# ANKITSANJYAL/nerf-few-shot-limitations

Measured on AMD Instinct MI355X. Metric: M ray-samples/sec (sample+MLP+composite) at 800^2x64, higher is better.
Workload: dtype f16; 1 GPU; 800x800 camera frame x 64 samples/ray, NeRFMLP v1 8x256, scene solid, 1 view(s)/step, 16-row pixel tiles dealt round-robin over 1 GPU(s), one launch + one all_gather per step; samples_per_ray=64, parallelism=pixel-tile x1, gather=none (one GPU)

## Files before the change

include/nerfhip.h:

```cpp
#ifndef NERFHIP_H
#define NERFHIP_H

#include <stdint.h>

#ifdef __cplusplus
extern "C" {
#endif

#define NRF_ABI_VERSION 5

#define NRF_OK            0
#define NRF_EINVAL       -1
#define NRF_EUNSUPPORTED -2
#define NRF_EHIP         -3
#define NRF_ENOMEM       -4

#define NRF_NET_V1 1
#define NRF_NET_V2 2
#define NRF_NET_V3 3

#define NRF_MMA_BF16 0
#define NRF_MMA_F16  1
#define NRF_MMA_F32  2
#define NRF_MMA_F16X3 3
// ... 79 lines not shown
                                  int64_t tile_rays, int64_t first_tile, int64_t tile_step, int64_t n_tiles,
                                  const nrf_render_opts* opts, const nrf_tail* tail,
                                  float* rgb, float* depth, float* weights, float* z_vals, void* stream);

typedef struct nrf_occupancy {
    int32_t  struct_bytes;
    int32_t  outside;
    const uint32_t* bits;
    int32_t  res[3];
    float    lo[3];
    float    scale[3];
    unsigned long long* stats;
} nrf_occupancy;

int nrf_render_rays_occ(const nrf_model* m, const float* rays_o, const float* rays_d, int64_t n_rays,
                        const nrf_render_opts* opts, const nrf_occupancy* occ,
                        float* rgb, float* depth, float* weights, float* z_vals, void* stream);
int nrf_render_camera_occ(const nrf_model* m, int H, int W, float focal, const float c2w[12],
                          int64_t ray_begin, int64_t ray_end, const nrf_render_opts* opts, const nrf_occupancy* occ,
                          float* rgb, float* depth, float* weights, float* z_vals, void* stream);
int nrf_render_cameras_tiles_occ(const nrf_model* m, int H, int W, float focal, const float* c2w, int n_cams,
                                 int64_t tile_rays, int64_t first_tile, int64_t tile_step, int64_t n_tiles,
                                 const nrf_render_opts* opts, const nrf_occupancy* occ,
                                 float* rgb, float* depth, float* weights, float* z_vals, void* stream);

int nrf_occupancy_pack(const float* density, int64_t n_cells, int k, float threshold, uint32_t* bits, void* stream);
int nrf_occupancy_dilate(const uint32_t* bits_in, const int32_t res[3], uint32_t* bits_out, void* stream);

int nrf_occupancy_mark_rays(const float* rays_o, const float* rays_d, int64_t n_rays, int n_samples,
                            const float* z_vals, const float* weights,
                            const int32_t res[3], const float lo[3], const float scale[3],
                            float weight_threshold, float seen_eps,
                            uint32_t* hit_bits, uint32_t* seen_bits, void* stream);
int nrf_occupancy_mark_camera(int H, int W, float focal, const float c2w[12], int64_t ray_begin, int64_t ray_end,
                              int n_samples, const float* z_vals, const float* weights,
                              const int32_t res[3], const float lo[3], const float scale[3],
                              float weight_threshold, float seen_eps,
                              uint32_t* hit_bits, uint32_t* seen_bits, void* stream);


int nrf_get_rays(int H, int W, float focal, const float c2w[12], int64_t ray_begin, int64_t ray_end,
                 float* rays_o, float* rays_d, void* stream);
int nrf_sample_along_rays(const float* rays_o, const float* rays_d, int64_t n_rays,
                          float near, float far, int n_samples, int lindisp, int perturb,
                          const float* t_rand, const float* z_ladder, uint64_t rng_seed,
                          float* pts, float* z_vals, void* stream);
int nrf_encode(const float* x, int64_t n, int dim, int num_freqs, int include_input, const float* freq_bands, float* out, void* stream);
int nrf_mlp_forward_v1(const nrf_model* m, int mma_mode, const float* x_enc, int64_t n, float* out4, void* stream);
int nrf_mlp_forward(const nrf_model* m, int mma_mode, const float* positions, const float* directions,
                    const float* dino, int64_t n, float* rgb, float* density, void* stream);
int nrf_composite(const float* rgb, int rgb_stride, const float* sigma, int sigma_stride,
                  const float* z_vals, const float* rays_d, int64_t n_rays, int n_samples, int white_bkgd,
                  float* out_rgb, float* out_depth, float* out_weights, void* stream);
int nrf_sample_pdf(const float* z_vals, const float* weights, int64_t n_rays, int n_samples, int n_importance,
                   const float* u, int64_t u_ray_stride, float* samples, float* z_union, void* stream);
int nrf_project_fetch(const nrf_dino* dino, const float* points, int64_t n, float* feats, float* xy, void* stream);

int nrf_sample_features(const float* features, int Hp, int Wp, int C, const float* points_2d, int64_t n, float* feats, void* stream);

int64_t nrf_fetch_backward_workspace_bytes(int Hp, int Wp, int C, int64_t n);
int nrf_project_fetch_backward(const nrf_dino* dino, const float* points, int64_t n, const float* d_feats,
                               float* d_map, int accumulate, void* ws, int64_t ws_bytes, void* stream);
int nrf_sample_features_backward(int Hp, int Wp, int C, const float* points_2d, int64_t n, const float* d_feats,
                                 float* d_map, int accumulate, void* ws, int64_t ws_bytes, void* stream);

int nrf_project_fetch_backward_points(const nrf_dino* dino, const float* points, int64_t n, const float* d_feats,
                                      float* d_points, int accumulate, void* stream);
int nrf_sample_features_backward_points(const float* features, int Hp, int Wp, int C, const float* points_2d, int64_t n,
                                        const float* d_feats, float* d_xy, void* stream);

int nrf_debug_pack(const nrf_arch* arch, const nrf_linear* linears, int n_linear, int mma_mode,
                   uint8_t* stream_out, int64_t stream_cap, int64_t* stream_bytes,
                   float* bias_out, int64_t bias_cap, int64_t* n_bias);

int nrf_debug_pack_backward(const nrf_arch* arch, const nrf_linear* linears, int n_linear, int mma_mode,
                            uint8_t* stream_out, int64_t stream_cap, int64_t* stream_bytes);
int nrf_debug_train_plan(const nrf_arch* arch, const nrf_linear* linears, int n_linear,
                         int32_t* out, int64_t cap, int64_t* n_ints);
int nrf_debug_pack_dino_grad(const nrf_arch* arch, const nrf_linear* linears, int n_linear, int mma_mode,
                             uint8_t* stream_out, int64_t stream_cap, int64_t* stream_bytes);
int nrf_debug_pack_input_grad(const nrf_arch* arch, const nrf_linear* linears, int n_linear, int mma_mode,
                              uint8_t* stream_out, int64_t stream_cap, int64_t* stream_bytes);

int nrf_debug_pack_input_grad_v3(const nrf_arch* arch, const nrf_linear* linears, int n_linear, int mma_mode,
                                 uint8_t* stream_out, int64_t stream_cap, int64_t* stream_bytes);

int nrf_debug_ray_deal(int64_t n_rays, int n_samples, int cols_per_wave, int n_cu, int64_t* head,
                       int64_t* items, int64_t cap, int64_t* n_items);

const char* nrf_last_error(void);
int nrf_abi_version(void);
int nrf_abi_sizeof(int which);

int64_t nrf_param_count(const nrf_model* m);

int nrf_model_update_device(nrf_model* m, const float* flat_params, int mode_mask, void* stream);

int64_t nrf_train_context_bytes(nrf_model* m, int mma_mode, int64_t n);

int nrf_mlp_forward_train_v1(nrf_model* m, int mma_mode, const float* x_enc, int64_t n, float* out4,
                             void* ctx, int64_t ctx_bytes, void* stream);

int nrf_mlp_backward_v1(nrf_model* m, int mma_mode, const float* out4, const float* g_out4, int64_t n,
                        void* ctx, int64_t ctx_bytes, float* flat_grad, void* stream);

int nrf_mlp_forward_train(nrf_model* m, int mma_mode, const float* positions, const float* directions,
                          const float* dino , int64_t n,
                          float* rgb, float* density, void* ctx, int64_t ctx_bytes, void* stream);
int nrf_mlp_backward(nrf_model* m, int mma_mode, const float* rgb, const float* density,
                     const float* g_rgb, const float* g_density, int64_t n,
                     void* ctx, int64_t ctx_bytes, float* flat_grad, void* stream);

int nrf_mlp_backward_dino(nrf_model* m, int mma_mode, int64_t n, void* ctx, int64_t ctx_bytes, float* d_dino, void* stream);

int nrf_mlp_backward_inputs(nrf_model* m, int mma_mode, int64_t n, void* ctx, int64_t ctx_bytes,
                            const float* positions, const float* directions,
                            float* d_x_enc, float* d_positions, float* d_directions, void* stream);

int nrf_mlp_backward_inputs_v3(nrf_model* m, int mma_mode, int64_t n, void* ctx, int64_t ctx_bytes,
                               const float* positions, const float* directions,
                               float* d_positions, float* d_directions, void* stream);

int nrf_composite_backward(const float* rgb, int rgb_stride, const float* sigma, int sigma_stride,
                           const float* z_vals, const float* rays_d, int64_t n_rays, int n_samples, int white_bkgd,
                           const float* g_rgb, const float* g_depth, const float* g_weights,
                           float* d_rgb, int d_rgb_stride, float* d_sigma, int d_sigma_stride, void* stream);
int nrf_composite_backward_geom(const float* rgb, int rgb_stride, const float* sigma, int sigma_stride,
                                const float* z_vals, const float* rays_d, int64_t n_rays, int n_samples, int white_bkgd,
                                const float* g_rgb, const float* g_depth, const float* g_weights,
                                float* d_rgb, int d_rgb_stride, float* d_sigma, int d_sigma_stride,
                                float* d_z, float* d_rays_d, void* stream);
int nrf_ray_grad(const float* d_points, const float* d_dirs, const float* z_vals, const float* rays_d,
                 const float* d_z_in, const float* d_rays_d_in, int64_t n_rays, int n_samples,
                 float* d_rays_o, float* d_rays_d, float* d_z_out, void* stream);

int nrf_mse_grad(const float* pred, const float* target, int64_t n, float weight, float* g_pred, float* loss, void* stream);

int nrf_composite_mse_backward(const float* rgb, int rgb_stride, const float* sigma, int sigma_stride,
                               const float* z_vals, const float* rays_d, int64_t n_rays, int n_samples, int white_bkgd,
                               const float* target, float weight, float* pred,
                               float* d_rgb, int d_rgb_stride, float* d_sigma, int d_sigma_stride,
                               float* ray_loss, float* zero_buf, int64_t zero_n, void* stream);

int nrf_adam_step(float* params, const float* grads, float* exp_avg, float* exp_avg_sq, int64_t n,
                  float lr, float beta1, float beta2, float eps, float weight_decay, int step, void* stream);
int nrf_adam_step_loss(float* params, const float* grads, float* exp_avg, float* exp_avg_sq, int64_t n,
                       float lr, float beta1, float beta2, float eps, float weight_decay, int step,
                       const float* ray_loss, int64_t n_rays, float loss_weight, float* loss, void* stream);

typedef struct nrf_loss_opts {
    int32_t      struct_bytes;
    float        rgb_weight;
    float        reg_weight;
    float        depth_weight;
    const float* target_depth;
    float        noise_std;
    const float* noise;
    uint64_t     rng_seed;
} nrf_loss_opts;

int nrf_composite_loss_backward(const float* rgb, int rgb_stride, const float* sigma, int sigma_stride,
                                const float* z_vals, const float* rays_d, int64_t n_rays, int n_samples, int white_bkgd,
                                const float* target, const nrf_loss_opts* loss, float* pred,
                                float* d_rgb, int d_rgb_stride, float* d_sigma, int d_sigma_stride,
                                float* ray_terms, float* zero_buf, int64_t zero_n, void* stream);

// ... 56 lines not shown
```

nerf_few_shot_limitations_amd/_lib.py:

```python
from __future__ import annotations

import ctypes as C
import os
import threading

import torch

_PKG = os.path.dirname(os.path.abspath(__file__))
LIB_PATH = os.path.join(_PKG, "libnerfhip.so")

NRF_NET_V1, NRF_NET_V2, NRF_NET_V3 = 1, 2, 3
MMA_MODES = {"bf16": 0, "f16": 1, "f32": 2, "f16x3": 3}
TRAIN_MODE = {"bf16": "bf16", "f16": "f16", "f32": "f32", "f16x3": "f32"}
TAIL_MODES = {"f16x3": 3}
TAIL_BASE_MODES = ("bf16", "f16")
ERRORS = {-1: "NRF_EINVAL", -2: "NRF_EUNSUPPORTED", -3: "NRF_EHIP", -4: "NRF_ENOMEM"}

c_float_p = C.POINTER(C.c_float)


class NrfError(RuntimeError):
    def __init__(self, code: int, msg: str):
        super().__init__(f"libnerfhip: {ERRORS.get(code, code)}: {msg}")
        self.code = code
# ... 56 lines not shown
class nrf_compact(C.Structure):
    _fields_ = [("struct_bytes", C.c_int32), ("reserved", C.c_int32), ("capacity", C.c_int64), ("index", C.c_void_p), ("slot", C.c_void_p),
                ("positions", C.c_void_p), ("directions", C.c_void_p), ("count", C.c_void_p), ("workspace", C.c_void_p),
                ("workspace_bytes", C.c_int64)]


def compact(capacity=0, index=None, slot=None, positions=None, directions=None, count=None, workspace=None, workspace_bytes=0):
    return nrf_compact(C.sizeof(nrf_compact), 0, int(capacity), index, slot, positions, directions, count, workspace, int(workspace_bytes))


SIGNATURES = {
    "nrf_abi_version": (C.c_int, []),
    "nrf_last_error": (C.c_char_p, []),
    "nrf_abi_sizeof": (C.c_int, [C.c_int]),
    "nrf_model_create": (C.c_int, [C.POINTER(C.c_void_p), C.c_int, C.POINTER(nrf_arch), C.POINTER(nrf_linear), C.c_int]),
    "nrf_model_update": (C.c_int, [C.c_void_p, C.POINTER(nrf_linear), C.c_int, C.c_void_p]),
    "nrf_model_destroy": (None, [C.c_void_p]),
    "nrf_model_flops_per_sample": (C.c_int64, [C.c_void_p]),
    "nrf_render_rays": (C.c_int, [C.c_void_p, C.c_void_p, C.c_void_p, C.c_int64, C.POINTER(nrf_render_opts),
                                  C.c_void_p, C.c_void_p, C.c_void_p, C.c_void_p, C.c_void_p]),
    "nrf_render_camera": (C.c_int, [C.c_void_p, C.c_int, C.c_int, C.c_float, C.c_float * 12, C.c_int64, C.c_int64,
                                    C.POINTER(nrf_render_opts), C.c_void_p, C.c_void_p, C.c_void_p, C.c_void_p, C.c_void_p]),
    "nrf_render_cameras_tiles": (C.c_int, [C.c_void_p, C.c_int, C.c_int, C.c_float, C.c_void_p, C.c_int, C.c_int64, C.c_int64, C.c_int64,
                                           C.c_int64, C.POINTER(nrf_render_opts), C.c_void_p, C.c_void_p, C.c_void_p, C.c_void_p, C.c_void_p]),
    "nrf_render_tail_bytes": (C.c_int64, [C.c_int64]),
    "nrf_render_rays_tail": (C.c_int, [C.c_void_p, C.c_void_p, C.c_void_p, C.c_int64, C.POINTER(nrf_render_opts), C.POINTER(nrf_tail),
                                       C.c_void_p, C.c_void_p, C.c_void_p, C.c_void_p, C.c_void_p]),
    "nrf_render_camera_tail": (C.c_int, [C.c_void_p, C.c_int, C.c_int, C.c_float, C.c_float * 12, C.c_int64, C.c_int64,
                                         C.POINTER(nrf_render_opts), C.POINTER(nrf_tail), C.c_void_p, C.c_void_p, C.c_void_p, C.c_void_p, C.c_void_p]),
    "nrf_render_cameras_tiles_tail": (C.c_int, [C.c_void_p, C.c_int, C.c_int, C.c_float, C.c_void_p, C.c_int, C.c_int64, C.c_int64, C.c_int64,
                                                C.c_int64, C.POINTER(nrf_render_opts), C.POINTER(nrf_tail), C.c_void_p, C.c_void_p, C.c_void_p,
                                                C.c_void_p, C.c_void_p]),
    "nrf_render_rays_occ": (C.c_int, [C.c_void_p, C.c_void_p, C.c_void_p, C.c_int64, C.POINTER(nrf_render_opts), C.POINTER(nrf_occupancy),
                                      C.c_void_p, C.c_void_p, C.c_void_p, C.c_void_p, C.c_void_p]),
    "nrf_render_camera_occ": (C.c_int, [C.c_void_p, C.c_int, C.c_int, C.c_float, C.c_float * 12, C.c_int64, C.c_int64,
                                        C.POINTER(nrf_render_opts), C.POINTER(nrf_occupancy), C.c_void_p, C.c_void_p, C.c_void_p, C.c_void_p, C.c_void_p]),
    "nrf_render_cameras_tiles_occ": (C.c_int, [C.c_void_p, C.c_int, C.c_int, C.c_float, C.c_void_p, C.c_int, C.c_int64, C.c_int64, C.c_int64,
                                               C.c_int64, C.POINTER(nrf_render_opts), C.POINTER(nrf_occupancy), C.c_void_p, C.c_void_p, C.c_void_p,
                                               C.c_void_p, C.c_void_p]),
    "nrf_occupancy_pack": (C.c_int, [C.c_void_p, C.c_int64, C.c_int, C.c_float, C.c_void_p, C.c_void_p]),
    "nrf_occupancy_dilate": (C.c_int, [C.c_void_p, C.c_int32 * 3, C.c_void_p, C.c_void_p]),
    "nrf_occupancy_mark_rays": (C.c_int, [C.c_void_p, C.c_void_p, C.c_int64, C.c_int, C.c_void_p, C.c_void_p, C.c_int32 * 3, C.c_float * 3,
                                          C.c_float * 3, C.c_float, C.c_float, C.c_void_p, C.c_void_p, C.c_void_p]),
    "nrf_occupancy_mark_camera": (C.c_int, [C.c_int, C.c_int, C.c_float, C.c_float * 12, C.c_int64, C.c_int64, C.c_int, C.c_void_p, C.c_void_p,
                                            C.c_int32 * 3, C.c_float * 3, C.c_float * 3, C.c_float, C.c_float, C.c_void_p, C.c_void_p, C.c_void_p]),
    "nrf_get_rays": (C.c_int, [C.c_int, C.c_int, C.c_float, C.c_float * 12, C.c_int64, C.c_int64, C.c_void_p, C.c_void_p, C.c_void_p]),
    "nrf_sample_along_rays": (C.c_int, [C.c_void_p, C.c_void_p, C.c_int64, C.c_float, C.c_float, C.c_int, C.c_int, C.c_int,
                                        C.c_void_p, C.c_void_p, C.c_uint64, C.c_void_p, C.c_void_p, C.c_void_p]),
    "nrf_encode": (C.c_int, [C.c_void_p, C.c_int64, C.c_int, C.c_int, C.c_int, C.c_void_p, C.c_void_p, C.c_void_p]),
    "nrf_mlp_forward_v1": (C.c_int, [C.c_void_p, C.c_int, C.c_void_p, C.c_int64, C.c_void_p, C.c_void_p]),
    "nrf_mlp_forward": (C.c_int, [C.c_void_p, C.c_int, C.c_void_p, C.c_void_p, C.c_void_p, C.c_int64, C.c_void_p, C.c_void_p, C.c_void_p]),
    "nrf_composite": (C.c_int, [C.c_void_p, C.c_int, C.c_void_p, C.c_int, C.c_void_p, C.c_void_p, C.c_int64, C.c_int, C.c_int,
                                C.c_void_p, C.c_void_p, C.c_void_p, C.c_void_p]),
    "nrf_sample_pdf": (C.c_int, [C.c_void_p, C.c_void_p, C.c_int64, C.c_int, C.c_int, C.c_void_p, C.c_int64, C.c_void_p, C.c_void_p, C.c_void_p]),
    "nrf_debug_pack": (C.c_int, [C.POINTER(nrf_arch), C.POINTER(nrf_linear), C.c_int, C.c_int, C.c_void_p, C.c_int64,
                                 C.POINTER(C.c_int64), C.c_void_p, C.c_int64, C.POINTER(C.c_int64)]),
    "nrf_debug_ray_deal": (C.c_int, [C.c_int64, C.c_int, C.c_int, C.c_int, C.POINTER(C.c_int64), C.POINTER(C.c_int64), C.c_int64, C.POINTER(C.c_int64)]),
    "nrf_project_fetch": (C.c_int, [C.POINTER(nrf_dino), C.c_void_p, C.c_int64, C.c_void_p, C.c_void_p, C.c_void_p]),
    "nrf_sample_features": (C.c_int, [C.c_void_p, C.c_int, C.c_int, C.c_int, C.c_void_p, C.c_int64, C.c_void_p, C.c_void_p]),
    "nrf_debug_pack_backward": (C.c_int, [C.POINTER(nrf_arch), C.POINTER(nrf_linear), C.c_int, C.c_int, C.c_void_p, C.c_int64, C.POINTER(C.c_int64)]),
    "nrf_debug_train_plan": (C.c_int, [C.POINTER(nrf_arch), C.POINTER(nrf_linear), C.c_int, C.c_void_p, C.c_int64, C.POINTER(C.c_int64)]),
    "nrf_debug_pack_dino_grad": (C.c_int, [C.POINTER(nrf_arch), C.POINTER(nrf_linear), C.c_int, C.c_int, C.c_void_p, C.c_int64, C.POINTER(C.c_int64)]),
    "nrf_fetch_backward_workspace_bytes": (C.c_int64, [C.c_int, C.c_int, C.c_int, C.c_int64]),
    "nrf_project_fetch_backward": (C.c_int, [C.POINTER(nrf_dino), C.c_void_p, C.c_int64, C.c_void_p, C.c_void_p, C.c_int, C.c_void_p, C.c_int64,
                                             C.c_void_p]),
    "nrf_sample_features_backward": (C.c_int, [C.c_int, C.c_int, C.c_int, C.c_void_p, C.c_int64, C.c_void_p, C.c_void_p, C.c_int, C.c_void_p,
                                               C.c_int64, C.c_void_p]),
    "nrf_mlp_backward_dino": (C.c_int, [C.c_void_p, C.c_int, C.c_int64, C.c_void_p, C.c_int64, C.c_void_p, C.c_void_p]),
    "nrf_mlp_backward_inputs": (C.c_int, [C.c_void_p, C.c_int, C.c_int64, C.c_void_p, C.c_int64, C.c_void_p, C.c_void_p, C.c_void_p, C.c_void_p,
                                          C.c_void_p, C.c_void_p]),
    "nrf_composite_backward_geom": (C.c_int, [C.c_void_p, C.c_int, C.c_void_p, C.c_int, C.c_void_p, C.c_void_p, C.c_int64, C.c_int, C.c_int,
                                              C.c_void_p, C.c_void_p, C.c_void_p, C.c_void_p, C.c_int, C.c_void_p, C.c_int, C.c_void_p, C.c_void_p,
                                              C.c_void_p]),
    "nrf_ray_grad": (C.c_int, [C.c_void_p, C.c_void_p, C.c_void_p, C.c_void_p, C.c_void_p, C.c_void_p, C.c_int64, C.c_int, C.c_void_p, C.c_void_p,
                               C.c_void_p, C.c_void_p]),
    "nrf_debug_pack_input_grad": (C.c_int, [C.POINTER(nrf_arch), C.POINTER(nrf_linear), C.c_int, C.c_int, C.c_void_p, C.c_int64, C.POINTER(C.c_int64)]),
    "nrf_mlp_backward_inputs_v3": (C.c_int, [C.c_void_p, C.c_int, C.c_int64, C.c_void_p, C.c_int64, C.c_void_p, C.c_void_p, C.c_void_p, C.c_void_p,
                                             C.c_void_p]),
    "nrf_project_fetch_backward_points": (C.c_int, [C.POINTER(nrf_dino), C.c_void_p, C.c_int64, C.c_void_p, C.c_void_p, C.c_int, C.c_void_p]),
    "nrf_sample_features_backward_points": (C.c_int, [C.c_void_p, C.c_int, C.c_int, C.c_int, C.c_void_p, C.c_int64, C.c_void_p, C.c_void_p,
                                                      C.c_void_p]),
    "nrf_debug_pack_input_grad_v3": (C.c_int, [C.POINTER(nrf_arch), C.POINTER(nrf_linear), C.c_int, C.c_int, C.c_void_p, C.c_int64,
                                               C.POINTER(C.c_int64)]),
    "nrf_param_count": (C.c_int64, [C.c_void_p]),
    "nrf_model_update_device": (C.c_int, [C.c_void_p, C.c_void_p, C.c_int, C.c_void_p]),
    "nrf_train_context_bytes": (C.c_int64, [C.c_void_p, C.c_int, C.c_int64]),
    "nrf_mlp_forward_train_v1": (C.c_int, [C.c_void_p, C.c_int, C.c_void_p, C.c_int64, C.c_void_p, C.c_void_p, C.c_int64, C.c_void_p]),
    "nrf_mlp_backward_v1": (C.c_int, [C.c_void_p, C.c_int, C.c_void_p, C.c_void_p, C.c_int64, C.c_void_p, C.c_int64, C.c_void_p, C.c_void_p]),
    "nrf_mlp_forward_train": (C.c_int, [C.c_void_p, C.c_int, C.c_void_p, C.c_void_p, C.c_void_p, C.c_int64, C.c_void_p, C.c_void_p, C.c_void_p, C.c_int64,
                                        C.c_void_p]),
    "nrf_mlp_backward": (C.c_int, [C.c_void_p, C.c_int, C.c_void_p, C.c_void_p, C.c_void_p, C.c_void_p, C.c_int64, C.c_void_p, C.c_int64,
                                   C.c_void_p, C.c_void_p]),
    "nrf_composite_backward": (C.c_int, [C.c_void_p, C.c_int, C.c_void_p, C.c_int, C.c_void_p, C.c_void_p, C.c_int64, C.c_int, C.c_int,
                                         C.c_void_p, C.c_void_p, C.c_void_p, C.c_void_p, C.c_int, C.c_void_p, C.c_int, C.c_void_p]),
    "nrf_mse_grad": (C.c_int, [C.c_void_p, C.c_void_p, C.c_int64, C.c_float, C.c_void_p, C.c_void_p, C.c_void_p]),
    "nrf_composite_mse_backward": (C.c_int, [C.c_void_p, C.c_int, C.c_void_p, C.c_int, C.c_void_p, C.c_void_p, C.c_int64, C.c_int, C.c_int,
                                             C.c_void_p, C.c_float, C.c_void_p, C.c_void_p, C.c_int, C.c_void_p, C.c_int, C.c_void_p, C.c_void_p,
                                             C.c_int64, C.c_void_p]),
    "nrf_adam_step": (C.c_int, [C.c_void_p, C.c_void_p, C.c_void_p, C.c_void_p, C.c_int64, C.c_float, C.c_float, C.c_float, C.c_float,
                                C.c_float, C.c_int, C.c_void_p]),
    "nrf_adam_step_loss": (C.c_int, [C.c_void_p, C.c_void_p, C.c_void_p, C.c_void_p, C.c_int64, C.c_float, C.c_float, C.c_float, C.c_float,
                                     C.c_float, C.c_int, C.c_void_p, C.c_int64, C.c_float, C.c_void_p, C.c_void_p]),
    "nrf_composite_loss_backward": (C.c_int, [C.c_void_p, C.c_int, C.c_void_p, C.c_int, C.c_void_p, C.c_void_p, C.c_int64, C.c_int, C.c_int,
                                              C.c_void_p, C.POINTER(nrf_loss_opts), C.c_void_p, C.c_void_p, C.c_int, C.c_void_p, C.c_int,
                                              C.c_void_p, C.c_void_p, C.c_int64, C.c_void_p]),
    "nrf_grad_sqnorm_workspace_bytes": (C.c_int64, [C.c_int64]),
    "nrf_grad_sqnorm_partials": (C.c_int, [C.c_void_p, C.c_int64, C.c_void_p, C.c_int64, C.c_void_p]),
    "nrf_adamw_step_loss": (C.c_int, [C.c_void_p, C.c_void_p, C.c_void_p, C.c_void_p, C.c_int64, C.c_float, C.c_float, C.c_float, C.c_float,
                                      C.c_float, C.c_int, C.c_int, C.c_float, C.c_void_p, C.c_void_p, C.c_void_p, C.c_int64, C.c_int,
                                      C.c_float, C.c_float, C.c_float, C.c_void_p, C.c_void_p]),
    "nrf_mlp_forward_train_rays": (C.c_int, [C.c_void_p, C.POINTER(nrf_train_rays), C.c_int64, C.POINTER(nrf_render_opts), C.c_void_p, C.c_void_p,
                                             C.c_void_p, C.c_int64, C.c_void_p]),
    "nrf_occupancy_compact_workspace_bytes": (C.c_int64, [C.c_int64]),
    "nrf_occupancy_compact_rays": (C.c_int, [C.POINTER(nrf_train_rays), C.c_int64, C.POINTER(nrf_render_opts), C.POINTER(nrf_occupancy),
                                             C.POINTER(nrf_compact), C.c_void_p]),
    "nrf_composite_loss_backward_indexed": (C.c_int, [C.c_void_p, C.c_int, C.c_void_p, C.c_int, C.c_void_p, C.c_void_p, C.c_int64, C.c_int, C.c_int,
                                                      C.c_void_p, C.POINTER(nrf_loss_opts), C.c_void_p, C.c_void_p, C.c_void_p, C.c_int, C.c_void_p,
                                                      C.c_int, C.c_void_p, C.c_void_p, C.c_int64, C.c_void_p]),
}

_lib = None
_lock = threading.Lock()


def lib() -> C.CDLL:
    global _lib
    if _lib is not None:
        return _lib
    with _lock:
        if _lib is None:
            if not os.path.exists(LIB_PATH):
                raise RuntimeError(f"{LIB_PATH} is missing: build it with `python -m nerf_few_shot_limitations_amd.build` "
                                   "(there is no fallback path)")
            handle = C.CDLL(LIB_PATH, mode=C.RTLD_GLOBAL)
            for name, (res, args) in SIGNATURES.items():
                fn = getattr(handle, name)
                fn.restype, fn.argtypes = res, args
            if handle.nrf_abi_version() != 5:
                raise RuntimeError("libnerfhip.so ABI version mismatch")
            for which, st in enumerate((nrf_arch, nrf_linear, nrf_dino, nrf_render_opts, nrf_tail)):
                if handle.nrf_abi_sizeof(which) != C.sizeof(st):
                    raise RuntimeError(f"libnerfhip.so: sizeof({st.__name__}) differs from the ctypes declaration")
            _lib = handle
    return _lib


def check(code: int) -> None:
    if code != 0:
        raise NrfError(code, lib().nrf_last_error().decode("utf-8", "replace"))


def ptr(t):
    if t is None:
        return None
    if not (t.is_cuda and t.dtype == torch.float32 and t.is_contiguous()):
        raise ValueError("expected a contiguous float32 tensor on the GPU")
    return t.data_ptr()


def dev_f32(t, device=None):
    if (type(t) is torch.Tensor and t.is_cuda and t.dtype == torch.float32 and not t.requires_grad and t.is_contiguous()
            and (device is None or t.device == device)):
        return t
    t = torch.as_tensor(t)
    if device is None:
        device = t.device if t.is_cuda else torch.device("cuda", torch.cuda.current_device())
# ... 77 lines not shown
```

nerf_few_shot_limitations_amd/build.py:

```python
from __future__ import annotations

import concurrent.futures as cf
import os
import shutil
import subprocess
import sys

PKG = os.path.dirname(os.path.abspath(__file__))
CSRC = os.path.join(PKG, "csrc")
OBJ = os.path.join(PKG, "build")
LIB = os.path.join(PKG, "libnerfhip.so")
INCLUDE = os.path.join(os.path.dirname(PKG), "include")

HALF16 = ["-DNRF_TU_HALF=16", "-DNRF_ACT_AGPR=1", "-mllvm", "-amdgpu-mfma-vgpr-form=1"]
HALF32 = ["-DNRF_TU_HALF=32"]
FUSED = [(f"fused_{fam}.hip", f"fused_{fam}_{half}", flags) for fam in ("v1", "v2", "v3", "v3w") for half, flags in (("16", HALF16), ("32", HALF32))]
TAIL = [("fused_tail.hip", "fused_tail", HALF32)]
OCC = [(f"fused_occ_{fam}.hip", f"fused_occ_{fam}_{half}", flags) for fam in ("v1", "v2", "v3", "v3w") for half, flags in (("16", HALF16), ("32", HALF32))]
SOURCES = FUSED + OCC + TAIL + [(f, os.path.splitext(f)[0], []) for f in
                   ("fused_kernels.hip", "train_shared.hip", "train_v1.hip", "train_v2.hip", "train_v3.hip", "train_dino_grad.hip", "train_input_grad.hip", "train_input_grad_v3.hip", "staged_kernels.hip", "api.cpp",
                    "packing.cpp")]
FLAGS = ["--offload-arch=gfx950", "-O3", "-std=c++17", "-fPIC", "-x", "hip", "-Wall", "-Wno-unused-function", "-Wno-unused-variable",
         "-fno-gpu-rdc", "-ffp-contract=off", "-Rpass-analysis=kernel-resource-usage", f"-I{INCLUDE}"]


def hipcc() -> str:
    exe = shutil.which("hipcc") or "/opt/rocm/bin/hipcc"
    if not os.path.exists(exe):
        raise RuntimeError("hipcc not found: libnerfhip.so cannot be built (ROCm toolchain required)")
    return exe


def _newest(paths):
    return max(os.path.getmtime(p) for p in paths)


def _deps():
    return [os.path.join(CSRC, f) for f in os.listdir(CSRC) if os.path.isfile(os.path.join(CSRC, f))] + [os.path.join(INCLUDE, "nerfhip.h"), os.path.abspath(__file__)]


def _obj_fresh(obj: str, cmd_key: str) -> bool:
    dep, key = obj + ".d", obj + ".cmd"
    if not (os.path.exists(obj) and os.path.exists(dep) and os.path.exists(key)):
        return False
    with open(key) as f:
        if f.read() != cmd_key:
            return False
    with open(dep) as f:
        words = f.read().replace("\\\n", " ").split()
    files = [w for w in words[1:] if not w.endswith(":")]
    t = os.path.getmtime(obj)
    return all(os.path.exists(p) and os.path.getmtime(p) <= t for p in files)


def build(force: bool = False, verbose: bool = False) -> str:
    deps = _deps()
    if not force and os.path.exists(LIB) and os.path.getmtime(LIB) >= _newest(deps):
        return LIB
    os.makedirs(OBJ, exist_ok=True)

    def one(item):
        src, name, flags = item
        obj = os.path.join(OBJ, name + ".o")
        cmd = [hipcc(), *FLAGS, *flags, "-MD", "-MF", obj + ".d", "-c", os.path.join(CSRC, src), "-o", obj]
        cmd_key = " ".join(cmd)
        if not force and _obj_fresh(obj, cmd_key):
            return obj, False
        if verbose:
            print(cmd_key, flush=True)
        r = subprocess.run(cmd, capture_output=True, text=True)
        if r.returncode != 0:
            raise RuntimeError(f"hipcc failed on {src}:\n{r.stdout}\n{r.stderr}")
        with open(obj + ".remarks", "w") as f:
            f.write(r.stderr)
        with open(obj + ".cmd", "w") as f:
            f.write(cmd_key)
        return obj, True

    with cf.ThreadPoolExecutor(max_workers=os.cpu_count() or 8) as ex:
        res = list(ex.map(one, SOURCES))
    objs = [o for o, _ in res]
    if not any(built for _, built in res) and os.path.exists(LIB) and os.path.getmtime(LIB) >= _newest(objs):
        os.utime(LIB)
        return LIB
    cmd = [hipcc(), "--offload-arch=gfx950", "-shared", "-fPIC", "-o", LIB + ".tmp", *objs]
    if verbose:
        print(" ".join(cmd), flush=True)
    r = subprocess.run(cmd, capture_output=True, text=True)
    if r.returncode != 0:
        raise RuntimeError(f"link failed:\n{r.stdout}\n{r.stderr}")
    os.replace(LIB + ".tmp", LIB)
    return LIB


def kernel_resources(obj_dir: str = OBJ):
    import re
    keys = {"VGPRs": "vgprs", "AGPRs": "agprs", "TotalSGPRs": "sgprs", "ScratchSize [bytes/lane]": "scratch", "VGPRs Spill": "vgpr_spill",
            "SGPRs Spill": "sgpr_spill", "Occupancy [waves/SIMD]": "occupancy", "LDS Size [bytes/block]": "lds"}
    out, mangled = {}, []
    for fn in sorted(os.listdir(obj_dir)):
        if not fn.endswith(".o.remarks"):
            continue
        cur = None
        with open(os.path.join(obj_dir, fn)) as f:
            for line in f:
                m = re.search(r"remark:\s+Function Name: (\S+)", line)
                if m:
                    cur = {"tu": fn[: -len(".o.remarks")]}
                    out[(fn, m.group(1))] = cur
                    mangled.append((fn, m.group(1)))
                    continue
                m = re.search(r"remark:\s+([A-Za-z ]+(?:\[[^\]]+\])?): (\d+)", line)
                if m and cur is not None and m.group(1).strip() in keys:
                    cur[keys[m.group(1).strip()]] = int(m.group(2))
    filt = shutil.which("c++filt") or shutil.which("llvm-cxxfilt") or "/usr/bin/c++filt"
    names = [n for _, n in mangled]
    if names and os.path.exists(filt):
        names = subprocess.run([filt], input="\n".join(names), capture_output=True, text=True).stdout.splitlines()
    return {f"{out[k]['tu']}: {n}": out[k] for k, n in zip(mangled, names)}


if __name__ == "__main__":
    print(build(force="--force" in sys.argv[1:], verbose=True))
```

nerf_few_shot_limitations_amd/csrc/api.cpp:

```cpp
#include <hip/hip_runtime.h>

#include <algorithm>
#include <cmath>
#include <cstdint>
#include <cstring>
#include <new>
#include <string>
#include <vector>

#include "../../include/nerfhip.h"
#include "kernels.hpp"
#include "packing.hpp"
#include "ray_deal.hpp"

namespace {

thread_local std::string g_err;

int fail(int code, const std::string& msg) {
    g_err = msg;
    return code;
}

int hip_fail(hipError_t e, const char* what) {
// ... 1 lines not shown
}

#define NRF_HIP(call)                                    \
    do {                                                 \
        const hipError_t e_ = (call);                    \
        if (e_ != hipSuccess) return hip_fail(e_, #call); \
    } while (0)

struct DeviceGuard {
    int prev = -1;
    bool ok = false;
    explicit DeviceGuard(int dev) {
        if (hipGetDevice(&prev) != hipSuccess) return;
        ok = (prev == dev) || (hipSetDevice(dev) == hipSuccess);
    }
    ~DeviceGuard() {
        int cur = -1;
        if (prev >= 0 && hipGetDevice(&cur) == hipSuccess && cur != prev) (void)hipSetDevice(prev);
    }
};

bool copy_linears(const nrf_linear* in, int n, std::vector<nrf::HostLinear>& out, std::string& err) {
    out.resize(n);
    for (int i = 0; i < n; ++i) {
        if (!in[i].weight || !in[i].bias || in[i].out_f <= 0 || in[i].in_f <= 0) {
            err = "linear " + std::to_string(i) + ": null pointer or non-positive shape";
            return false;
        }
        out[i].out_f = in[i].out_f;
        out[i].in_f = in[i].in_f;
        out[i].w.assign(in[i].weight, in[i].weight + (size_t)in[i].out_f * in[i].in_f);
        out[i].b.assign(in[i].bias, in[i].bias + in[i].out_f);
    }
    return true;
}

nrf::Camera make_camera(int H, int W, float focal, const float c2w[12]) {
    nrf::Camera c;
    c.H = H; c.W = W; c.focal = focal;
    for (int i = 0; i < 3; ++i) {
        for (int j = 0; j < 3; ++j) c.r[i][j] = c2w[4 * i + j];
        c.t[i] = c2w[4 * i + 3];
    }
    return c;
}

bool make_dino(const nrf_dino* in, int want_c, nrf::DinoDev& d, std::string& err) {
    if (!in || !in->features) { err = "dino side channel missing (features == NULL)"; return false; }
    if (in->Hp < 1 || in->Wp < 1 || in->C < 1 || in->H < 1 || in->W < 1) { err = "dino: bad map / image size"; return false; }
    if (want_c > 0 && in->C != want_c) { err = "dino: channel count differs from the model's dino_dim"; return false; }
    d.features = in->features; d.Hp = in->Hp; d.Wp = in->Wp; d.C = in->C;
    std::memcpy(d.inv_pose, in->inv_pose, sizeof(float) * 12);
    d.focal = in->focal; d.H = in->H; d.W = in->W;
    return true;
}

}

struct nrf_model {
    nrf_arch arch{};
    int device = 0;
    nrf::NetPlan plan;
    std::vector<nrf::HostLinear> lin;
    nrf::PackedStream h_stream[nrf::kModes];
    std::vector<float> h_bias;
    void* d_stream[nrf::kModes] = {nullptr, nullptr, nullptr, nullptr};
    float* d_bias = nullptr;
    unsigned long long* d_queues = nullptr;
    nrf::DeviceNet net{};
    bool train_ready = false;
    bool lin_stale = false;
    bool bfresh[3] = {false, false, false};
    nrf::ParamLayout layout;
    nrf::NetPlan bplan;
    int g_frags16 = 0;
    int i_frags16[2] = {0, 0};
    nrf::TrainPlan tplan;
    nrf::TrainDev train{};
    void* d_bstream[3] = {nullptr, nullptr, nullptr};
    int32_t* d_maps = nullptr;
    int32_t* d_src[2][3] = {{nullptr, nullptr, nullptr}, {nullptr, nullptr, nullptr}};
    int64_t n_src[2][3] = {{0, 0, 0}, {0, 0, 0}};
    int32_t* d_bias_src = nullptr;
};

namespace {

int upload(nrf_model* m, hipStream_t s, bool allocate) {
    for (int mode = 0; mode < nrf::kModes; ++mode) {
        m->h_stream[mode] = nrf::pack_stream(m->plan, m->lin, mode);
        const size_t bytes = m->h_stream[mode].bytes.size();
        if (allocate) NRF_HIP(hipMalloc(&m->d_stream[mode], bytes));
        NRF_HIP(hipMemcpyAsync(m->d_stream[mode], m->h_stream[mode].bytes.data(), bytes, hipMemcpyHostToDevice, s));
        m->net.stream[mode] = m->d_stream[mode];
        m->net.n_chunks[mode] = m->h_stream[mode].n_chunks;
    }
    m->lin_stale = false;
    if (m->train_ready) {
        for (int mode = 0; mode < 3; ++mode) {
            const nrf::PackedStream ps = nrf::pack_stream(m->bplan, m->lin, mode);
            NRF_HIP(hipMemcpyAsync(m->d_bstream[mode], ps.bytes.data(), ps.bytes.size(), hipMemcpyHostToDevice, s));
            NRF_HIP(hipStreamSynchronize(s));
            m->bfresh[mode] = true;
        }
    }
    m->h_bias = nrf::pack_bias(m->plan, m->lin);
    if (allocate) NRF_HIP(hipMalloc((void**)&m->d_bias, m->h_bias.size() * sizeof(float)));
    if (allocate) {
        NRF_HIP(hipMalloc((void**)&m->d_queues, nrf::kQueueSlots * sizeof(unsigned long long)));
        m->net.queues = m->d_queues;
    }
    NRF_HIP(hipMemcpyAsync(m->d_bias, m->h_bias.data(), m->h_bias.size() * sizeof(float), hipMemcpyHostToDevice, s));
    NRF_HIP(hipStreamSynchronize(s));
    m->net.bias = m->d_bias;
    m->net.n_bias = m->plan.n_bias;
    m->net.flops_per_sample = m->plan.flops_per_sample;
    return NRF_OK;
}

int ensure_sources(nrf_model* m) {
    if (m->d_src[0][0]) return NRF_OK;
    m->layout = nrf::param_layout(m->lin);
    for (int kind = 0; kind < 3; ++kind) {
        const std::vector<int32_t> src = nrf::stream_sources(m->plan, m->layout, kind);
        NRF_HIP(hipMalloc((void**)&m->d_src[0][kind], src.size() * sizeof(int32_t)));
        NRF_HIP(hipMemcpy(m->d_src[0][kind], src.data(), src.size() * sizeof(int32_t), hipMemcpyHostToDevice));
        m->n_src[0][kind] = (int64_t)src.size();
    }
    const std::vector<int32_t> bsrc = nrf::bias_sources(m->plan, m->layout);
    NRF_HIP(hipMalloc((void**)&m->d_bias_src, bsrc.size() * sizeof(int32_t)));
    NRF_HIP(hipMemcpy(m->d_bias_src, bsrc.data(), bsrc.size() * sizeof(int32_t), hipMemcpyHostToDevice));
    return NRF_OK;
}

int ensure_train(nrf_model* m) {
    if (m->train_ready) return NRF_OK;
    int rc = ensure_sources(m);
    if (rc != NRF_OK) return rc;
    std::string err;
    if (!nrf::make_backward_plan(m->arch, m->lin, m->bplan, err) || !nrf::make_train_plan(m->arch, m->plan, m->layout, m->tplan, err))
        return fail(NRF_EUNSUPPORTED, err);
    if ((int)m->tplan.slot_tiles.size() > nrf::kMaxSlots || (int)m->tplan.jobs.size() > nrf::kMaxJobs || m->tplan.n_mask_slots > nrf::kMaxMaskSlots)
        return fail(NRF_EUNSUPPORTED, "network too deep for the training path");
    if (m->arch.net == NRF_NET_V3) {
        nrf::NetPlan gplan;
        if (!nrf::make_dino_grad_plan(m->arch, m->lin, gplan, err)) return fail(NRF_EUNSUPPORTED, err);
        m->g_frags16 = gplan.layers[0].MT * gplan.layers[0].KT * 2;
        m->bplan.layers.push_back(gplan.layers[0]);
        nrf::NetPlan iplan;
        if (!nrf::make_input_grad_v3_plan(m->arch, m->lin, iplan, err)) return fail(NRF_EUNSUPPORTED, err);
        for (size_t i = 0; i < iplan.layers.size() && i < 2; ++i) {
            m->i_frags16[i] = iplan.layers[i].MT * iplan.layers[i].KT * 2;
            m->bplan.layers.push_back(iplan.layers[i]);
        }
    } else {
        nrf::NetPlan iplan;
        if (!nrf::make_input_grad_plan(m->arch, m->lin, iplan, err)) return fail(NRF_EUNSUPPORTED, err);
        for (size_t i = 0; i < iplan.layers.size() && i < 2; ++i) {
            m->i_frags16[i] = iplan.layers[i].MT * iplan.layers[i].KT * 2;
            m->bplan.layers.push_back(iplan.layers[i]);
        }
    }
    for (int mode = 0; mode < 3; ++mode) {
        const nrf::PackedStream ps = nrf::pack_stream(m->bplan, m->lin, mode);
        NRF_HIP(hipMalloc(&m->d_bstream[mode], ps.bytes.size()));
        NRF_HIP(hipMemcpy(m->d_bstream[mode], ps.bytes.data(), ps.bytes.size(), hipMemcpyHostToDevice));
        const uint32_t g_chunks = (uint32_t)(m->g_frags16 * (mode == NRF_MMA_F32 ? 2 : 1) / 16);
        uint32_t i_chunks = 0;
        for (int i = 0; i < 2; ++i) i_chunks += (uint32_t)((m->i_frags16[i] * (mode == NRF_MMA_F32 ? 2 : 1) + 15) / 16);
        m->train.bstream[mode] = m->d_bstream[mode];
        m->train.n_bchunks[mode] = ps.n_chunks - g_chunks - i_chunks;
        m->train.gstream[mode] = g_chunks ? static_cast<const char*>(m->d_bstream[mode]) + (size_t)m->train.n_bchunks[mode] * 16 * 1024 : nullptr;
        m->train.istream[mode] = i_chunks ? static_cast<const char*>(m->d_bstream[mode]) + ((size_t)m->train.n_bchunks[mode] + g_chunks) * 16 * 1024 : nullptr;
        m->bfresh[mode] = !m->lin_stale;
    }
    for (int f32 = 0; f32 < 2; ++f32) {
        const std::vector<int32_t> src = nrf::stream_sources(m->bplan, m->layout, f32);
        NRF_HIP(hipMalloc((void**)&m->d_src[1][f32], src.size() * sizeof(int32_t)));
        NRF_HIP(hipMemcpy(m->d_src[1][f32], src.data(), src.size() * sizeof(int32_t), hipMemcpyHostToDevice));
        m->n_src[1][f32] = (int64_t)src.size();
    }
    const int nj = (int)m->tplan.jobs.size();
    std::vector<int32_t> maps((size_t)nj * nrf::kMapStride, -1);
    for (int j = 0; j < nj; ++j) {
        const nrf::GradJobPlan& J = m->tplan.jobs[j];
        if (J.row_w.size() > 320 || J.col.size() > 320) return fail(NRF_EUNSUPPORTED, "layer too wide for the weight-gradient maps");
        std::copy(J.row_w.begin(), J.row_w.end(), maps.begin() + (size_t)j * nrf::kMapStride);
        std::copy(J.row_b.begin(), J.row_b.end(), maps.begin() + (size_t)j * nrf::kMapStride + 320);
        std::copy(J.col.begin(), J.col.end(), maps.begin() + (size_t)j * nrf::kMapStride + 640);
        m->train.job_x_slot[j] = J.x_slot; m->train.job_dz_slot[j] = J.dz_slot; m->train.job_KT[j] = J.KT; m->train.job_MT[j] = J.MT; m->train.job_x_first[j] = J.x_first;
    }
    NRF_HIP(hipMalloc((void**)&m->d_maps, maps.size() * sizeof(int32_t)));
    NRF_HIP(hipMemcpy(m->d_maps, maps.data(), maps.size() * sizeof(int32_t), hipMemcpyHostToDevice));
    m->train.maps = m->d_maps;
    m->train.n_jobs = nj;
    m->train.n_slots = (int)m->tplan.slot_tiles.size();
    for (int i = 0; i < m->train.n_slots; ++i) m->train.slot_tiles[i] = m->tplan.slot_tiles[i];
    m->train.n_mask_slots = m->tplan.n_mask_slots;
    m->train.aux_floats = m->tplan.aux_floats;
    m->train.cu_count = m->net.cu_count;
    m->train.n_params = m->layout.total;
    m->train_ready = true;
    return NRF_OK;
}

int check_opts(const nrf_render_opts* o) {
    if (!o) return fail(NRF_EINVAL, "opts is NULL");
    if (o->n_samples < 1 || o->n_samples > 4096) return fail(NRF_EINVAL, "n_samples must be in 1..4096");
    if (!(o->near > 0.0f) || !(o->far > o->near) || !std::isfinite(o->far)) return fail(NRF_EINVAL, "need 0 < near < far");
    if (o->mma_mode < 0 || o->mma_mode >= nrf::kModes) return fail(NRF_EINVAL, "unknown mma_mode");
// ... 55 lines not shown

int launch_any(const nrf_model* m, const nrf_render_opts* opts, const nrf_tail* tail, const nrf_occupancy* occ, const nrf::RenderArgs& a, void* stream,
               std::string& err) {
    if (occ) return nrf::launch_render_occ(m->net, opts->mma_mode, a, make_occ(occ), (hipStream_t)stream, err);
    if (tail) return nrf::launch_render_tail(m->net, opts->mma_mode, a, static_cast<float*>(tail->workspace), (hipStream_t)stream, err);
    return nrf::launch_render(m->net, opts->mma_mode, a, (hipStream_t)stream, err);
}

int render_rays_any(const nrf_model* m, const float* rays_o, const float* rays_d, int64_t n_rays, const nrf_render_opts* opts,
                    const nrf_tail* tail, bool tailed, const nrf_occupancy* occ, float* rgb, float* depth, float* weights, float* z_vals, void* stream);
int render_camera_any(const nrf_model* m, int H, int W, float focal, const float c2w[12], int64_t ray_begin, int64_t ray_end,
                      const nrf_render_opts* opts, const nrf_tail* tail, bool tailed, const nrf_occupancy* occ, float* rgb, float* depth, float* weights, float* z_vals,
                      void* stream);
int render_cameras_tiles_any(const nrf_model* m, int H, int W, float focal, const float* c2w, int n_cams, int64_t tile_rays,
                             int64_t first_tile, int64_t tile_step, int64_t n_tiles, const nrf_render_opts* opts, const nrf_tail* tail,
                             bool tailed, const nrf_occupancy* occ, float* rgb, float* depth, float* weights, float* z_vals, void* stream);

}

extern "C" {

int nrf_abi_version(void) { return NRF_ABI_VERSION; }

int nrf_abi_sizeof(int which) {
    switch (which) {
        case 0: return (int)sizeof(nrf_arch);
        case 1: return (int)sizeof(nrf_linear);
        case 2: return (int)sizeof(nrf_dino);
        case 3: return (int)sizeof(nrf_render_opts);
        case 4: return (int)sizeof(nrf_tail);
        default: return -1;
    }
}

const char* nrf_last_error(void) { return g_err.c_str(); }

int nrf_model_create(nrf_model** out, int device, const nrf_arch* arch, const nrf_linear* linears, int n_linear) {
    if (!out || !arch || !linears || n_linear <= 0) return fail(NRF_EINVAL, "nrf_model_create: null argument");
    *out = nullptr;
    nrf_model* m = new (std::nothrow) nrf_model();
    if (!m) return fail(NRF_ENOMEM, "out of host memory");
    m->arch = *arch;
    m->device = device;
    std::string err;
    if (!copy_linears(linears, n_linear, m->lin, err) || !nrf::make_plan(*arch, m->lin, m->plan, err)) {
        delete m;
        return fail(NRF_EINVAL, err);
    }
    DeviceGuard guard(device);
    if (!guard.ok) { delete m; return fail(NRF_EHIP, "cannot select device " + std::to_string(device)); }
    hipDeviceProp_t prop;
    if (hipGetDeviceProperties(&prop, device) != hipSuccess) { delete m; return fail(NRF_EHIP, "hipGetDeviceProperties failed"); }
    if (std::string(prop.gcnArchName).rfind("gfx950", 0) != 0) {
        delete m;
        return fail(NRF_EUNSUPPORTED, std::string("libnerfhip is built for gfx950 only, device is ") + prop.gcnArchName);
    }
    m->net.arch = *arch;
    m->net.device = device;
    m->net.cu_count = prop.multiProcessorCount;
    const int rc = upload(m, nullptr, true);
    if (rc != NRF_OK) { nrf_model_destroy(m); return rc; }
    *out = m;
    return NRF_OK;
}

int nrf_model_update(nrf_model* m, const nrf_linear* linears, int n_linear, void* stream) {
    if (!m || !linears) return fail(NRF_EINVAL, "nrf_model_update: null argument");
    std::string err;
    std::vector<nrf::HostLinear> lin;
    nrf::NetPlan plan;
    if (!copy_linears(linears, n_linear, lin, err) || !nrf::make_plan(m->arch, lin, plan, err)) return fail(NRF_EINVAL, err);
    m->lin.swap(lin);
    m->plan = plan;
    DeviceGuard guard(m->device);
    if (!guard.ok) return fail(NRF_EHIP, "cannot select the model's device");
    return upload(m, (hipStream_t)stream, false);
}

void nrf_model_destroy(nrf_model* m) {
    if (!m) return;
    DeviceGuard guard(m->device);
    for (int i = 0; i < nrf::kModes; ++i)
        if (m->d_stream[i]) (void)hipFree(m->d_stream[i]);
    if (m->d_bias) (void)hipFree(m->d_bias);
    if (m->d_queues) (void)hipFree(m->d_queues);
    for (int i = 0; i < 3; ++i)
        if (m->d_bstream[i]) (void)hipFree(m->d_bstream[i]);
    for (int i = 0; i < 2; ++i)
        for (int j = 0; j < 3; ++j)
            if (m->d_src[i][j]) (void)hipFree(m->d_src[i][j]);
    if (m->d_maps) (void)hipFree(m->d_maps);
    if (m->d_bias_src) (void)hipFree(m->d_bias_src);
    delete m;
}

int64_t nrf_model_flops_per_sample(const nrf_model* m) { return m ? m->plan.flops_per_sample : 0; }

int64_t nrf_render_tail_bytes(int64_t n_rays) {
    if (n_rays < 0) { (void)fail(NRF_EINVAL, "nrf_render_tail_bytes: n_rays < 0"); return -1; }
    return (nrf::render_tail_floats(n_rays) * (int64_t)sizeof(float) + 15) & ~(int64_t)15;
}

int nrf_render_rays(const nrf_model* m, const float* rays_o, const float* rays_d, int64_t n_rays, const nrf_render_opts* opts,
                    float* rgb, float* depth, float* weights, float* z_vals, void* stream) {
    return render_rays_any(m, rays_o, rays_d, n_rays, opts, nullptr, false, nullptr, rgb, depth, weights, z_vals, stream);
}
int nrf_render_rays_tail(const nrf_model* m, const float* rays_o, const float* rays_d, int64_t n_rays, const nrf_render_opts* opts,
                         const nrf_tail* tail, float* rgb, float* depth, float* weights, float* z_vals, void* stream) {
    return render_rays_any(m, rays_o, rays_d, n_rays, opts, tail, true, nullptr, rgb, depth, weights, z_vals, stream);
}
int nrf_render_camera(const nrf_model* m, int H, int W, float focal, const float c2w[12], int64_t ray_begin, int64_t ray_end,
                      const nrf_render_opts* opts, float* rgb, float* depth, float* weights, float* z_vals, void* stream) {
    return render_camera_any(m, H, W, focal, c2w, ray_begin, ray_end, opts, nullptr, false, nullptr, rgb, depth, weights, z_vals, stream);
}
int nrf_render_camera_tail(const nrf_model* m, int H, int W, float focal, const float c2w[12], int64_t ray_begin, int64_t ray_end,
                           const nrf_render_opts* opts, const nrf_tail* tail, float* rgb, float* depth, float* weights, float* z_vals,
                           void* stream) {
    return render_camera_any(m, H, W, focal, c2w, ray_begin, ray_end, opts, tail, true, nullptr, rgb, depth, weights, z_vals, stream);
}
int nrf_render_cameras_tiles(const nrf_model* m, int H, int W, float focal, const float* c2w, int n_cams, int64_t tile_rays,
                             int64_t first_tile, int64_t tile_step, int64_t n_tiles, const nrf_render_opts* opts, float* rgb, float* depth,
                             float* weights, float* z_vals, void* stream) {
    return render_cameras_tiles_any(m, H, W, focal, c2w, n_cams, tile_rays, first_tile, tile_step, n_tiles, opts, nullptr, false, nullptr, rgb, depth,
                                    weights, z_vals, stream);
}
int nrf_render_cameras_tiles_tail(const nrf_model* m, int H, int W, float focal, const float* c2w, int n_cams, int64_t tile_rays,
                                  int64_t first_tile, int64_t tile_step, int64_t n_tiles, const nrf_render_opts* opts, const nrf_tail* tail,
                                  float* rgb, float* depth, float* weights, float* z_vals, void* stream) {
    return render_cameras_tiles_any(m, H, W, focal, c2w, n_cams, tile_rays, first_tile, tile_step, n_tiles, opts, tail, true, nullptr, rgb, depth,
                                    weights, z_vals, stream);
}

int nrf_render_rays_occ(const nrf_model* m, const float* rays_o, const float* rays_d, int64_t n_rays, const nrf_render_opts* opts,
                        const nrf_occupancy* occ, float* rgb, float* depth, float* weights, float* z_vals, void* stream) {
    if (check_occ(occ, n_rays) != NRF_OK) return NRF_EINVAL;
    return render_rays_any(m, rays_o, rays_d, n_rays, opts, nullptr, false, occ, rgb, depth, weights, z_vals, stream);
}
int nrf_render_camera_occ(const nrf_model* m, int H, int W, float focal, const float c2w[12], int64_t ray_begin, int64_t ray_end,
                          const nrf_render_opts* opts, const nrf_occupancy* occ, float* rgb, float* depth, float* weights, float* z_vals,
                          void* stream) {
    if (check_occ(occ, ray_end - ray_begin) != NRF_OK) return NRF_EINVAL;
    return render_camera_any(m, H, W, focal, c2w, ray_begin, ray_end, opts, nullptr, false, occ, rgb, depth, weights, z_vals, stream);
}
int nrf_render_cameras_tiles_occ(const nrf_model* m, int H, int W, float focal, const float* c2w, int n_cams, int64_t tile_rays,
                                 int64_t first_tile, int64_t tile_step, int64_t n_tiles, const nrf_render_opts* opts, const nrf_occupancy* occ,
                                 float* rgb, float* depth, float* weights, float* z_vals, void* stream) {
    const double rays = (double)(n_tiles > 0 ? n_tiles : 0) * (double)(tile_rays > 0 ? tile_rays : 0) * (double)(n_cams > 0 ? n_cams : 0);
    if (check_occ(occ, rays >= 2147483648.0 ? (int64_t)1 << 31 : (int64_t)rays) != NRF_OK) return NRF_EINVAL;
    return render_cameras_tiles_any(m, H, W, focal, c2w, n_cams, tile_rays, first_tile, tile_step, n_tiles, opts, nullptr, false, occ, rgb, depth,
                                    weights, z_vals, stream);
}

int nrf_occupancy_pack(const float* density, int64_t n_cells, int k, float threshold, uint32_t* bits, void* stream) {
    if (n_cells < 0 || n_cells % 32 != 0 || k < 1) return fail(NRF_EINVAL, "nrf_occupancy_pack: n_cells must be a non-negative multiple of 32 and k >= 1");
    if (n_cells == 0) return NRF_OK;
    if (!density || !bits) return fail(NRF_EINVAL, "nrf_occupancy_pack: null pointer");
    const int r = nrf::launch_occupancy_pack(density, n_cells, k, threshold, bits, (hipStream_t)stream);
    return r == NRF_OK ? NRF_OK : fail(r, "occupancy_pack launch failed");
}

int nrf_occupancy_dilate(const uint32_t* bits_in, const int32_t res[3], uint32_t* bits_out, void* stream) {
    if (!bits_in || !bits_out || !res || bits_in == bits_out) return fail(NRF_EINVAL, "nrf_occupancy_dilate: null pointer, or bits_out is bits_in");
    for (int k = 0; k < 3; ++k)
        if (res[k] < 1 || res[k] > 512) return fail(NRF_EINVAL, "nrf_occupancy_dilate: res must be in 1..512 on every axis");
    if (res[0] % 32 != 0) return fail(NRF_EINVAL, "nrf_occupancy_dilate: res[0] must be a multiple of 32");
    const int r3[3] = {res[0], res[1], res[2]};
// ... 138 lines not shown

int nrf_sample_along_rays(const float* rays_o, const float* rays_d, int64_t n_rays, float near, float far, int n_samples, int lindisp,
                          int perturb, const float* t_rand, const float* z_ladder, uint64_t rng_seed, float* pts, float* z_vals,
                          void* stream) {
    if (n_rays < 0 || n_samples < 1) return fail(NRF_EINVAL, "bad sizes");
    if (n_rays == 0) return NRF_OK;
    if (!rays_o || !rays_d || (!pts && !z_vals)) return fail(NRF_EINVAL, "null pointer");
    const int r = nrf::launch_sample(rays_o, rays_d, n_rays, near, far, n_samples, lindisp, perturb, perturb ? t_rand : nullptr, z_ladder, rng_seed,
                                     pts, z_vals, (hipStream_t)stream);
    return r == NRF_OK ? NRF_OK : fail(r, "sample launch failed");
}

int nrf_encode(const float* x, int64_t n, int dim, int num_freqs, int include_input, const float* freq_bands, float* out, void* stream) {
    if (n < 0 || dim < 1 || num_freqs < 0 || (num_freqs > 31 && !freq_bands)) return fail(NRF_EINVAL, "bad sizes");
    if (n == 0) return NRF_OK;
    if (!x || !out) return fail(NRF_EINVAL, "null pointer");
    const int r = nrf::launch_encode(x, n, dim, num_freqs, include_input, freq_bands, out, (hipStream_t)stream);
    return r == NRF_OK ? NRF_OK : fail(r, "encode launch failed");
}

int nrf_mlp_forward_v1(const nrf_model* m, int mma_mode, const float* x_enc, int64_t n, float* out4, void* stream) {
    if (!m) return fail(NRF_EINVAL, "model is NULL");
    if (n < 0) return fail(NRF_EINVAL, "n < 0");
    if (n == 0) return NRF_OK;
    if (!x_enc || !out4) return fail(NRF_EINVAL, "null pointer");
    DeviceGuard guard(m->device);
    if (!guard.ok) return fail(NRF_EHIP, "cannot select the model's device");
    std::string err;
    const int r = nrf::launch_forward_v1(m->net, mma_mode, x_enc, n, out4, (hipStream_t)stream, err);
    return r == NRF_OK ? NRF_OK : fail(r, err);
}

int nrf_mlp_forward(const nrf_model* m, int mma_mode, const float* positions, const float* directions, const float* dino, int64_t n,
                    float* rgb, float* density, void* stream) {
    if (!m) return fail(NRF_EINVAL, "model is NULL");
    if (n < 0) return fail(NRF_EINVAL, "n < 0");
    if (n == 0) return NRF_OK;
    if (!positions || !directions || !rgb || !density) return fail(NRF_EINVAL, "null pointer");
    if (m->arch.net == NRF_NET_V3 && !dino) return fail(NRF_EINVAL, "V3 needs dino features");
    DeviceGuard guard(m->device);
    if (!guard.ok) return fail(NRF_EHIP, "cannot select the model's device");
    std::string err;
    const int r = nrf::launch_forward(m->net, mma_mode, positions, directions, dino, n, rgb, density, (hipStream_t)stream, err);
    return r == NRF_OK ? NRF_OK : fail(r, err);
}

int nrf_composite(const float* rgb, int rgb_stride, const float* sigma, int sigma_stride, const float* z_vals, const float* rays_d,
                  int64_t n_rays, int n_samples, int white_bkgd, float* out_rgb, float* out_depth, float* out_weights, void* stream) {
    if (n_rays < 0 || n_samples < 1) return fail(NRF_EINVAL, "bad sizes");
    if (rgb_stride < 3 || sigma_stride < 1) return fail(NRF_EINVAL, "bad strides");
    if (n_rays == 0) return NRF_OK;
    if (!rgb || !sigma || !z_vals || !rays_d || !out_rgb) return fail(NRF_EINVAL, "null pointer");
    const int r = nrf::launch_composite(rgb, rgb_stride, sigma, sigma_stride, z_vals, rays_d, n_rays, n_samples, white_bkgd, out_rgb,
                                        out_depth, out_weights, (hipStream_t)stream);
    return r == NRF_OK ? NRF_OK : fail(r, "composite launch failed");
}

int64_t nrf_param_count(const nrf_model* m) {
    if (!m) return 0;
    int64_t n = 0;
    for (const auto& l : m->lin) n += (int64_t)l.out_f * l.in_f + l.out_f;
    return n;
}

int nrf_model_update_device(nrf_model* m, const float* flat_params, int mode_mask, void* stream) {
    if (!m || !flat_params) return fail(NRF_EINVAL, "nrf_model_update_device: null argument");
    if (mode_mask <= 0 || mode_mask >= (1 << nrf::kModes)) return fail(NRF_EINVAL, "mode_mask must select at least one of the NRF_MMA_* modes");
    DeviceGuard guard(m->device);
    if (!guard.ok) return fail(NRF_EHIP, "cannot select the model's device");
    int rc = ensure_sources(m);
    if (rc != NRF_OK) return rc;
    hipStream_t s = (hipStream_t)stream;
    bool bias = true;
    for (int mode = 0; mode < nrf::kModes; ++mode) {
        if (!(mode_mask & (1 << mode))) continue;
        const int kind = nrf::stream_kind(mode);
        const bool bwd = m->train_ready && mode < 3;
        const int32_t* src[3] = {m->d_src[0][kind], bwd ? m->d_src[1][kind] : nullptr, bias ? m->d_bias_src : nullptr};
        const int64_t n[3] = {m->n_src[0][kind], bwd ? m->n_src[1][kind] : 0, bias ? m->plan.n_bias : 0};
        const int modes[3] = {mode, mode, NRF_MMA_F32};
        void* out[3] = {m->d_stream[mode], bwd ? m->d_bstream[mode] : nullptr, bias ? m->d_bias : nullptr};
        rc = nrf::launch_repack3(flat_params, src, n, modes, out, s);
        if (rc != NRF_OK) return fail(rc, "repack launch failed");
        bias = false;
    }
    m->lin_stale = true;
    for (int k = 0; k < 3; ++k) m->bfresh[k] = (mode_mask & (1 << k)) && m->train_ready;
    return NRF_OK;
}

int64_t nrf_train_context_bytes(nrf_model* m, int mma_mode, int64_t n) {
    if (!m || n < 0 || mma_mode < 0 || mma_mode > 2) { (void)fail(NRF_EINVAL, "nrf_train_context_bytes: bad argument"); return -1; }
    DeviceGuard guard(m->device);
    if (!guard.ok) { (void)fail(NRF_EHIP, "cannot select the model's device"); return -1; }
    if (ensure_train(m) != NRF_OK) return -1;
    return nrf::train_ctx_bytes(m->train, mma_mode, n);
}

extern "C++" {
namespace {

template <class Wrong, class Launch>
int train_entry(nrf_model* m, int mma_mode, int64_t n, bool null_ptr, int64_t ctx_bytes, bool backward, Wrong&& wrong, Launch&& launch) {
    if (!m) return fail(NRF_EINVAL, "model is NULL");
    if (n < 0 || mma_mode < 0 || mma_mode > 2) return fail(NRF_EINVAL, "bad n / mma_mode (the training path is built for bf16, f16 and f32)");
    if (n == 0) return NRF_OK;
    if (null_ptr) return fail(NRF_EINVAL, "null pointer");
    if (const char* w = wrong()) return fail(NRF_EINVAL, w);
    DeviceGuard guard(m->device);
    if (!guard.ok) return fail(NRF_EHIP, "cannot select the model's device");
    const int rc = ensure_train(m);
    if (rc != NRF_OK) return rc;
    if (ctx_bytes < nrf::train_ctx_bytes(m->train, mma_mode, n)) return fail(NRF_EINVAL, "context buffer smaller than nrf_train_context_bytes");
    if (backward && !m->bfresh[mma_mode])
        return fail(NRF_EINVAL, "backward weights of this mode are older than the parameters: call nrf_model_update_device (with this mode) first");
    std::string err;
    const int r = launch(err);
    return r == NRF_OK ? NRF_OK : fail(r, err);
}

const char* any_family() { return nullptr; }

}
}

int nrf_mlp_forward_train_v1(nrf_model* m, int mma_mode, const float* x_enc, int64_t n, float* out4, void* ctx, int64_t ctx_bytes,
                             void* stream) {
    return train_entry(m, mma_mode, n, !x_enc || !out4 || !ctx, ctx_bytes, false, any_family, [&](std::string& err) {
        return nrf::launch_train_forward(m->net, m->train, mma_mode, x_enc, n, out4, ctx, (hipStream_t)stream, err);
    });
}

int nrf_mlp_backward_v1(nrf_model* m, int mma_mode, const float* out4, const float* g_out4, int64_t n, void* ctx, int64_t ctx_bytes,
                        float* flat_grad, void* stream) {
    return train_entry(m, mma_mode, n, !out4 || !g_out4 || !ctx || !flat_grad, ctx_bytes, true, any_family, [&](std::string& err) {
        return nrf::launch_train_backward(m->net, m->train, mma_mode, out4, g_out4, n, ctx, flat_grad, (hipStream_t)stream, err);
    });
}

int nrf_mlp_forward_train(nrf_model* m, int mma_mode, const float* positions, const float* directions, const float* dino, int64_t n, float* rgb,
                          float* density, void* ctx, int64_t ctx_bytes, void* stream) {
    auto wrong = [&]() -> const char* {
        if (m->arch.net == NRF_NET_V1) return "V1 models take encoded inputs: nrf_mlp_forward_train_v1";
        if (m->arch.net == NRF_NET_V3 && !dino) return "V3 needs per-sample dino features";
        return nullptr;
    };
    return train_entry(m, mma_mode, n, !positions || !directions || !rgb || !density || !ctx, ctx_bytes, false, wrong, [&](std::string& err) {
        return m->arch.net == NRF_NET_V3
            ? nrf::launch_train_forward_v3(m->net, m->train, mma_mode, positions, directions, dino, n, rgb, density, ctx, (hipStream_t)stream, err)
            : nrf::launch_train_forward_v2(m->net, m->train, mma_mode, positions, directions, n, rgb, density, ctx, (hipStream_t)stream, err);
    });
}

int nrf_mlp_backward(nrf_model* m, int mma_mode, const float* rgb, const float* density, const float* g_rgb, const float* g_density, int64_t n,
                     void* ctx, int64_t ctx_bytes, float* flat_grad, void* stream) {
    auto wrong = [&]() -> const char* { return m->arch.net == NRF_NET_V1 ? "V1 models: nrf_mlp_backward_v1" : nullptr; };
    return train_entry(m, mma_mode, n, !rgb || !density || !g_rgb || !g_density || !ctx || !flat_grad, ctx_bytes, true, wrong,
                       [&](std::string& err) {
        return m->arch.net == NRF_NET_V3
            ? nrf::launch_train_backward_v3(m->net, m->train, mma_mode, rgb, density, g_rgb, g_density, n, ctx, flat_grad, (hipStream_t)stream, err)
            : nrf::launch_train_backward_v2(m->net, m->train, mma_mode, rgb, density, g_rgb, g_density, n, ctx, flat_grad, (hipStream_t)stream, err);
    });
}

int nrf_mlp_backward_dino(nrf_model* m, int mma_mode, int64_t n, void* ctx, int64_t ctx_bytes, float* d_dino, void* stream) {
    auto wrong = [&]() -> const char* {
// ... 363 lines not shown
int nrf_project_fetch_backward(const nrf_dino* dino, const float* points, int64_t n, const float* d_feats, float* d_map, int accumulate, void* ws,
                               int64_t ws_bytes, void* stream) {
    if (!dino) return fail(NRF_EINVAL, "dino is NULL");
    if (dino->Hp < 1 || dino->Wp < 1 || dino->C < 1 || dino->H < 1 || dino->W < 1) return fail(NRF_EINVAL, "dino: bad map / image size");
    const int c = fetch_backward_check(dino->Hp, dino->Wp, dino->C, points, n, d_feats, d_map, accumulate, ws, ws_bytes);
    if (c != NRF_OK) return c == 1 ? NRF_OK : c;
    nrf::DinoDev d{};
    d.Hp = dino->Hp; d.Wp = dino->Wp; d.C = dino->C;
    std::memcpy(d.inv_pose, dino->inv_pose, sizeof(float) * 12);
    d.focal = dino->focal; d.H = dino->H; d.W = dino->W;
    const int r = nrf::launch_project_fetch_backward(d, points, n, d_feats, d_map, accumulate, (float*)ws, (hipStream_t)stream);
    return r == NRF_OK ? NRF_OK : fail(r, "project_fetch backward launch failed");
}

int nrf_sample_features_backward(int Hp, int Wp, int C, const float* points_2d, int64_t n, const float* d_feats, float* d_map, int accumulate,
                                 void* ws, int64_t ws_bytes, void* stream) {
    const int c = fetch_backward_check(Hp, Wp, C, points_2d, n, d_feats, d_map, accumulate, ws, ws_bytes);
    if (c != NRF_OK) return c == 1 ? NRF_OK : c;
    const int r = nrf::launch_sample_features_backward(Hp, Wp, C, points_2d, n, d_feats, d_map, accumulate, (float*)ws, (hipStream_t)stream);
    return r == NRF_OK ? NRF_OK : fail(r, "sample_features backward launch failed");
}

int nrf_project_fetch_backward_points(const nrf_dino* dino, const float* points, int64_t n, const float* d_feats, float* d_points, int accumulate,
                                      void* stream) {
    if (n < 0) return fail(NRF_EINVAL, "n < 0");
    if (n == 0) return NRF_OK;
    if (!points || !d_feats || !d_points) return fail(NRF_EINVAL, "null pointer");
    if (((reinterpret_cast<uintptr_t>(points) | reinterpret_cast<uintptr_t>(d_feats) | reinterpret_cast<uintptr_t>(d_points)) & 3u) != 0)
        return fail(NRF_EINVAL, "nrf_project_fetch_backward_points: float tensors must be 4-byte aligned");
    nrf::DinoDev d{};
    std::string err;
    if (!make_dino(dino, 0, d, err)) return fail(NRF_EINVAL, err);
    if ((reinterpret_cast<uintptr_t>(d.features) & 3u) != 0) return fail(NRF_EINVAL, "nrf_project_fetch_backward_points: float tensors must be 4-byte aligned");
    const int r = nrf::launch_project_fetch_backward_points(d, points, n, d_feats, d_points, accumulate, (hipStream_t)stream);
    return r == NRF_OK ? NRF_OK : fail(r, "project_fetch backward (points) launch failed");
}

int nrf_sample_features_backward_points(const float* features, int Hp, int Wp, int C, const float* points_2d, int64_t n, const float* d_feats,
                                        float* d_xy, void* stream) {
    if (n < 0 || Hp < 1 || Wp < 1 || C < 1) return fail(NRF_EINVAL, "bad sizes");
    if (n == 0) return NRF_OK;
    if (!features || !points_2d || !d_feats || !d_xy) return fail(NRF_EINVAL, "null pointer");
    if (((reinterpret_cast<uintptr_t>(features) | reinterpret_cast<uintptr_t>(points_2d) | reinterpret_cast<uintptr_t>(d_feats) |
          reinterpret_cast<uintptr_t>(d_xy)) & 3u) != 0)
        return fail(NRF_EINVAL, "nrf_sample_features_backward_points: float tensors must be 4-byte aligned");
    const int r = nrf::launch_sample_features_backward_points(features, Hp, Wp, C, points_2d, n, d_feats, d_xy, (hipStream_t)stream);
    return r == NRF_OK ? NRF_OK : fail(r, "sample_features backward (points) launch failed");
}

int nrf_debug_pack_dino_grad(const nrf_arch* arch, const nrf_linear* linears, int n_linear, int mma_mode, uint8_t* stream_out, int64_t stream_cap,
                             int64_t* stream_bytes) {
    if (!arch || !linears || n_linear <= 0) return fail(NRF_EINVAL, "nrf_debug_pack_dino_grad: null argument");
    if (mma_mode < 0 || mma_mode > 2) return fail(NRF_EINVAL, "unknown mma_mode");
    std::string err;
    std::vector<nrf::HostLinear> lin;
    nrf::NetPlan plan;
    if (!copy_linears(linears, n_linear, lin, err) || !nrf::make_dino_grad_plan(*arch, lin, plan, err)) return fail(NRF_EINVAL, err);
    const nrf::PackedStream ps = nrf::pack_stream(plan, lin, mma_mode);
    if (stream_bytes) *stream_bytes = (int64_t)ps.bytes.size();
    if (stream_out) {
        if (stream_cap < (int64_t)ps.bytes.size()) return fail(NRF_EINVAL, "stream_out too small");
        std::memcpy(stream_out, ps.bytes.data(), ps.bytes.size());
    }
    return NRF_OK;
}

int nrf_debug_pack_input_grad(const nrf_arch* arch, const nrf_linear* linears, int n_linear, int mma_mode, uint8_t* stream_out, int64_t stream_cap,
                              int64_t* stream_bytes) {
    if (!arch || !linears || n_linear <= 0) return fail(NRF_EINVAL, "nrf_debug_pack_input_grad: null argument");
    if (mma_mode < 0 || mma_mode > 2) return fail(NRF_EINVAL, "unknown mma_mode");
    std::string err;
    std::vector<nrf::HostLinear> lin;
    nrf::NetPlan plan;
    if (!copy_linears(linears, n_linear, lin, err) || !nrf::make_input_grad_plan(*arch, lin, plan, err)) return fail(NRF_EINVAL, err);
    const nrf::PackedStream ps = nrf::pack_stream(plan, lin, mma_mode);
    if (stream_bytes) *stream_bytes = (int64_t)ps.bytes.size();
    if (stream_out) {
        if (stream_cap < (int64_t)ps.bytes.size()) return fail(NRF_EINVAL, "stream_out too small");
        std::memcpy(stream_out, ps.bytes.data(), ps.bytes.size());
    }
    return NRF_OK;
}

int nrf_debug_pack_input_grad_v3(const nrf_arch* arch, const nrf_linear* linears, int n_linear, int mma_mode, uint8_t* stream_out, int64_t stream_cap,
                                 int64_t* stream_bytes) {
    if (!arch || !linears || n_linear <= 0) return fail(NRF_EINVAL, "nrf_debug_pack_input_grad_v3: null argument");
    if (mma_mode < 0 || mma_mode > 2) return fail(NRF_EINVAL, "unknown mma_mode");
    std::string err;
    std::vector<nrf::HostLinear> lin;
    nrf::NetPlan plan;
    if (!copy_linears(linears, n_linear, lin, err) || !nrf::make_input_grad_v3_plan(*arch, lin, plan, err)) return fail(NRF_EINVAL, err);
    const nrf::PackedStream ps = nrf::pack_stream(plan, lin, mma_mode);
    if (stream_bytes) *stream_bytes = (int64_t)ps.bytes.size();
    if (stream_out) {
        if (stream_cap < (int64_t)ps.bytes.size()) return fail(NRF_EINVAL, "stream_out too small");
        std::memcpy(stream_out, ps.bytes.data(), ps.bytes.size());
    }
    return NRF_OK;
}

int nrf_debug_pack_backward(const nrf_arch* arch, const nrf_linear* linears, int n_linear, int mma_mode, uint8_t* stream_out, int64_t stream_cap,
                            int64_t* stream_bytes) {
    if (!arch || !linears || n_linear <= 0) return fail(NRF_EINVAL, "nrf_debug_pack_backward: null argument");
    if (mma_mode < 0 || mma_mode > 2) return fail(NRF_EINVAL, "unknown mma_mode");
    std::string err;
    std::vector<nrf::HostLinear> lin;
    nrf::NetPlan plan, bplan;
    if (!copy_linears(linears, n_linear, lin, err) || !nrf::make_plan(*arch, lin, plan, err)) return fail(NRF_EINVAL, err);
    if (!nrf::make_backward_plan(*arch, lin, bplan, err)) return fail(NRF_EUNSUPPORTED, err);
    const nrf::PackedStream ps = nrf::pack_stream(bplan, lin, mma_mode);
    if (stream_bytes) *stream_bytes = (int64_t)ps.bytes.size();
    if (stream_out) {
        if (stream_cap < (int64_t)ps.bytes.size()) return fail(NRF_EINVAL, "stream_out too small");
        std::memcpy(stream_out, ps.bytes.data(), ps.bytes.size());
    }
    return NRF_OK;
}

int nrf_debug_train_plan(const nrf_arch* arch, const nrf_linear* linears, int n_linear, int32_t* out, int64_t cap, int64_t* n_ints) {
    if (!arch || !linears || n_linear <= 0) return fail(NRF_EINVAL, "nrf_debug_train_plan: null argument");
    std::string err;
    std::vector<nrf::HostLinear> lin;
    nrf::NetPlan plan;
    nrf::TrainPlan tp;
    if (!copy_linears(linears, n_linear, lin, err) || !nrf::make_plan(*arch, lin, plan, err)) return fail(NRF_EINVAL, err);
    if (!nrf::make_train_plan(*arch, plan, nrf::param_layout(lin), tp, err)) return fail(NRF_EUNSUPPORTED, err);
    std::vector<int32_t> v;
    v.push_back((int32_t)tp.slot_tiles.size());
    v.insert(v.end(), tp.slot_tiles.begin(), tp.slot_tiles.end());
    v.push_back((int32_t)tp.jobs.size());
    for (const auto& J : tp.jobs) {
        v.push_back(J.x_slot); v.push_back(J.dz_slot); v.push_back(J.KT); v.push_back(J.MT); v.push_back(J.x_first);
        v.insert(v.end(), J.row_w.begin(), J.row_w.end());
        v.insert(v.end(), J.row_b.begin(), J.row_b.end());
        v.insert(v.end(), J.col.begin(), J.col.end());
    }
    v.push_back(tp.n_mask_slots);
    if (n_ints) *n_ints = (int64_t)v.size();
    if (out) {
        if (cap < (int64_t)v.size()) return fail(NRF_EINVAL, "out too small");
        std::memcpy(out, v.data(), v.size() * sizeof(int32_t));
    }
    return NRF_OK;
}

int nrf_debug_ray_deal(int64_t n_rays, int n_samples, int cols_per_wave, int n_cu, int64_t* head, int64_t* items, int64_t cap, int64_t* n_items) {
    if (n_rays <= 0 || n_samples <= 0 || n_cu <= 0 || (cols_per_wave != 32 && cols_per_wave != 64) || !head)
        return fail(NRF_EINVAL, "nrf_debug_ray_deal: bad argument");
    constexpr int waves = 4;
    const int whole = waves * cols_per_wave;
    const nrf::Deal d = nrf::pick_deal(n_rays, n_samples, waves, cols_per_wave, n_cu);
    const int64_t grid = d.items < n_cu ? d.items : n_cu;
    head[0] = d.even; head[1] = d.spw_log2; head[2] = grid; head[3] = d.passes;
    int64_t n = 0;
    auto put = [&](int64_t b, int64_t first, int64_t rays, int l) {
        if (items && n < cap) { items[4 * n] = b; items[4 * n + 1] = first; items[4 * n + 2] = rays; items[4 * n + 3] = l; }
        ++n;
    };
    for (int64_t b = 0; b < grid; ++b) {
        if (d.even) {
            nrf::DealRange r = nrf::deal_range(d.items, grid, b, waves);
            while (r.rays > 0) {
                const int l = nrf::deal_split(r.rays, whole);
                put(b, r.first, whole >> l, l);
                r.first += whole >> l;
                r.rays -= whole >> l;
// ... 24 lines not shown
```

nerf_few_shot_limitations_amd/csrc/feature_map.hpp:

```cpp
#pragma once

namespace nrf {

constexpr __host__ __device__ int pe_tiles(int L) { return (3 * L + 2 + 15) / 16; }
constexpr __host__ __device__ int pe_dim(int L) { return 3 * (2 * L + 1); }

constexpr __host__ __device__ int pe_ref_index(int L, int u, int h) {
    if (u < 3 * L) return 3 + 6 * (u / 3) + 3 * h + (u % 3);
    if (u == 3 * L) return h ? 2 : 0;
    if (u == 3 * L + 1) return h ? -1 : 1;
    return -1;
}

constexpr __host__ __device__ int k_tile(int k) { return k >> 5; }
constexpr __host__ __device__ int k_half(int k) { return (k >> 2) & 1; }
constexpr __host__ __device__ int k_reg(int k) { return (k & 3) | (((k & 31) >> 3) << 2); }
constexpr __host__ __device__ int k_slot(int k) { return 16 * k_tile(k) + k_reg(k); }
constexpr __host__ __device__ int slot_k(int u, int h) {
    const int t = u >> 4, r = u & 15;
    return 32 * t + (r & 3) + 8 * (r >> 2) + 4 * h;
}

}
```

nerf_few_shot_limitations_amd/csrc/fused_impl.hpp:

```cpp
#pragma once
#include <atomic>
#include <cstdlib>

#include "kernels.hpp"
#include "nets.hpp"
#include "ray_deal.hpp"

namespace nrf {

constexpr int kBiasMaxFloats = 4096;
constexpr int kLdsRing = kSlots * kChunkBytes;
constexpr int kLdsBytes = kLdsRing + kBiasMaxFloats * 4 + 64 + 4096;
constexpr int kLadderLds = 4096;
constexpr int kRenderThreads = 256;
constexpr int kLdsBytesQueue = kLdsRing + kBiasMaxFloats * 4 + 64 + kLadderLds * 4 + 14 * kRenderThreads * 4;
static_assert(kLdsBytesQueue <= 160 * 1024, "renderers: LDS over budget (use a 6-slot ring)");

struct NetArgs {
    const void* stream;
    const float* bias;
    uint32_t n_chunks;
    int n_bias;
    int n_layers;
};

struct RenderKArgs {
    NetArgs net;
    RenderArgs a;
    int64_t n_tiles;
    int even = 0;
    float* carry = nullptr;
};

struct ForwardKArgs {
    NetArgs net;
    const float* x_enc;
    const float* pos;
    const float* dir;
    const float* dino;
    int64_t n;
    float* out4;
    float* rgb;
    float* density;
    int64_t n_tiles;
};

struct OccKArgs {
    RenderKArgs r;
    OccDev g;
};

template <bool FAST>
__device__ __forceinline__ float sigmoid_sel(float x) { return FAST ? sigmoid_fast(x) : sigmoid_precise(x); }

__device__ __forceinline__ float pick_reg(float lo, float hi, bool take_hi) {
    asm volatile("" : "+v"(lo), "+v"(hi));
    return take_hi ? hi : lo;
}

__device__ __forceinline__ void load_bias_table(NRF_LDS float* bias, const float* src, int n) {
    for (int i = threadIdx.x; i < n; i += blockDim.x) bias[i] = src[i];
    __syncthreads();
}

__device__ __forceinline__ int64_t global_ray(const RenderArgs& a, int64_t i, int& cam) {
    cam = 0;
    if (!a.camera_mode) return i;
    if (a.n_cams > 1) {
        cam = (int)(i / a.rays_per_cam);
        i -= (int64_t)cam * a.rays_per_cam;
    }
    int64_t g = a.ray_begin + i;
    if (a.tile_rays < a.rays_per_cam) {
        const int64_t k = i / a.tile_rays;
        g = a.ray_begin + k * a.tile_stride + (i - k * a.tile_rays);
    }
    const int64_t last = (int64_t)a.cams[0].H * a.cams[0].W - 1;
    return g < last ? g : last;
}

enum { F_OX, F_OY, F_OZ, F_DX, F_DY, F_DZ, F_NORM, F_Z, F_T, F_R, F_G, F_B, F_DEPTH, F_ACC, kFields };
constexpr int kLdsState = kLdsRing + kBiasMaxFloats * 4 + 64 + kLadderLds * 4;

enum { kWhole = 0, kPrefix = 1, kTail = 2 };

template <class Net, class Mode, int NT, int WAVES, int LP, int LD, int PART>
__device__ __forceinline__ void render_march(const RenderKArgs& P) {
    static_assert(NT == 1 || NT == 2, "a wave marches 32 or 64 sample columns");
    constexpr int COLS = 32 * NT;
    extern __shared__ __attribute__((aligned(16))) char smem[];
    NRF_LDS char* lds = (NRF_LDS char*)smem;
    NRF_LDS float* bias = (NRF_LDS float*)(lds + kLdsRing);
    NRF_LDS float* st = (NRF_LDS float*)(lds + kLdsState);
    constexpr int nthreads = WAVES * 64;
    int tid_now = threadIdx.x;
    NRF_LDS float* st_me = st + tid_now;
    auto ST = [&](int f) -> NRF_LDS float& { return st_me[f * nthreads]; };
    typedef typename Mode::Act Act;
    constexpr int KT0 = pe_tiles(LP);

    int lane = threadIdx.x & 63, c = lane & 31, h = lane >> 5;
    const int wave = __builtin_amdgcn_readfirstlane(threadIdx.x >> 6);
    const RenderArgs& a = P.a;
    const int S = a.n_samples;
    static_assert(WAVES * 64 <= kRenderThreads, "state rows are sized for 4 waves");
    NRF_LDS float* zl = (NRF_LDS float*)(bias + kBiasMaxFloats) + 16;
    {
        const DepthLadder lad = make_ladder(a.near, a.far, S, a.lindisp, nullptr);
        for (int i = threadIdx.x; i < S; i += blockDim.x) zl[i] = a.z_ladder ? a.z_ladder[i] : ladder_z(lad, i);
    }
    load_bias_table(bias, P.net.bias, P.net.n_bias);

    Pipe<WAVES, pinned_walk<Mode, NT>()> pipe;
    pipe.init(P.net.stream, P.net.n_chunks, lds);
    pipe.start();

    auto z_base = [&](int s) -> float { return zl[s]; };
    const int SM = PART == kPrefix ? S - 1 : S;
    const int s_begin = PART == kTail ? S - 1 : 0;

    auto z_ray = [&](int64_t ray, int s) -> float {
        if (a.z_in) return a.z_in[ray * S + s];
        if (!a.perturb) return z_base(s);
        float u;
        if (a.t_rand) {
            u = a.t_rand[ray * S + s];
        } else {
            int ci;
            const int64_t g = global_ray(a, ray, ci);
            u = counter_uniform(a.seed + (uint64_t)ci * 0x51ED27ull, (uint64_t)g, (uint32_t)s);
        }
        const float zc = z_base(s);
        const float lower = s > 0 ? __fmul_rn(0.5f, __fadd_rn(zc, z_base(s - 1))) : zc;
        const float upper = s < S - 1 ? __fmul_rn(0.5f, __fadd_rn(z_base(s + 1), zc)) : zc;
        return __fadd_rn(lower, __fmul_rn(__fsub_rn(upper, lower), u));
    };

    const bool even = PART != kTail && P.even;
    int64_t next = blockIdx.x, left = 0;
    if (even) {
        const DealRange r = deal_range(P.n_tiles, gridDim.x, blockIdx.x, WAVES);
        next = r.first;
        left = r.rays;
    }
    for (;;) {
        int spw_log2 = 0;
        int64_t base;
        if (even) {
            if (left <= 0) break;
            spw_log2 = deal_split(left, WAVES * COLS);
            base = next;
            next += (WAVES * COLS) >> spw_log2;
            left -= (WAVES * COLS) >> spw_log2;
        } else {
            if (next >= P.n_tiles) break;
            if (PART != kTail) spw_log2 = a.spw_log2;
            base = next * (int64_t)(WAVES * (COLS >> spw_log2));
            next += gridDim.x;
        }
        const int rpw_log2 = (NT == 2 ? 6 : 5) - spw_log2;
        const int SPW = 1 << spw_log2, RPW = COLS >> spw_log2;
        const int n_pass = PART == kTail ? 1 : (SM + SPW - 1) >> spw_log2;
        auto column_ray = [&](int q) -> int64_t {
            const int64_t r = base + wave * RPW + (q & (RPW - 1));
            return r < a.n_rays ? r : a.n_rays - 1;
        };
        {
            const int64_t rid = column_ray(lane);
            float o[3], d[3];
            if (a.camera_mode) {
                int ci;
                const int64_t g = global_ray(a, rid, ci);
                camera_ray(a.cams[ci], g, o, d);
            } else {
#pragma unroll
                for (int k = 0; k < 3; ++k) { o[k] = a.rays_o[rid * 3 + k]; d[k] = a.rays_d[rid * 3 + k]; }
            }
            ST(F_OX) = o[0]; ST(F_OY) = o[1]; ST(F_OZ) = o[2];
            ST(F_DX) = d[0]; ST(F_DY) = d[1]; ST(F_DZ) = d[2];
            ST(F_NORM) = ray_norm(d);
            int s_first = s_begin;
            asm volatile("" : "+s"(s_first));
            ST(F_Z) = z_ray(rid, s_first);
            if (PART == kTail && S > 1) {
                const float* cy = P.carry + rid;
                ST(F_T) = cy[0]; ST(F_R) = cy[a.n_rays]; ST(F_G) = cy[2 * a.n_rays]; ST(F_B) = cy[3 * a.n_rays];
                ST(F_DEPTH) = cy[4 * a.n_rays]; ST(F_ACC) = cy[5 * a.n_rays];
            } else {
                ST(F_T) = 1.0f; ST(F_R) = 0.0f; ST(F_G) = 0.0f; ST(F_B) = 0.0f; ST(F_DEPTH) = 0.0f; ST(F_ACC) = 0.0f;
            }
        }

        for (int p = 0; p < n_pass; ++p) {
            tid_now = threadIdx.x;
            asm volatile("" : "+v"(tid_now));
            lane = tid_now & 63; c = lane & 31; h = lane >> 5;
            st_me = st + tid_now;

            auto SQ = [&](int n, int f) -> NRF_LDS float& { return (NT == 1 ? st_me : st_me - lane + c + 32 * n)[f * nthreads]; };
            auto dirT = [&](Act (&dt)[1][NT]) {
#pragma unroll
                for (int n = 0; n < NT; ++n) {
                    const float d[3] = {SQ(n, F_DX), SQ(n, F_DY), SQ(n, F_DZ)};
                    Act t1[pe_tiles(LD)];
                    encode3<Mode, LD>(d, h, t1);
                    dt[0][n] = t1[0];
                }
            };
            DinoHeld<Mode, Net::kDino ? Net::KT0 - KT0 : 1> held[NT];
            auto inputs = [&](const float (&w0)[NT], const float (&w1)[NT], Act (&x)[Net::KT0][NT], auto pass_) {
                constexpr int PASS = decltype(pass_)::value;
#pragma unroll
                for (int n = 0; n < NT; ++n) {
                    float zc;
                    if (SPW == 1) {
                        zc = SQ(n, F_Z);
                    } else {
                        const int q = c + 32 * n;
                        const int sc = p * SPW + (q >> rpw_log2);
                        zc = z_ray(column_ray(q), sc < S ? sc : S - 1);
                    }
                    float pt[3];
                    pt[0] = point_on_ray(SQ(n, F_OX), SQ(n, F_DX), zc);
                    pt[1] = point_on_ray(SQ(n, F_OY), SQ(n, F_DY), zc);
                    pt[2] = point_on_ray(SQ(n, F_OZ), SQ(n, F_DZ), zc);
                    DinoTaps tp;
                    DinoRaw<Net::kDino ? Net::KT0 - KT0 : 1> raw;
                    if constexpr (Net::kDino && PASS == 0) {
                        tp = dino_taps(a.dino, pt);
                        raw.issue(a.dino.features, tp, h);
                    }
                    Act e1[KT0];
                    encode3<Mode, LP>(pt, h, e1, w0[n]);
#pragma unroll
                    for (int t = 0; t < KT0; ++t) x[t][n] = e1[t];
                    if constexpr (Net::kDino) {
                        constexpr int DT = Net::KT0 - KT0;
                        if constexpr (PASS == 0) held[n].finish(raw, tp);
                        Act dt[DT];
                        held[n].template tiles<PASS>(w1[n], dt);
#pragma unroll
                        for (int t = 0; t < DT; ++t) x[KT0 + t][n] = dt[t];
                    }
                }
            };

            float out4[NT][4];
            Net::eval(pipe, bias, h, P.net.n_layers, inputs, dirT, out4);

            tid_now = threadIdx.x;
            asm volatile("" : "+v"(tid_now));
            lane = tid_now & 63; c = lane & 31; h = lane >> 5;
            st_me = st + tid_now;
            const int64_t rid = column_ray(lane);
            const int64_t raw = base + wave * RPW + (lane & (RPW - 1));
            const bool own_valid = lane < RPW && raw < a.n_rays;
            Composite comp;
            comp.T = ST(F_T); comp.r = ST(F_R); comp.g = ST(F_G); comp.b = ST(F_B); comp.depth = ST(F_DEPTH); comp.acc = ST(F_ACC);
            float zo = ST(F_Z);
            const float norm = ST(F_NORM);
            if (SPW == 1) {
                const int s = PART == kTail ? S - 1 : p;
                const bool last = PART == kTail || (PART == kWhole && s + 1 == S);
                float v[4];
#pragma unroll
                for (int k = 0; k < 4; ++k) v[k] = NT == 2 ? pick_reg(out4[0][k], out4[NT - 1][k], h != 0) : out4[0][k];
                const float zn = last ? 0.0f : z_ray(rid, s + 1);
                const float dist = last ? __fmul_rn(1e10f, norm) : __fmul_rn(__fsub_rn(zn, zo), norm);
                const float w = comp.template add<Mode::FAST_EXP>(v[3], sigmoid_sel<Mode::FAST_EXP>(v[0]), sigmoid_sel<Mode::FAST_EXP>(v[1]),
                                                                  sigmoid_sel<Mode::FAST_EXP>(v[2]), zo, dist);
                if (own_valid) {
                    if (a.weights) a.weights[rid * S + s] = w;
                    if (a.z_vals) a.z_vals[rid * S + s] = zo;
                }
                zo = zn;
            } else {
                const int q = NT == 2 ? lane : c;
                const int sq = p * SPW + (q >> rpw_log2);
                float ca = 0.0f, cr = 0.0f, cg = 0.0f, cb = 0.0f, cz = 0.0f;
                if (sq < SM) {
                    const bool last = PART == kWhole && (sq + 1 == S);
                    float v[4];
#pragma unroll
                    for (int k = 0; k < 4; ++k) v[k] = NT == 2 ? pick_reg(out4[0][k], out4[NT - 1][k], h != 0) : out4[0][k];
                    cz = z_ray(rid, sq);
                    const float zn = last ? 0.0f : z_ray(rid, sq + 1);
                    const float dist = last ? __fmul_rn(1e10f, norm) : __fmul_rn(__fsub_rn(zn, cz), norm);
                    ca = Composite::alpha_of<Mode::FAST_EXP>(v[3], dist);
                    cr = sigmoid_sel<Mode::FAST_EXP>(v[0]); cg = sigmoid_sel<Mode::FAST_EXP>(v[1]); cb = sigmoid_sel<Mode::FAST_EXP>(v[2]);
                }
                for (int j = 0; j < SPW; ++j) {
                    const int s = p * SPW + j;
                    if (s >= SM) break;
                    const int qj = lane + (j << rpw_log2);
                    const int src = (NT == 2 ? (qj & 63) : ((lane & 32) | (qj & 31))) << 2;
                    auto from = [&](float x) { return __builtin_bit_cast(float, __builtin_amdgcn_ds_bpermute(src, __builtin_bit_cast(int, x))); };
                    const float aj = from(ca), rj = from(cr), gj = from(cg), bj = from(cb), zj = from(cz);
                    const float w = comp.add_alpha(aj, rj, gj, bj, zj);
                    if (own_valid) {
                        if (a.weights) a.weights[rid * S + s] = w;
                        if (a.z_vals) a.z_vals[rid * S + s] = zj;
                    }
                }
            }
            ST(F_T) = comp.T; ST(F_R) = comp.r; ST(F_G) = comp.g; ST(F_B) = comp.b; ST(F_DEPTH) = comp.depth; ST(F_ACC) = comp.acc;
            ST(F_Z) = zo;
        }

        {
            const int64_t raw = base + wave * RPW + (lane & (RPW - 1));
            if (PART == kPrefix) {
                if (lane < RPW && raw < a.n_rays) {
                    float* cy = P.carry + raw;
                    cy[0] = ST(F_T); cy[a.n_rays] = ST(F_R); cy[2 * a.n_rays] = ST(F_G); cy[3 * a.n_rays] = ST(F_B);
                    cy[4 * a.n_rays] = ST(F_DEPTH); cy[5 * a.n_rays] = ST(F_ACC);
                }
            } else if (lane < RPW && raw < a.n_rays) {
                float r = ST(F_R), g = ST(F_G), b = ST(F_B);
                if (a.white_bkgd) {
                    const float bg = __fsub_rn(1.0f, ST(F_ACC));
                    r = __fadd_rn(r, bg); g = __fadd_rn(g, bg); b = __fadd_rn(b, bg);
                }
                if (a.interleaved) {
                    *(float4*)(a.rgb + raw * 4) = make_float4(r, g, b, ST(F_DEPTH));
                } else {
                    a.rgb[raw * 3 + 0] = r;
                    a.rgb[raw * 3 + 1] = g;
                    a.rgb[raw * 3 + 2] = b;
                    a.depth[raw] = ST(F_DEPTH);
                }
            }
        }
    }
    pipe.drain();
}

template <class Net, class Mode, int NT, int WAVES, int LP, int LD>
__global__ void __launch_bounds__(WAVES * 64) render_kernel(const RenderKArgs P) {
    render_march<Net, Mode, NT, WAVES, LP, LD, kWhole>(P);
}
template <class Net, class Mode, int NT, int WAVES, int LP, int LD>
__global__ void __launch_bounds__(WAVES * 64) render_hold_kernel(const RenderKArgs P) {
    render_march<Net, Mode, NT, WAVES, LP, LD, kPrefix>(P);
}
template <class Net, class Mode, int NT, int WAVES, int LP, int LD>
__global__ void __launch_bounds__(WAVES * 64) render_tail_kernel(const RenderKArgs P) {
    render_march<Net, Mode, NT, WAVES, LP, LD, kTail>(P);
}

constexpr int kStrip = 32;

__device__ __forceinline__ bool occ_skips(const OccDev& g, const float (&p)[3]) {
    float t[3];
    bool inside = true;
#pragma unroll
    for (int k = 0; k < 3; ++k) {
        t[k] = __fmul_rn(__fsub_rn(p[k], g.lo[k]), g.scale[k]);
        inside = inside && t[k] >= 0.0f && t[k] < (float)g.res[k];
    }
    if (!inside) {
        const float big = __builtin_huge_valf();
        return g.outside && fabsf(p[0]) < big && fabsf(p[1]) < big && fabsf(p[2]) < big;
    }
    const int idx = ((int)floorf(t[2]) * g.res[1] + (int)floorf(t[1])) * g.res[0] + (int)floorf(t[0]);
    return ((g.bits[idx >> 5] >> (idx & 31)) & 1u) == 0u;
}

template <class Net, class Mode, int NT, int WAVES, int LP, int LD>
__global__ void __launch_bounds__(WAVES * 64) render_queue_kernel(const RenderKArgs P) {
    constexpr bool OCC = false;
    const OccDev G{};
#include "render_queue_body.inc"
}
template <class Net, class Mode, int NT, int WAVES, int LP, int LD>
__global__ void __launch_bounds__(WAVES * 64) render_queue_occ_kernel(const OccKArgs Q) {
    constexpr bool OCC = true;
    const RenderKArgs& P = Q.r;
    const OccDev& G = Q.g;
// ... 32 lines not shown
                for (int n = 0; n < NT; ++n) {
                    float dd[3];
#pragma unroll
                    for (int k = 0; k < 3; ++k) dd[k] = P.dir[sid[n] * 3 + k];
                    Act t1[pe_tiles(LD)];
                    encode3<Mode, LD>(dd, h, t1);
                    dt[0][n] = t1[0];
                }
            }
        };
        auto inputs = [&](const float (&w0)[NT], const float (&w1)[NT], Act (&x)[Net::KT0][NT], auto) {
#pragma unroll
            for (int n = 0; n < NT; ++n) {
                if constexpr (Net::kNeedsDir) {
                    float p[3];
#pragma unroll
                    for (int k = 0; k < 3; ++k) p[k] = P.pos[sid[n] * 3 + k];
                    Act e1[KT0];
                    encode3<Mode, LP>(p, h, e1, w0[n]);
#pragma unroll
                    for (int t = 0; t < KT0; ++t) x[t][n] = e1[t];
                    if constexpr (Net::kDino) {
                        constexpr int DT = Net::KT0 - KT0;
                        const float* f = P.dino + sid[n] * (32 * DT);
#pragma unroll
                        for (int t = 0; t < DT; ++t) {
                            f32x16 e;
#pragma unroll
                            for (int g = 0; g < 4; ++g) {
                                const f32x4 v = *(const f32x4*)(f + 32 * t + 8 * g + 4 * h);
#pragma unroll
                                for (int q = 0; q < 4; ++q) e[4 * g + q] = v[q] * w1[n];
                            }
                            x[KT0 + t][n] = Mode::template to_act<false>(e);
                        }
                    }
                } else {
                    const float* xin = P.x_enc + sid[n] * PE;
                    f32x16 e[KT0];
                    static_for<16 * KT0>([&](auto u_) {
                        constexpr int u = decltype(u_)::value;
                        constexpr int i0 = pe_ref_index(LP, u, 0), i1 = pe_ref_index(LP, u, 1);
                        float val = 0.0f;
                        if constexpr (i0 >= 0 && i1 >= 0) val = xin[h ? i1 : i0];
                        else if constexpr (i0 >= 0) val = h ? 0.0f : xin[i0];
                        else if constexpr (i1 >= 0) val = h ? xin[i1] : 0.0f;
                        e[u / 16][u % 16] = val;
                    });
#pragma unroll
                    for (int t = 0; t < KT0; ++t) x[t][n] = Mode::template to_act<false>(e[t]);
                }
            }
        };
        float out4[NT][4];
        Net::eval(pipe, bias, h, P.net.n_layers, inputs, dirT, out4);
        const int64_t own_raw = tile * TILE + wave * (32 * NT) + 32 * own + c;
        if (owner && own_raw < P.n) {
            float v[4];
#pragma unroll
            for (int k = 0; k < 4; ++k) v[k] = NT == 2 ? pick_reg(out4[0][k], out4[NT - 1][k], own != 0) : out4[0][k];
            const float r = sigmoid_sel<Mode::FAST_EXP>(v[0]), g = sigmoid_sel<Mode::FAST_EXP>(v[1]), b = sigmoid_sel<Mode::FAST_EXP>(v[2]);
            if constexpr (Net::kNeedsDir) {
                P.rgb[own_raw * 3 + 0] = r; P.rgb[own_raw * 3 + 1] = g; P.rgb[own_raw * 3 + 2] = b;
                P.density[own_raw] = fmaxf(v[3], 0.0f);
            } else {
                *(float4*)(P.out4 + own_raw * 4) = make_float4(r, g, b, v[3]);
            }
        }
    }
    pipe.drain();
}

namespace {

template <class K>
int prepare(K kernel, int device, unsigned char (&done)[64], std::string& err, int lds_bytes = kLdsBytes) {
    if (device >= 0 && device < 64 && done[device]) return NRF_OK;
    const hipError_t e = hipFuncSetAttribute((const void*)kernel, hipFuncAttributeMaxDynamicSharedMemorySize, lds_bytes);
    if (e != hipSuccess) { err = std::string("hipFuncSetAttribute: ") + hipGetErrorString(e); return NRF_EHIP; }
    if (device >= 0 && device < 64) done[device] = 1;
    return NRF_OK;
}

NetArgs net_args(const DeviceNet& net, int mode) {
    NetArgs n;
    n.stream = net.stream[mode]; n.bias = net.bias; n.n_chunks = net.n_chunks[mode]; n.n_bias = net.n_bias; n.n_layers = net.arch.n_layers;
    return n;
}

template <auto kernel, int WAVES, int LDS = kLdsBytes, class KArgs>
int launch_persistent(const DeviceNet& net, const NetArgs& na, KArgs k, int64_t n_tiles, hipStream_t s, const char* what, std::string& err) {
    static unsigned char done[64] = {};
    const int prepared = prepare(kernel, net.device, done, err, LDS);
    if (prepared != NRF_OK) return prepared;
    k.net = na;
    k.n_tiles = n_tiles;
    const int64_t grid = n_tiles < net.cu_count ? n_tiles : net.cu_count;
    hipLaunchKernelGGL(kernel, dim3((unsigned)grid), dim3(WAVES * 64), LDS, s, k);
    const hipError_t e = hipGetLastError();
    if (e != hipSuccess) { err = std::string(what) + " launch: " + hipGetErrorString(e); return NRF_EHIP; }
    return NRF_OK;
}

template <class Net, class Mode, int NT, int WAVES, int LP, int LD>
int run_render_v(const DeviceNet& net, int mode, const RenderArgs& a, hipStream_t s, std::string& err) {
    RenderKArgs k;
    k.a = a;
    const Deal d = pick_deal(a.n_rays, a.n_samples, WAVES, 32 * NT, net.cu_count);
    k.a.spw_log2 = d.spw_log2;
    k.even = d.even;
    return launch_persistent<render_kernel<Net, Mode, NT, WAVES, LP, LD>, WAVES, kLdsBytesQueue>(net, net_args(net, mode), k, d.items, s, "render", err);
}

template <class Net, class Mode, int NT, int WAVES, int LP, int LD>
int run_render_hold(const DeviceNet& net, int mode, const RenderArgs& a, float* carry, hipStream_t s, std::string& err) {
    RenderKArgs k;
    k.a = a;
    k.carry = carry;
    const Deal d = pick_deal(a.n_rays, a.n_samples - 1, WAVES, 32 * NT, net.cu_count);
    k.a.spw_log2 = d.spw_log2;
    k.even = d.even;
    return launch_persistent<render_hold_kernel<Net, Mode, NT, WAVES, LP, LD>, WAVES, kLdsBytesQueue>(net, net_args(net, mode), k, d.items,
                                                                                                      s, "render (tail mode, prefix)", err);
}

template <class Net, class Mode, int NT, int WAVES, int LP, int LD>
int run_render_tail(const DeviceNet& net, int mode, const RenderArgs& a, float* carry, hipStream_t s, std::string& err) {
    RenderKArgs k;
    k.a = a;
    k.carry = carry;
    k.a.spw_log2 = 0;
    const int64_t tile = (int64_t)WAVES * 32 * NT;
    return launch_persistent<render_tail_kernel<Net, Mode, NT, WAVES, LP, LD>, WAVES, kLdsBytesQueue>(net, net_args(net, mode), k, (a.n_rays + tile - 1) / tile,
                                                                                                      s, "render (tail mode, last sample)", err);
}

inline RenderKArgs& render_part(RenderKArgs& k) { return k; }
inline RenderKArgs& render_part(OccKArgs& k) { return k.r; }

template <auto kernel, int NT, int WAVES, class KArgs>
int launch_queue(const DeviceNet& net, int mode, RenderArgs a, KArgs k, hipStream_t s, std::string& err) {
    static unsigned char done[64] = {};
    const int prepared = prepare(kernel, net.device, done, err, kLdsBytesQueue);
    if (prepared != NRF_OK) return prepared;
    static std::atomic<unsigned> turn{0};
    a.queue = net.queues + (turn.fetch_add(1) % kQueueSlots);
    hipError_t e = hipMemsetAsync(a.queue, 0, sizeof(unsigned long long), s);
    if (e != hipSuccess) { err = std::string("queue reset: ") + hipGetErrorString(e); return NRF_EHIP; }
    RenderKArgs& r = render_part(k);
    r.net = net_args(net, mode);
    r.a = a;
    r.n_tiles = 0;
    const int64_t strips = (a.n_rays + kStrip * NT - 1) / (kStrip * NT);
    const int64_t blocks = (strips + WAVES - 1) / WAVES;
    const int64_t grid = blocks < net.cu_count ? blocks : net.cu_count;
    hipLaunchKernelGGL(kernel, dim3((unsigned)grid), dim3(WAVES * 64), kLdsBytesQueue, s, k);
    e = hipGetLastError();
    if (e != hipSuccess) { err = std::string("render (ray queue) launch: ") + hipGetErrorString(e); return NRF_EHIP; }
    return NRF_OK;
}

template <class Net, class Mode, int NT, int WAVES, int LP, int LD>
int run_render_queue(const DeviceNet& net, int mode, const RenderArgs& a, hipStream_t s, std::string& err) {
    return launch_queue<render_queue_kernel<Net, Mode, NT, WAVES, LP, LD>, NT, WAVES>(net, mode, a, RenderKArgs{}, s, err);
}

template <class Net, class Mode, int NT, int WAVES, int LP, int LD>
int run_render_occ(const DeviceNet& net, int mode, const RenderArgs& a, const OccDev& g, hipStream_t s, std::string& err) {
    if (!net.queues || a.n_rays >= (int64_t)1 << 31) { err = "render with a grid: launch too large (>= 2^31 rays)"; return NRF_EINVAL; }
    OccKArgs k{};
    k.g = g;
    return launch_queue<render_queue_occ_kernel<Net, Mode, NT, WAVES, LP, LD>, NT, WAVES>(net, mode, a, k, s, err);
}

template <class Net, class Mode, int NT, int WAVES, int LP, int LD>
int run_render(const DeviceNet& net, int mode, const RenderArgs& a, hipStream_t s, std::string& err) {
    if (a.ert_eps > 0.0f) {
        if (!net.queues || a.n_rays >= (int64_t)1 << 31) { err = "early ray termination: launch too large (>= 2^31 rays)"; return NRF_EINVAL; }
        return run_render_queue<Net, Mode, NT, WAVES, LP, LD>(net, mode, a, s, err);
    }
    return run_render_v<Net, Mode, NT, WAVES, LP, LD>(net, mode, a, s, err);
}

template <class Net, class Mode, int NT, int WAVES, int LP, int LD>
int run_forward(const DeviceNet& net, int mode, const ForwardKArgs& k, hipStream_t s, std::string& err) {
    constexpr int TILE = WAVES * 32 * NT;
    return launch_persistent<forward_kernel<Net, Mode, NT, WAVES, LP, LD>, WAVES>(net, net_args(net, mode), k, (k.n + TILE - 1) / TILE, s, "forward", err);
}

bool check_net(const DeviceNet& net, int mode, std::string& err) {
    if (mode < 0 || mode >= kModes) { err = "unknown mma_mode"; return false; }
    if (net.n_bias > kBiasMaxFloats) { err = "bias table exceeds the LDS carve-out"; return false; }
    if (net.arch.dir_freq != 4 && net.arch.net != NRF_NET_V1) { err = "only dir_freq=4 is built"; return false; }
    return true;
}

}

#if !defined(NRF_TU_HALF)
#elif NRF_TU_HALF == 16
#define NRF_TU_NAME(f) f##_16
#define NRF_DISPATCH_MODE(FN, NETT, LP, ...)                                                         \
    switch (mode) {                                                                                   \
        case NRF_MMA_BF16: return FN<NETT(ModeBF16, 2), ModeBF16, 2, 4, LP, 4>(__VA_ARGS__);          \
        default:           return FN<NETT(ModeF16, 2), ModeF16, 2, 4, LP, 4>(__VA_ARGS__);            \
    }
#define NRF_DEFINE_HOLD(fam, NETT, LP)                                                                                              \
    int render_hold_##fam##_16(const DeviceNet& net, int mode, const RenderArgs& a, float* carry, hipStream_t s, std::string& err) { \
        NRF_DISPATCH_MODE(run_render_hold, NETT, LP, net, mode, a, carry, s, err)                                                   \
    }
#else
#define NRF_DEFINE_HOLD(fam, NETT, LP)
#define NRF_TU_NAME(f) f##_32
#define NRF_DISPATCH_MODE(FN, NETT, LP, ...)                                                         \
    switch (mode) {                                                                                   \
        case NRF_MMA_F16X3: return FN<NETT(ModeF16X3, 1), ModeF16X3, 1, 4, LP, 4>(__VA_ARGS__);       \
        default:            return FN<NETT(ModeF32, 1), ModeF32, 1, 4, LP, 4>(__VA_ARGS__);           \
    }
#endif
#define NRF_NET_V1_10(M, NT) NetV1<M, NT, 10>
#define NRF_NET_V2_10(M, NT) NetV2<M, NT, 10>
#define NRF_NET_V3_12_64(M, NT) NetV3<M, NT, 12, 2>
#define NRF_NET_V3_12_128(M, NT) NetV3<M, NT, 12, 4>

#define NRF_DECLARE_FAMILY(fam)                                                                                            \
    int render_##fam##_16(const DeviceNet& net, int mode, const RenderArgs& a, hipStream_t s, std::string& err);           \
    int render_##fam##_32(const DeviceNet& net, int mode, const RenderArgs& a, hipStream_t s, std::string& err);           \
    int forward_##fam##_16(const DeviceNet& net, int mode, ForwardKArgs k, hipStream_t s, std::string& err);               \
    int forward_##fam##_32(const DeviceNet& net, int mode, ForwardKArgs k, hipStream_t s, std::string& err);               \
           \
    int render_hold_##fam##_16(const DeviceNet& net, int mode, const RenderArgs& a, float* carry, hipStream_t s, std::string& err); \
    int render_tail_##fam(const DeviceNet& net, const RenderArgs& a, float* carry, hipStream_t s, std::string& err);       \
       \
    int render_occ_##fam##_16(const DeviceNet& net, int mode, const RenderArgs& a, const OccDev& g, hipStream_t s, std::string& err); \
    int render_occ_##fam##_32(const DeviceNet& net, int mode, const RenderArgs& a, const OccDev& g, hipStream_t s, std::string& err); \
    inline int render_occ_##fam(const DeviceNet& net, int mode, const RenderArgs& a, const OccDev& g, hipStream_t s, std::string& err) { \
        return (mode == NRF_MMA_BF16 || mode == NRF_MMA_F16) ? render_occ_##fam##_16(net, mode, a, g, s, err) : render_occ_##fam##_32(net, mode, a, g, s, err); \
    }                                                                                                                      \
    inline int render_##fam(const DeviceNet& net, int mode, const RenderArgs& a, hipStream_t s, std::string& err) {        \
        return (mode == NRF_MMA_BF16 || mode == NRF_MMA_F16) ? render_##fam##_16(net, mode, a, s, err) : render_##fam##_32(net, mode, a, s, err); \
    }                                                                                                                      \
    inline int forward_##fam(const DeviceNet& net, int mode, ForwardKArgs k, hipStream_t s, std::string& err) {            \
        return (mode == NRF_MMA_BF16 || mode == NRF_MMA_F16) ? forward_##fam##_16(net, mode, k, s, err) : forward_##fam##_32(net, mode, k, s, err); \
    }
NRF_DECLARE_FAMILY(v1)
NRF_DECLARE_FAMILY(v2)
NRF_DECLARE_FAMILY(v3)
NRF_DECLARE_FAMILY(v3w)

}
```

nerf_few_shot_limitations_amd/csrc/fused_kernels.hip:

```cpp
#include "fused_impl.hpp"

namespace nrf {

int launch_render(const DeviceNet& net, int mode, const RenderArgs& a, hipStream_t s, std::string& err) {
    if (!check_net(net, mode, err)) return NRF_EINVAL;
    if (a.n_rays <= 0) return NRF_OK;
    if (net.arch.net == NRF_NET_V1 && net.arch.pos_freq == 10) return render_v1(net, mode, a, s, err);
    if (net.arch.net == NRF_NET_V2 && net.arch.pos_freq == 10) return render_v2(net, mode, a, s, err);
    if (net.arch.net == NRF_NET_V3 && net.arch.pos_freq == 12 && net.arch.dino_dim == 64) return render_v3(net, mode, a, s, err);
    if (net.arch.net == NRF_NET_V3 && net.arch.pos_freq == 12 && net.arch.dino_dim == 128) return render_v3w(net, mode, a, s, err);
    err = "no fused renderer built for this (net, pos_freq): V1/V2 with pos_freq 10 (baseline.yaml) and V3 with pos_freq 12 and dino_dim 64/128 (dino_nerf.yaml, lora.yaml, multiscale.yaml) are";
    return NRF_EUNSUPPORTED;
}

int launch_render_occ(const DeviceNet& net, int mode, const RenderArgs& a, const OccDev& g, hipStream_t s, std::string& err) {
    if (!check_net(net, mode, err)) return NRF_EINVAL;
    if (a.n_rays <= 0) return NRF_OK;
    if (net.arch.net == NRF_NET_V1 && net.arch.pos_freq == 10) return render_occ_v1(net, mode, a, g, s, err);
    if (net.arch.net == NRF_NET_V2 && net.arch.pos_freq == 10) return render_occ_v2(net, mode, a, g, s, err);
    if (net.arch.net == NRF_NET_V3 && net.arch.pos_freq == 12 && net.arch.dino_dim == 64) return render_occ_v3(net, mode, a, g, s, err);
    if (net.arch.net == NRF_NET_V3 && net.arch.pos_freq == 12 && net.arch.dino_dim == 128) return render_occ_v3w(net, mode, a, g, s, err);
    err = "no fused renderer built for this (net, pos_freq): see nrf_render_rays";
    return NRF_EUNSUPPORTED;
}

int launch_render_tail(const DeviceNet& net, int base_mode, const RenderArgs& a, float* carry, hipStream_t s, std::string& err) {
    if (!check_net(net, base_mode, err) || !check_net(net, NRF_MMA_F16X3, err)) return NRF_EINVAL;
    if (a.n_rays <= 0) return NRF_OK;
    const bool prefix = a.n_samples > 1;
    int rc = NRF_OK;
    if (net.arch.net == NRF_NET_V1 && net.arch.pos_freq == 10) {
        if (prefix) rc = render_hold_v1_16(net, base_mode, a, carry, s, err);
        return rc != NRF_OK ? rc : render_tail_v1(net, a, carry, s, err);
    }
    if (net.arch.net == NRF_NET_V2 && net.arch.pos_freq == 10) {
        if (prefix) rc = render_hold_v2_16(net, base_mode, a, carry, s, err);
        return rc != NRF_OK ? rc : render_tail_v2(net, a, carry, s, err);
    }
    if (net.arch.net == NRF_NET_V3 && net.arch.pos_freq == 12 && net.arch.dino_dim == 64) {
        if (prefix) rc = render_hold_v3_16(net, base_mode, a, carry, s, err);
        return rc != NRF_OK ? rc : render_tail_v3(net, a, carry, s, err);
    }
    if (net.arch.net == NRF_NET_V3 && net.arch.pos_freq == 12 && net.arch.dino_dim == 128) {
        if (prefix) rc = render_hold_v3w_16(net, base_mode, a, carry, s, err);
        return rc != NRF_OK ? rc : render_tail_v3w(net, a, carry, s, err);
    }
    err = "no fused renderer built for this (net, pos_freq): see nrf_render_rays";
    return NRF_EUNSUPPORTED;
}

int launch_forward_v1(const DeviceNet& net, int mode, const float* x_enc, int64_t n, float* out4, hipStream_t s, std::string& err) {
    if (!check_net(net, mode, err)) return NRF_EINVAL;
    if (net.arch.net != NRF_NET_V1) { err = "nrf_mlp_forward_v1 needs a V1 model"; return NRF_EINVAL; }
    if (n <= 0) return NRF_OK;
    ForwardKArgs k{};
    k.x_enc = x_enc; k.n = n; k.out4 = out4;
    if (net.arch.pos_freq == 10) return forward_v1(net, mode, k, s, err);
    err = "no V1 forward built for this pos_freq";
    return NRF_EUNSUPPORTED;
}

int launch_forward(const DeviceNet& net, int mode, const float* pos, const float* dir, const float* dino, int64_t n,
                   float* rgb, float* density, hipStream_t s, std::string& err) {
    if (!check_net(net, mode, err)) return NRF_EINVAL;
    if (n <= 0) return NRF_OK;
    ForwardKArgs k{};
    k.pos = pos; k.dir = dir; k.dino = dino; k.n = n; k.rgb = rgb; k.density = density;
    if (net.arch.net == NRF_NET_V2 && net.arch.pos_freq == 10) return forward_v2(net, mode, k, s, err);
    if (net.arch.net == NRF_NET_V3 && net.arch.pos_freq == 12) {
        if (!dino) { err = "V3 forward needs per-sample dino features"; return NRF_EINVAL; }
        if (net.arch.dino_dim == 64) return forward_v3(net, mode, k, s, err);
        if (net.arch.dino_dim == 128) return forward_v3w(net, mode, k, s, err);
    }
    err = "no forward built for this (net, pos_freq)";
    return NRF_EUNSUPPORTED;
}

}
```

nerf_few_shot_limitations_amd/csrc/kernels.hpp:

```cpp
#pragma once
#include <hip/hip_runtime.h>
#include <stdint.h>

#include <string>

#include "../../include/nerfhip.h"
#include "device_math.hpp"

namespace nrf {

constexpr int kMaxCams = 8;
constexpr int kModes = 4;

struct DeviceNet {
    nrf_arch arch;
    const void* stream[kModes];
    uint32_t n_chunks[kModes];
    const float* bias;
    int n_bias;
    int64_t flops_per_sample;
    int device;
    int cu_count;
    unsigned long long* queues;
};

constexpr int kQueueSlots = 64;

struct DinoDev {
    const float* features;
    int Hp, Wp, C;
    float inv_pose[12];
    float focal;
    int H, W;
};

struct RenderArgs {
    const float* rays_o;
    const float* rays_d;
    int camera_mode;
    int n_cams;
    int64_t rays_per_cam;
    Camera cams[8];
    int64_t ray_begin;
    int64_t n_rays;
    int64_t tile_rays;
    int64_t tile_stride;
    float near, far;
    int n_samples, lindisp, perturb;
    const float* t_rand;
    const float* z_ladder;
    const float* z_in;
    uint64_t seed;
    float ert_eps;
    int white_bkgd;
    int interleaved;
    float* rgb;
    float* depth;
    float* weights;
    float* z_vals;
    DinoDev dino;
    unsigned long long* queue;
    int spw_log2;
};

int launch_render(const DeviceNet& net, int mma_mode, const RenderArgs& a, hipStream_t s, std::string& err);
constexpr int kCarryRows = 6;
inline int64_t render_tail_floats(int64_t n_rays) { return kCarryRows * n_rays; }
int launch_render_tail(const DeviceNet& net, int base_mode, const RenderArgs& a, float* carry, hipStream_t s, std::string& err);
struct OccDev {
    const uint32_t* bits;
    int res[3];
    float lo[3], scale[3];
    int outside;
    unsigned long long* stats;
};
int launch_render_occ(const DeviceNet& net, int mma_mode, const RenderArgs& a, const OccDev& g, hipStream_t s, std::string& err);
int launch_forward_v1(const DeviceNet& net, int mma_mode, const float* x_enc, int64_t n, float* out4, hipStream_t s, std::string& err);
int launch_forward(const DeviceNet& net, int mma_mode, const float* pos, const float* dir, const float* dino, int64_t n,
                   float* rgb, float* density, hipStream_t s, std::string& err);

constexpr int kMaxSlots = 40;
constexpr int kMaxJobs = 24;
constexpr int kMaxMaskSlots = 20;
constexpr int kMapStride = 3 * 320;

struct TrainDev {
    const void* bstream[3];
    uint32_t n_bchunks[3];
    const int32_t* maps;
    int n_slots;
    int slot_tiles[kMaxSlots];
    int n_mask_slots;
    int aux_floats;
    int cu_count;
    int n_jobs;
    int job_x_slot[kMaxJobs], job_dz_slot[kMaxJobs], job_KT[kMaxJobs], job_MT[kMaxJobs], job_x_first[kMaxJobs];
    int64_t n_params;
    const void* gstream[3];
    const void* istream[3];
};

int64_t train_ctx_bytes(const TrainDev& t, int mma_mode, int64_t n);
int launch_train_forward(const DeviceNet& net, const TrainDev& t, int mma_mode, const float* x_enc, int64_t n, float* out4, void* ctx,
                         hipStream_t s, std::string& err);
int launch_train_backward(const DeviceNet& net, const TrainDev& t, int mma_mode, const float* out4, const float* g_out4, int64_t n,
                          void* ctx, float* grad, hipStream_t s, std::string& err);
// ... 110 lines not shown
```

nerf_few_shot_limitations_amd/csrc/packing.cpp:

```cpp
#include "packing.hpp"

#include <cmath>
#include <cstring>

#include "feature_map.hpp"
#include "stream_config.hpp"
#include "train_slots.hpp"

namespace nrf {

namespace {
constexpr int kFragBytes = 1024;

uint32_t f32_bits(float x) { uint32_t u; std::memcpy(&u, &x, 4); return u; }
}

uint16_t f32_to_bf16(float x) {
    uint32_t u = f32_bits(x);
    if ((u & 0x7F800000u) == 0x7F800000u && (u & 0x007FFFFFu)) return (uint16_t)((u >> 16) | 0x0040u);
    u += 0x7FFFu + ((u >> 16) & 1u);
    return (uint16_t)(u >> 16);
}

uint16_t f32_to_f16(float x) {
// ... 149 lines not shown
        const int b = 5;
        for (int i = 0; i < n; ++i)
            if (!check(lin, b + i, H, H, "density_layers.N", err)) return false;
        if (!check(lin, b + n, 1, H, "density_head", err) || !check(lin, b + n + 1, H, H, "feature_head", err) ||
            !check(lin, b + n + 2, H / 2, H + de, "color_layers.0", err) || !check(lin, b + n + 3, H / 4, H / 2, "color_layers.2", err) ||
            !check(lin, b + n + 4, 3, H / 4, "color_layers.4", err))
            return false;
        auto fusion0 = [&]() {
            LayerPlan L; L.KT = peT + DT; L.MT = HT; L.col.assign(32 * (peT + DT), -1);
            pe_cols(L.col, 0, a.pos_freq, 0);
            for (int k = 0; k < a.dino_dim; ++k) L.col[32 * peT + k] = pe + k;
            L.row = rows_of(0, H, HT);
            return L;
        };
        auto square = [&](int li) { LayerPlan L; L.KT = HT; L.MT = HT; L.col = identity_cols(H); L.row = rows_of(li, H, HT); return L; };
        add(fusion0()); add(square(1));
        LayerPlan A0; A0.KT = HT; A0.MT = H / 128; A0.col = identity_cols(H); A0.row = rows_of(2, H / 4, H / 128); add(std::move(A0));
        LayerPlan A2; A2.KT = H / 128; A2.MT = 1; A2.col = identity_cols(H / 4); A2.row.assign(32, {-1, 0});
        for (int rep = 0; rep < 2; ++rep) { A2.row[4 * rep + 0] = {3, 0}; A2.row[4 * rep + 1] = {3, 1}; }
        add(std::move(A2));
        add(fusion0()); add(square(1));
        add(square(4));
        for (int i = 0; i < n; ++i) add(square(b + i));
        LayerPlan Dh; Dh.KT = HT; Dh.MT = 1; Dh.col = identity_cols(H); Dh.row.assign(32, {-1, 0});
        Dh.row[0] = {b + n, 0}; Dh.row[4] = {b + n, 0}; add(std::move(Dh));
        add(square(b + n + 1));
        LayerPlan C0; C0.KT = HT + 1; C0.MT = H / 64; C0.col.assign(32 * (HT + 1), -1);
        for (int k = 0; k < H; ++k) C0.col[k] = k;
        pe_cols(C0.col, H, a.dir_freq, H);
        C0.row = rows_of(b + n + 2, H / 2, H / 64); add(std::move(C0));
        LayerPlan C2; C2.KT = H / 64; C2.MT = H / 128; C2.col = identity_cols(H / 2); C2.row = rows_of(b + n + 3, H / 4, H / 128); add(std::move(C2));
        LayerPlan C4; C4.KT = H / 128; C4.MT = 1; C4.col = identity_cols(H / 4); C4.row.assign(32, {-1, 0});
        for (int rep = 0; rep < 2; ++rep)
            for (int c = 0; c < 3; ++c) C4.row[4 * rep + c] = {b + n + 4, c};
        add(std::move(C4));
    } else {
        err = "unknown network family";
        return false;
    }

    int off = 0;
    for (auto& L : plan.layers) { L.bias_off = off; off += 32 * L.MT; }
    plan.n_bias = off;
    int64_t mac = 0;
    for (const auto& l : lin) mac += (int64_t)l.out_f * l.in_f;
    if (a.net == NRF_NET_V3) mac += (int64_t)lin[0].out_f * lin[0].in_f + (int64_t)lin[1].out_f * lin[1].in_f;
    plan.flops_per_sample = 2 * mac;
    return true;
}

std::vector<float> pack_bias(const NetPlan& plan, const std::vector<HostLinear>& lin) {
    std::vector<float> b(plan.n_bias, 0.0f);
    for (const auto& L : plan.layers)
        for (int r = 0; r < 32 * L.MT; ++r)
            if (L.row[r].first >= 0) b[L.bias_off + r] = lin[L.row[r].first].b[L.row[r].second];
    return b;
}

ParamLayout param_layout(const std::vector<HostLinear>& lin) {
    ParamLayout lay;
    int64_t off = 0;
    for (const auto& l : lin) {
        lay.w_off.push_back(off); off += (int64_t)l.out_f * l.in_f;
        lay.b_off.push_back(off); off += l.out_f;
        lay.in_f.push_back(l.in_f);
    }
    lay.total = off;
    return lay;
}

namespace {
int64_t element_source(const LayerPlan& L, const ParamLayout& lay, int r, int k) {
    if (L.transposed) {
        const auto& ks = L.krow[k];
        if (ks.first < 0 || L.rcol[r] < 0) return -1;
        return lay.w_off[ks.first] + (int64_t)ks.second * lay.in_f[ks.first] + L.rcol[r];
    }
    const auto& rs = L.row[r];
    if (rs.first < 0 || L.col[k] < 0) return -1;
    return lay.w_off[rs.first] + (int64_t)rs.second * lay.in_f[rs.first] + L.col[k];
}
}

std::vector<int32_t> stream_sources(const NetPlan& plan, const ParamLayout& lay, int kind) {
    const bool f32 = kind == kStreamF32, x3 = kind == kStreamX3;
    const int SUB = (f32 || x3) ? 4 : 2, n_el = f32 ? 4 : 8;
    size_t total_frags = 0;
    for (const auto& L : plan.layers) {
        const size_t f = (size_t)L.MT * L.KT * SUB;
        total_frags += (f + kChunkFrags - 1) / kChunkFrags * kChunkFrags;
    }
    std::vector<int32_t> src(total_frags * 64 * n_el, -1);
    size_t frag = 0;
    for (const auto& L : plan.layers) {
        for (int m = 0; m < L.MT; ++m)
            for (int t = 0; t < L.KT; ++t)
                for (int s = 0; s < SUB; ++s, ++frag)
                    for (int lane = 0; lane < 64; ++lane) {
                        const int i = lane & 31, h = lane >> 5;
                        for (int e = 0; e < n_el; ++e) {
                            const int s16 = x3 ? (s >> 1) : s;
                            const int k = f32 ? (32 * t + 8 * s + 4 * h + e)
                                              : (32 * t + 16 * s16 + 8 * (e >> 2) + 4 * h + (e & 3));
                            src[(frag * 64 + lane) * n_el + e] = (int32_t)element_source(L, lay, 32 * m + i, k);
                        }
                    }
        frag = (frag + kChunkFrags - 1) / kChunkFrags * kChunkFrags;
    }
    return src;
}

std::vector<int32_t> bias_sources(const NetPlan& plan, const ParamLayout& lay) {
    std::vector<int32_t> b(plan.n_bias, -1);
    for (const auto& L : plan.layers) {
        if (L.transposed) continue;
        for (int r = 0; r < 32 * L.MT; ++r)
            if (L.row[r].first >= 0) b[L.bias_off + r] = (int32_t)(lay.b_off[L.row[r].first] + L.row[r].second);
    }
    return b;
}

PackedStream pack_stream(const NetPlan& plan, const std::vector<HostLinear>& lin, int mode) {
    const bool f32 = (mode == NRF_MMA_F32), x3 = (mode == NRF_MMA_F16X3);
    const ParamLayout lay = param_layout(lin);
    std::vector<float> flat((size_t)lay.total);
    for (size_t i = 0; i < lin.size(); ++i) {
        std::memcpy(flat.data() + lay.w_off[i], lin[i].w.data(), lin[i].w.size() * sizeof(float));
        std::memcpy(flat.data() + lay.b_off[i], lin[i].b.data(), lin[i].b.size() * sizeof(float));
    }
    const std::vector<int32_t> src = stream_sources(plan, lay, stream_kind(mode));
    PackedStream out;
    const size_t per_frag = f32 ? 256 : 512;
    out.n_chunks = (uint32_t)(src.size() / per_frag / kChunkFrags);
    out.bytes.assign(src.size() / per_frag * kFragBytes, 0);
    for (size_t i = 0; i < src.size(); ++i) {
        float v = src[i] >= 0 ? flat[src[i]] : 0.0f;
        if (!f32 && mode != NRF_MMA_BF16) v = std::fmin(std::fmax(v, -65504.0f), 65504.0f);
        if (f32) {
            std::memcpy(out.bytes.data() + i * 4, &v, 4);
        } else if (x3) {
            const uint16_t hi = f32_to_f16(v);
            uint16_t q = hi;
            if ((i / per_frag) & 1) q = f32_to_f16(v - f16_to_f32(hi));
            std::memcpy(out.bytes.data() + i * 2, &q, 2);
        } else {
            const uint16_t q = (mode == NRF_MMA_BF16) ? f32_to_bf16(v) : f32_to_f16(v);
            std::memcpy(out.bytes.data() + i * 2, &q, 2);
        }
    }
    return out;
}

bool make_backward_plan(const nrf_arch& a, const std::vector<HostLinear>& lin, NetPlan& plan, std::string& err) {
    plan = NetPlan();
    if (a.net != NRF_NET_V1 && a.net != NRF_NET_V2 && a.net != NRF_NET_V3) { err = "unknown network family"; return false; }
    if (a.hidden != 256 || (int)lin.size() != expected_linears(a)) { err = "backward plan: unexpected architecture"; return false; }
    const int n = a.n_layers, H = a.hidden, HT = H / 32;
    const int b = a.net == NRF_NET_V3 ? 5 : 0;
    auto first_cols = [&](int count, int MT) { std::vector<int> r(32 * MT, -1); for (int i = 0; i < count; ++i) r[i] = i; return r; };
    auto transposed = [&](int li, int out_rows, int KT, int in_cols, int MT) {
        LayerPlan L; L.transposed = true; L.KT = KT; L.MT = MT; L.krow.assign(32 * KT, {-1, 0});
        for (int k = 0; k < out_rows; ++k) L.krow[k] = {li, k};
        L.rcol = first_cols(in_cols, MT);
        return L;
    };
    if (a.net == NRF_NET_V1) {
        LayerPlan L; L.transposed = true; L.KT = 1; L.MT = HT; L.krow.assign(32, {-1, 0});
        for (int c = 0; c < 3; ++c) L.krow[c] = {n + 1, c};
        L.krow[3] = {n, 0};
        L.rcol = first_cols(H, HT);
        plan.layers.push_back(std::move(L));
    } else {
        plan.layers.push_back(transposed(b + n + 4, 3, 1, H / 4, H / 128));
        plan.layers.push_back(transposed(b + n + 3, H / 4, H / 128, H / 2, H / 64));
        plan.layers.push_back(transposed(b + n + 2, H / 2, H / 64, H, HT));
        LayerPlan FD = transposed(b + n + 1, H, HT + 1, H, HT);
        FD.krow[H] = {b + n, 0};
        plan.layers.push_back(std::move(FD));
    }
    for (int l = n - 1; l >= 1; --l) plan.layers.push_back(transposed(b + l, H, HT, H, HT));
    if (a.net == NRF_NET_V3) {
        NetPlan fwd;
        if (!make_plan(a, lin, fwd, err)) return false;
        const LayerPlan& F0 = fwd.layers[0];
        plan.layers.push_back(transposed(b, H, HT, H, HT));
        plan.layers.push_back(transposed(4, H, HT, H, HT));
        plan.layers.push_back(transposed(1, H, HT, H, HT));
        LayerPlan F0T = transposed(0, H, HT, 0, F0.KT);
        for (int r = 0; r < 32 * F0.KT; ++r) F0T.rcol[r] = F0.col[r];
        plan.layers.push_back(std::move(F0T));
        plan.layers.push_back(transposed(3, 2, 1, H / 4, H / 128));
        plan.layers.push_back(transposed(2, H / 4, H / 128, H, HT));
        plan.layers.push_back(transposed(1, H, HT, H, HT));
    }
    int off = 0;
    for (auto& L : plan.layers) { L.bias_off = off; off += 32 * L.MT; }
    plan.n_bias = off;
    return true;
}

bool make_dino_grad_plan(const nrf_arch& a, const std::vector<HostLinear>& lin, NetPlan& plan, std::string& err) {
    plan = NetPlan();
    if (a.net != NRF_NET_V3) { err = "the DINO feature gradient belongs to the V3 network"; return false; }
    NetPlan fwd;
    if (!make_plan(a, lin, fwd, err)) return false;
    const LayerPlan& F0 = fwd.layers[0];
    const int H = a.hidden, HT = H / 32, DT = a.dino_dim / 32, PT = F0.KT - DT;
    LayerPlan L; L.transposed = true; L.KT = HT; L.MT = DT; L.krow.assign(32 * HT, {-1, 0});
    for (int k = 0; k < H; ++k) L.krow[k] = {0, k};
    L.rcol.assign(F0.col.begin() + 32 * PT, F0.col.begin() + 32 * F0.KT);
    L.bias_off = 0;
    plan.layers.push_back(std::move(L));
    plan.n_bias = 32 * DT;
    return true;
}

bool make_input_grad_plan(const nrf_arch& a, const std::vector<HostLinear>& lin, NetPlan& plan, std::string& err) {
    plan = NetPlan();
    if (a.net != NRF_NET_V1 && a.net != NRF_NET_V2) { err = "the input gradient is built for the V1 and V2 networks"; return false; }
    NetPlan fwd;
    if (!make_plan(a, lin, fwd, err)) return false;
    const int H = a.hidden, HT = H / 32, n = a.n_layers;
    const LayerPlan& F0 = fwd.layers[0];
    LayerPlan L; L.transposed = true; L.KT = HT; L.MT = F0.KT; L.krow.assign(32 * HT, {-1, 0});
    for (int k = 0; k < H; ++k) L.krow[k] = {0, k};
    L.rcol = F0.col;
    L.bias_off = 0;
    int off = 32 * L.MT;
    plan.layers.push_back(std::move(L));
    if (a.net == NRF_NET_V2) {
        const LayerPlan& C0 = fwd.layers[n + 2];
        LayerPlan D; D.transposed = true; D.KT = H / 64; D.MT = 1; D.krow.assign(32 * D.KT, {-1, 0});
        for (int k = 0; k < H / 2; ++k) D.krow[k] = {n + 2, k};
// ... 106 lines not shown
```

nerf_few_shot_limitations_amd/csrc/packing.hpp:

```cpp
#pragma once
#include <cstdint>
#include <string>
#include <utility>
#include <vector>

#include "../../include/nerfhip.h"

namespace nrf {

struct HostLinear {
    std::vector<float> w, b;
    int out_f = 0, in_f = 0;
};

struct LayerPlan {
    int KT = 0, MT = 0;
    std::vector<int> col;
    std::vector<std::pair<int, int>> row;
    int bias_off = 0;
    bool transposed = false;
    std::vector<std::pair<int, int>> krow;
    std::vector<int> rcol;
};

struct ParamLayout {
    std::vector<int64_t> w_off, b_off;
    std::vector<int> in_f;
    int64_t total = 0;
};
ParamLayout param_layout(const std::vector<HostLinear>& lin);

struct NetPlan {
    std::vector<LayerPlan> layers;
    int n_bias = 0;
    int64_t flops_per_sample = 0;
};

bool make_plan(const nrf_arch& arch, const std::vector<HostLinear>& lin, NetPlan& plan, std::string& err);

int expected_linears(const nrf_arch& arch);

bool make_backward_plan(const nrf_arch& arch, const std::vector<HostLinear>& lin, NetPlan& plan, std::string& err);

bool make_dino_grad_plan(const nrf_arch& arch, const std::vector<HostLinear>& lin, NetPlan& plan, std::string& err);
bool make_input_grad_plan(const nrf_arch& arch, const std::vector<HostLinear>& lin, NetPlan& plan, std::string& err);
bool make_input_grad_v3_plan(const nrf_arch& arch, const std::vector<HostLinear>& lin, NetPlan& plan, std::string& err);

enum { kStream16 = 0, kStreamF32 = 1, kStreamX3 = 2 };
inline int stream_kind(int mma_mode) { return mma_mode == NRF_MMA_F32 ? kStreamF32 : (mma_mode == NRF_MMA_F16X3 ? kStreamX3 : kStream16); }
std::vector<int32_t> stream_sources(const NetPlan& plan, const ParamLayout& lay, int kind);
std::vector<int32_t> bias_sources(const NetPlan& plan, const ParamLayout& lay);

struct GradJobPlan {
    int x_slot = 0, dz_slot = 0, KT = 0, MT = 0, x_first = 0;
    std::vector<int32_t> row_w, row_b;
    std::vector<int32_t> col;
};
struct TrainPlan {
    std::vector<int> slot_tiles;
    int n_mask_slots = 0;
    int aux_floats = 0;
    std::vector<GradJobPlan> jobs;
};
bool make_train_plan(const nrf_arch& arch, const NetPlan& fwd, const ParamLayout& lay, TrainPlan& tp, std::string& err);

struct PackedStream {
    std::vector<uint8_t> bytes;
    uint32_t n_chunks = 0;
};
PackedStream pack_stream(const NetPlan& plan, const std::vector<HostLinear>& lin, int mma_mode);
std::vector<float> pack_bias(const NetPlan& plan, const std::vector<HostLinear>& lin);

uint16_t f32_to_bf16(float x);
uint16_t f32_to_f16(float x);
float f16_to_f32(uint16_t h);

}
```

nerf_few_shot_limitations_amd/csrc/ray_deal.hpp:

```cpp
#pragma once
#include <hip/hip_runtime.h>
#include <stdint.h>

#include <cstdlib>

namespace nrf {

constexpr double kCompositePerSample = 0.0015;
inline double pass_cost(int64_t passes, int l) { return (double)passes * (1.0 + kCompositePerSample * (double)(1 << l)); }

inline int pinned_spw_log2() {
    const char* env = getenv("NRF_SPW");
    return (env && *env) ? atoi(env) : -1;
}

inline int pick_spw_log2(int64_t n_rays, int S, int waves, int cols_per_wave, int cu, int64_t* passes = nullptr, double* cost = nullptr) {
    const int pinned = pinned_spw_log2();
    int max_l = 0;
    while ((2 << max_l) <= cols_per_wave) ++max_l;
    int best = -1;
    double best_t = 0.0;
    for (int l = 0; l <= max_l; ++l) {
        if (pinned >= 0 && l != (pinned < max_l ? pinned : max_l)) continue;
        const int64_t tile = (int64_t)waves * (cols_per_wave >> l);
        const int64_t tiles = (n_rays + tile - 1) / tile;
        const int64_t rounds = (tiles + cu - 1) / cu;
        const int64_t n = rounds * (int64_t)((S + (1 << l) - 1) >> l);
        const double t = pass_cost(n, l);
        if (best < 0 || t < best_t * (1.0 - 1e-9)) {
            best_t = t; best = l;
            if (passes) *passes = n;
            if (cost) *cost = t;
        }
    }
    return best;
}

struct DealRange {
    int64_t first;
    int64_t rays;
};

__host__ __device__ inline DealRange deal_range(int64_t units, int64_t grid, int64_t b, int waves) {
    const int64_t per = units / grid, extra = units % grid;
    return {(b * per + (b < extra ? b : extra)) * waves, (per + (b < extra ? 1 : 0)) * waves};
}

__host__ __device__ inline int deal_split(int64_t left, int whole) {
    int l = 0;
    while ((int64_t)(whole >> l) > left) ++l;
    return l;
}

struct Deal {
    int spw_log2 = 0;
    bool even = false;
    int64_t items = 0;
    int64_t passes = 0;
};

inline void even_range_cost(int64_t rays, int S, int whole, int64_t& passes, double& cost) {
    passes = (rays / whole) * S;
    cost = pass_cost(passes, 0);
    for (int64_t left = rays % whole; left > 0;) {
        const int l = deal_split(left, whole);
        const int64_t n = (S + (1 << l) - 1) >> l;
        passes += n;
        cost += pass_cost(n, l);
        left -= whole >> l;
    }
}

inline Deal pick_deal(int64_t n_rays, int S, int waves, int cols_per_wave, int cu) {
    Deal d;
    double uni_cost = 0.0;
    d.spw_log2 = pick_spw_log2(n_rays, S, waves, cols_per_wave, cu, &d.passes, &uni_cost);
    const int64_t tile = (int64_t)waves * (cols_per_wave >> d.spw_log2);
    d.items = (n_rays + tile - 1) / tile;
    if (pinned_spw_log2() >= 0 || n_rays <= 0 || S <= 0) return d;
    const int64_t units = (n_rays + waves - 1) / waves;
    const int64_t grid = units < cu ? units : cu;
    int64_t passes;
    double cost;
    even_range_cost(deal_range(units, grid, 0, waves).rays, S, waves * cols_per_wave, passes, cost);
    if (units % grid) {
        int64_t p2;
        double c2;
        even_range_cost(deal_range(units, grid, grid - 1, waves).rays, S, waves * cols_per_wave, p2, c2);
        if (p2 > passes) passes = p2;
        if (c2 > cost) cost = c2;
    }
    if (passes < d.passes && cost < uni_cost) {
        d.even = true;
        d.items = units;
        d.passes = passes;
    }
// ... 5 lines not shown
```

nerf_few_shot_limitations_amd/csrc/render_queue_body.inc:

```
    static_assert(NT == 1 || NT == 2, "a wave marches 32 or 64 sample columns");
    constexpr int STRIP = kStrip * NT;
    extern __shared__ __attribute__((aligned(16))) char smem[];
    NRF_LDS char* lds = (NRF_LDS char*)smem;
    NRF_LDS float* bias = (NRF_LDS float*)(lds + kLdsRing);
    NRF_LDS int* flags = (NRF_LDS int*)(bias + kBiasMaxFloats);
    NRF_LDS float* zl = (NRF_LDS float*)(flags + 16);
    NRF_LDS float* st = zl + kLadderLds;
    constexpr int nthreads = WAVES * 64;
    int tid_now = threadIdx.x;
    NRF_LDS float* st_me = st + tid_now;
    auto ST = [&](int f) -> NRF_LDS float& { return st_me[f * nthreads]; };
    typedef typename Mode::Act Act;
    constexpr int KT0 = pe_tiles(LP);

    int lane = threadIdx.x & 63, c = lane & 31, h = lane >> 5;
    const int wave = __builtin_amdgcn_readfirstlane(threadIdx.x >> 6);
    const RenderArgs& a = P.a;
    const int S = a.n_samples;
    static_assert(WAVES * 64 <= kRenderThreads, "state rows are sized for 4 waves");
    {
        const DepthLadder lad = make_ladder(a.near, a.far, S, a.lindisp, nullptr);
        for (int i = threadIdx.x; i < S; i += blockDim.x) zl[i] = a.z_ladder ? a.z_ladder[i] : ladder_z(lad, i);
    }
    ST(F_OX) = 0.f; ST(F_OY) = 0.f; ST(F_OZ) = 0.f; ST(F_DX) = 0.f; ST(F_DY) = 0.f; ST(F_DZ) = -1.f; ST(F_Z) = 1.f;
    load_bias_table(bias, P.net.bias, P.net.n_bias);

    Pipe<WAVES, pinned_walk<Mode, NT>()> pipe;
    pipe.init(P.net.stream, P.net.n_chunks, lds);
    pipe.start();

    auto z_base = [&](int s) -> float { return zl[s]; };
    auto z_of = [&](int64_t ray, int s) -> float {
        if (a.z_in) return a.z_in[ray * S + s];
        if (!a.perturb) return z_base(s);
        float u;
        if (a.t_rand) {
            u = a.t_rand[ray * S + s];
        } else {
            int ci;
            const int64_t g = global_ray(a, ray, ci);
            u = counter_uniform(a.seed + (uint64_t)ci * 0x51ED27ull, (uint64_t)g, (uint32_t)s);
        }
        const float zc = z_base(s);
        const float lower = s > 0 ? __fmul_rn(0.5f, __fadd_rn(zc, z_base(s - 1))) : zc;
        const float upper = s < S - 1 ? __fmul_rn(0.5f, __fadd_rn(z_base(s + 1), zc)) : zc;
        return __fadd_rn(lower, __fmul_rn(__fsub_rn(upper, lower), u));
    };

    int ray = -1;
    int s = 0;
    int64_t pool_next = 0, pool_end = 0;
    bool exhausted = false;
    unsigned long long n_eval = 0, n_live = 0;

    auto skip_empty = [&](int64_t rr, int s_from, bool stores, float& z) -> int {
        const float o[3] = {ST(F_OX), ST(F_OY), ST(F_OZ)}, d[3] = {ST(F_DX), ST(F_DY), ST(F_DZ)};
        int s2 = s_from;
        for (; s2 < S; ++s2) {
            z = z_of(rr, s2);
            const float p[3] = {point_on_ray(o[0], d[0], z), point_on_ray(o[1], d[1], z), point_on_ray(o[2], d[2], z)};
            if (!occ_skips(G, p)) break;
            if (stores) {
                if (a.weights) a.weights[rr * S + s2] = 0.0f;
                if (a.z_vals) a.z_vals[rr * S + s2] = z;
            }
        }
        return s2;
    };

    for (int pass = 0;; ++pass) {
        tid_now = threadIdx.x;
        asm volatile("" : "+v"(tid_now));
        lane = tid_now & 63; c = lane & 31; h = lane >> 5;
        st_me = st + tid_now;
        if (!pipe.skip) {
            for (;;) {
                const bool need = ray < 0;
                const uint64_t m = NT == 2 ? (uint64_t)__ballot(need) : (uint64_t)(__ballot(need) & 0xFFFFFFFFull);
                const int cnt = __builtin_popcountll(m);
                if (cnt > 0 && !exhausted) {
                    if (pool_next == pool_end) {
                        unsigned long long base = 0;
                        if (lane == 0) base = atomicAdd(a.queue, (unsigned long long)STRIP);
                        base = ((unsigned long long)__builtin_amdgcn_readfirstlane((unsigned)(base >> 32)) << 32) |
                               (unsigned)__builtin_amdgcn_readfirstlane((unsigned)base);
                        if ((int64_t)base >= a.n_rays) {
                            exhausted = true;
                        } else {
                            pool_next = (int64_t)base;
                            pool_end = (int64_t)base + STRIP < a.n_rays ? (int64_t)base + STRIP : a.n_rays;
                        }
                    }
                    if (pool_next < pool_end) {
                        const int64_t idx = pool_next + __builtin_popcountll(m & ((1ull << (NT == 2 ? lane : c)) - 1ull));
                        if (need && idx < pool_end) {
                            ray = (int)idx;
                            s = 0;
                            float o[3], d[3];
                            if (a.camera_mode) {
                                int ci;
                                const int64_t g = global_ray(a, idx, ci);
                                camera_ray(a.cams[ci], g, o, d);
                            } else {
#pragma unroll
                                for (int k = 0; k < 3; ++k) { o[k] = a.rays_o[idx * 3 + k]; d[k] = a.rays_d[idx * 3 + k]; }
                            }
                            ST(F_OX) = o[0]; ST(F_OY) = o[1]; ST(F_OZ) = o[2];
                            ST(F_DX) = d[0]; ST(F_DY) = d[1]; ST(F_DZ) = d[2];
                            ST(F_NORM) = ray_norm(d);
                            if constexpr (!OCC) {
                                ST(F_Z) = z_of(idx, 0);
                            } else {
                                const bool stores = NT == 2 || h == 0;
                                float z = 0.0f;
                                s = skip_empty(idx, 0, stores, z);
                                ST(F_Z) = z;
                                if (s >= S) {
                                    if (stores) {
                                        const float bg = a.white_bkgd ? 1.0f : 0.0f;
                                        if (a.interleaved) {
                                            *(float4*)(a.rgb + idx * 4) = make_float4(bg, bg, bg, 0.0f);
                                        } else {
                                            a.rgb[idx * 3 + 0] = bg;
                                            a.rgb[idx * 3 + 1] = bg;
                                            a.rgb[idx * 3 + 2] = bg;
                                            a.depth[idx] = 0.0f;
                                        }
                                    }
                                    ray = -1;
                                }
                            }
                            ST(F_T) = 1.0f; ST(F_R) = 0.0f; ST(F_G) = 0.0f; ST(F_B) = 0.0f; ST(F_DEPTH) = 0.0f; ST(F_ACC) = 0.0f;
                        }
                        pool_next = pool_next + cnt < pool_end ? pool_next + cnt : pool_end;
                    }
                }
                if (!OCC || cnt == 0 || exhausted) break;
            }
            const int run_dry = (exhausted && pool_next == pool_end && !__any(ray >= 0)) ? 1 : 0;
            pipe.skip = (uint32_t)__builtin_amdgcn_readfirstlane(run_dry);
            if constexpr (OCC) {
                if (G.stats && !pipe.skip) {
                    const uint64_t live = NT == 2 ? (uint64_t)__ballot(ray >= 0) : (uint64_t)(__ballot(ray >= 0) & 0xFFFFFFFFull);
                    n_eval += (unsigned)__builtin_popcountll(live);
                    n_live += 1;
                }
            }
        }

        auto SQ = [&](int n, int f) -> NRF_LDS float& { return (NT == 1 ? st_me : st_me - lane + c + 32 * n)[f * nthreads]; };
        auto dirT = [&](Act (&dt)[1][NT]) {
#pragma unroll
            for (int n = 0; n < NT; ++n) {
                const float d[3] = {SQ(n, F_DX), SQ(n, F_DY), SQ(n, F_DZ)};
                Act t1[pe_tiles(LD)];
                encode3<Mode, LD>(d, h, t1);
                dt[0][n] = t1[0];
            }
        };
        DinoHeld<Mode, Net::kDino ? Net::KT0 - KT0 : 1> held[NT];
        auto inputs = [&](const float (&w0)[NT], const float (&w1)[NT], Act (&x)[Net::KT0][NT], auto pass_) {
            constexpr int PASS = decltype(pass_)::value;
#pragma unroll
            for (int n = 0; n < NT; ++n) {
                const float zc = SQ(n, F_Z);
                float p[3];
                p[0] = point_on_ray(SQ(n, F_OX), SQ(n, F_DX), zc);
                p[1] = point_on_ray(SQ(n, F_OY), SQ(n, F_DY), zc);
                p[2] = point_on_ray(SQ(n, F_OZ), SQ(n, F_DZ), zc);
                DinoTaps tp;
                DinoRaw<Net::kDino ? Net::KT0 - KT0 : 1> raw;
                if constexpr (Net::kDino && PASS == 0) {
                    tp = dino_taps(a.dino, p);
                    raw.issue(a.dino.features, tp, h);
                }
                Act e1[KT0];
                encode3<Mode, LP>(p, h, e1, w0[n]);
#pragma unroll
                for (int t = 0; t < KT0; ++t) x[t][n] = e1[t];
                if constexpr (Net::kDino) {
                    constexpr int DT = Net::KT0 - KT0;
                    if constexpr (PASS == 0) held[n].finish(raw, tp);
                    Act dt[DT];
                    held[n].template tiles<PASS>(w1[n], dt);
#pragma unroll
                    for (int t = 0; t < DT; ++t) x[KT0 + t][n] = dt[t];
                }
            }
        };
        float out4[NT][4];
        Net::eval(pipe, bias, h, P.net.n_layers, inputs, dirT, out4);

        if (!pipe.skip && ray >= 0) {
            const bool last = (s + 1 == S);
            const float zc = ST(F_Z);
            const float norm = ST(F_NORM);
            const float zn = last ? 0.0f : z_of(ray, s + 1);
            const float dist = last ? __fmul_rn(1e10f, norm) : __fmul_rn(__fsub_rn(zn, zc), norm);
            Composite comp;
            comp.T = ST(F_T); comp.r = ST(F_R); comp.g = ST(F_G); comp.b = ST(F_B); comp.depth = ST(F_DEPTH); comp.acc = ST(F_ACC);
            float v[4];
#pragma unroll
            for (int k = 0; k < 4; ++k) v[k] = NT == 2 ? pick_reg(out4[0][k], out4[NT - 1][k], h != 0) : out4[0][k];
            const float w = comp.template add<Mode::FAST_EXP>(v[3], sigmoid_sel<Mode::FAST_EXP>(v[0]),
                                                              sigmoid_sel<Mode::FAST_EXP>(v[1]), sigmoid_sel<Mode::FAST_EXP>(v[2]), zc, dist);
            const int64_t rr = ray;
            const bool stores = NT == 2 || h == 0;
            if (stores) {
                if (a.weights) a.weights[rr * S + s] = w;
                if (a.z_vals) a.z_vals[rr * S + s] = zc;
            }
            bool fin = last || comp.T < a.ert_eps;
            int s_next = s + 1;
            float z_next = zn;
            if constexpr (OCC) {
                if (!fin) {
                    s_next = skip_empty(rr, s + 1, stores, z_next);
                    fin = s_next >= S;
                }
            }
            if (fin) {
                if (stores) {
                    for (int s2 = s_next; s2 < S; ++s2) {
                        if (a.weights) a.weights[rr * S + s2] = 0.0f;
                        if (a.z_vals) a.z_vals[rr * S + s2] = z_of(rr, s2);
                    }
                    float r = comp.r, g = comp.g, b = comp.b;
                    if (a.white_bkgd) {
                        const float bg = __fsub_rn(1.0f, comp.acc);
                        r = __fadd_rn(r, bg); g = __fadd_rn(g, bg); b = __fadd_rn(b, bg);
                    }
                    if (a.interleaved) {
                        *(float4*)(a.rgb + rr * 4) = make_float4(r, g, b, comp.depth);
                    } else {
                        a.rgb[rr * 3 + 0] = r;
                        a.rgb[rr * 3 + 1] = g;
                        a.rgb[rr * 3 + 2] = b;
                        a.depth[rr] = comp.depth;
                    }
                }
                ray = -1;
            } else {
                ST(F_T) = comp.T; ST(F_R) = comp.r; ST(F_G) = comp.g; ST(F_B) = comp.b; ST(F_DEPTH) = comp.depth; ST(F_ACC) = comp.acc;
                ST(F_Z) = z_next;
                s = s_next;
            }
        }

        if ((pass & 3) == 3) {
            if (lane == 0) flags[((pass >> 2) & 1) * WAVES + wave] = (int)pipe.skip;
            asm volatile("s_waitcnt lgkmcnt(0)" ::: "memory");
            __builtin_amdgcn_s_barrier();
            const NRF_LDS int* fl = flags + ((pass >> 2) & 1) * WAVES;
            int all_done = 1;
#pragma unroll
            for (int wv = 0; wv < WAVES; ++wv) all_done &= fl[wv];
            if (all_done) break;
        }
    }
    if constexpr (OCC) {
        if (G.stats && lane == 0) {
            atomicAdd(G.stats, n_eval);
            atomicAdd(G.stats + 1, n_live);
        }
    }
    pipe.drain();
```

Baseline: 1545 M ray-samples/s.

## Add 16-column MFMA walk for v1 NeRF MLP with repacked weight stream

```diff
diff --git a/include/nerfhip.h b/include/nerfhip.h
--- a/include/nerfhip.h
+++ b/include/nerfhip.h
@@ -185,6 +185,12 @@
 int nrf_debug_pack_input_grad(const nrf_arch* arch, const nrf_linear* linears, int n_linear, int mma_mode,
                               uint8_t* stream_out, int64_t stream_cap, int64_t* stream_bytes);
 
+int nrf_debug_pack_walk16(const nrf_arch* arch, const nrf_linear* linears, int n_linear, int mma_mode,
+                          uint8_t* stream_out, int64_t stream_cap, int64_t* stream_bytes,
+                          int32_t* sources_out, int64_t sources_cap, int64_t* n_sources);
+
+int nrf_debug_set_walk16(int walk);
+
 int nrf_debug_pack_input_grad_v3(const nrf_arch* arch, const nrf_linear* linears, int n_linear, int mma_mode,
                                  uint8_t* stream_out, int64_t stream_cap, int64_t* stream_bytes);
 
diff --git a/nerf_few_shot_limitations_amd/_lib.py b/nerf_few_shot_limitations_amd/_lib.py
--- a/nerf_few_shot_limitations_amd/_lib.py
+++ b/nerf_few_shot_limitations_amd/_lib.py
@@ -162,6 +162,9 @@
                                                       C.c_void_p]),
     "nrf_debug_pack_input_grad_v3": (C.c_int, [C.POINTER(nrf_arch), C.POINTER(nrf_linear), C.c_int, C.c_int, C.c_void_p, C.c_int64,
                                                C.POINTER(C.c_int64)]),
+    "nrf_debug_set_walk16": (C.c_int, [C.c_int]),
+    "nrf_debug_pack_walk16": (C.c_int, [C.POINTER(nrf_arch), C.POINTER(nrf_linear), C.c_int, C.c_int, C.c_void_p, C.c_int64, C.POINTER(C.c_int64),
+                                        C.c_void_p, C.c_int64, C.POINTER(C.c_int64)]),
     "nrf_param_count": (C.c_int64, [C.c_void_p]),
     "nrf_model_update_device": (C.c_int, [C.c_void_p, C.c_void_p, C.c_int, C.c_void_p]),
     "nrf_train_context_bytes": (C.c_int64, [C.c_void_p, C.c_int, C.c_int64]),
diff --git a/nerf_few_shot_limitations_amd/build.py b/nerf_few_shot_limitations_amd/build.py
--- a/nerf_few_shot_limitations_amd/build.py
+++ b/nerf_few_shot_limitations_amd/build.py
@@ -11,13 +11,16 @@
 OBJ = os.path.join(PKG, "build")
 LIB = os.path.join(PKG, "libnerfhip.so")
 INCLUDE = os.path.join(os.path.dirname(PKG), "include")
+W16_OBJ = os.path.join(OBJ, "w16")
 
 HALF16 = ["-DNRF_TU_HALF=16", "-DNRF_ACT_AGPR=1", "-mllvm", "-amdgpu-mfma-vgpr-form=1"]
 HALF32 = ["-DNRF_TU_HALF=32"]
 FUSED = [(f"fused_{fam}.hip", f"fused_{fam}_{half}", flags) for fam in ("v1", "v2", "v3", "v3w") for half, flags in (("16", HALF16), ("32", HALF32))]
 TAIL = [("fused_tail.hip", "fused_tail", HALF32)]
 OCC = [(f"fused_occ_{fam}.hip", f"fused_occ_{fam}_{half}", flags) for fam in ("v1", "v2", "v3", "v3w") for half, flags in (("16", HALF16), ("32", HALF32))]
-SOURCES = FUSED + OCC + TAIL + [(f, os.path.splitext(f)[0], []) for f in
+W16_DIR = "w16"
+W16 = [("fused_w16_v1.hip", os.path.join(W16_DIR, "fused_w16_v1"), HALF16), ("fused_occ_w16_v1.hip", os.path.join(W16_DIR, "fused_occ_w16_v1"), HALF16)]
+SOURCES = FUSED + OCC + W16 + TAIL + [(f, os.path.splitext(f)[0], []) for f in
                    ("fused_kernels.hip", "train_shared.hip", "train_v1.hip", "train_v2.hip", "train_v3.hip", "train_dino_grad.hip", "train_input_grad.hip", "train_input_grad_v3.hip", "staged_kernels.hip", "api.cpp",
                     "packing.cpp")]
 FLAGS = ["--offload-arch=gfx950", "-O3", "-std=c++17", "-fPIC", "-x", "hip", "-Wall", "-Wno-unused-function", "-Wno-unused-variable",
@@ -57,7 +60,7 @@
     deps = _deps()
     if not force and os.path.exists(LIB) and os.path.getmtime(LIB) >= _newest(deps):
         return LIB
-    os.makedirs(OBJ, exist_ok=True)
+    os.makedirs(W16_OBJ, exist_ok=True)
 
     def one(item):
         src, name, flags = item
diff --git a/nerf_few_shot_limitations_amd/csrc/api.cpp b/nerf_few_shot_limitations_amd/csrc/api.cpp
--- a/nerf_few_shot_limitations_amd/csrc/api.cpp
+++ b/nerf_few_shot_limitations_amd/csrc/api.cpp
@@ -107,6 +107,11 @@
     int32_t* d_src[2][3] = {{nullptr, nullptr, nullptr}, {nullptr, nullptr, nullptr}};
     int64_t n_src[2][3] = {{0, 0, 0}, {0, 0, 0}};
     int32_t* d_bias_src = nullptr;
+    bool walk16 = false;
+    nrf::NetPlan plan16w;
+    void* d_stream16w[2] = {nullptr, nullptr};
+    int32_t* d_src16w = nullptr;
+    int64_t n_src16w = 0;
 };
 
 namespace {
@@ -120,6 +125,19 @@
         m->net.stream[mode] = m->d_stream[mode];
         m->net.n_chunks[mode] = m->h_stream[mode].n_chunks;
     }
+    m->walk16 = m->arch.net == NRF_NET_V1 && m->arch.pos_freq == 10;
+    if (m->walk16) {
+        std::string err;
+        if (!nrf::make_walk16_plan(m->arch, m->lin, m->plan16w, err)) return fail(NRF_EINVAL, err);
+        for (int mode = 0; mode < 2; ++mode) {
+            const nrf::PackedStream ps = nrf::pack_stream_walk16(m->plan16w, m->lin, mode);
+            if (allocate) NRF_HIP(hipMalloc(&m->d_stream16w[mode], ps.bytes.size()));
+            NRF_HIP(hipMemcpyAsync(m->d_stream16w[mode], ps.bytes.data(), ps.bytes.size(), hipMemcpyHostToDevice, s));
+            NRF_HIP(hipStreamSynchronize(s));
+            m->net.stream16w[mode] = m->d_stream16w[mode];
+            m->net.n_chunks16w[mode] = ps.n_chunks;
+        }
+    }
     m->lin_stale = false;
     if (m->train_ready) {
         for (int mode = 0; mode < 3; ++mode) {
@@ -151,6 +169,12 @@
         NRF_HIP(hipMalloc((void**)&m->d_src[0][kind], src.size() * sizeof(int32_t)));
         NRF_HIP(hipMemcpy(m->d_src[0][kind], src.data(), src.size() * sizeof(int32_t), hipMemcpyHostToDevice));
         m->n_src[0][kind] = (int64_t)src.size();
+    }
+    if (m->walk16) {
+        const std::vector<int32_t> src = nrf::stream_sources(m->plan16w, m->layout, nrf::kStream16W);
+        NRF_HIP(hipMalloc((void**)&m->d_src16w, src.size() * sizeof(int32_t)));
+        NRF_HIP(hipMemcpy(m->d_src16w, src.data(), src.size() * sizeof(int32_t), hipMemcpyHostToDevice));
+        m->n_src16w = (int64_t)src.size();
     }
     const std::vector<int32_t> bsrc = nrf::bias_sources(m->plan, m->layout);
     NRF_HIP(hipMalloc((void**)&m->d_bias_src, bsrc.size() * sizeof(int32_t)));
@@ -372,6 +396,9 @@
     DeviceGuard guard(m->device);
     for (int i = 0; i < nrf::kModes; ++i)
         if (m->d_stream[i]) (void)hipFree(m->d_stream[i]);
+    for (int i = 0; i < 2; ++i)
+        if (m->d_stream16w[i]) (void)hipFree(m->d_stream16w[i]);
+    if (m->d_src16w) (void)hipFree(m->d_src16w);
     if (m->d_bias) (void)hipFree(m->d_bias);
     if (m->d_queues) (void)hipFree(m->d_queues);
     for (int i = 0; i < 3; ++i)
@@ -676,6 +703,13 @@
         void* out[3] = {m->d_stream[mode], bwd ? m->d_bstream[mode] : nullptr, bias ? m->d_bias : nullptr};
         rc = nrf::launch_repack3(flat_params, src, n, modes, out, s);
         if (rc != NRF_OK) return fail(rc, "repack launch failed");
+        if (m->walk16 && mode < 2) {
+            const int32_t* src16[3] = {m->d_src16w, nullptr, nullptr};
+            const int64_t n16[3] = {m->n_src16w, 0, 0};
+            void* out16[3] = {m->d_stream16w[mode], nullptr, nullptr};
+            rc = nrf::launch_repack3(flat_params, src16, n16, modes, out16, s);
+            if (rc != NRF_OK) return fail(rc, "repack launch failed");
+        }
         bias = false;
     }
     m->lin_stale = true;
@@ -1205,6 +1239,35 @@
     return NRF_OK;
 }
 
+int nrf_debug_set_walk16(int walk) {
+    if (walk < -1 || walk > 1) return fail(NRF_EINVAL, "nrf_debug_set_walk16: -1 (defaults), 0 or 1");
+    nrf::walk16_pin() = walk;
+    return NRF_OK;
+}
+
+int nrf_debug_pack_walk16(const nrf_arch* arch, const nrf_linear* linears, int n_linear, int mma_mode, uint8_t* stream_out, int64_t stream_cap,
+                          int64_t* stream_bytes, int32_t* sources_out, int64_t sources_cap, int64_t* n_sources) {
+    if (!arch || !linears || n_linear <= 0) return fail(NRF_EINVAL, "nrf_debug_pack_walk16: null argument");
+    if (mma_mode != NRF_MMA_BF16 && mma_mode != NRF_MMA_F16) return fail(NRF_EINVAL, "nrf_debug_pack_walk16: bf16 or f16");
+    std::string err;
+    std::vector<nrf::HostLinear> lin;
+    nrf::NetPlan plan;
+    if (!copy_linears(linears, n_linear, lin, err) || !nrf::make_walk16_plan(*arch, lin, plan, err)) return fail(NRF_EINVAL, err);
+    const nrf::PackedStream ps = nrf::pack_stream_walk16(plan, lin, mma_mode);
+    const std::vector<int32_t> src = nrf::stream_sources(plan, nrf::param_layout(lin), nrf::kStream16W);
+    if (stream_bytes) *stream_bytes = (int64_t)ps.bytes.size();
+    if (n_sources) *n_sources = (int64_t)src.size();
+    if (stream_out) {
+        if (stream_cap < (int64_t)ps.bytes.size()) return fail(NRF_EINVAL, "stream_out too small");
+        std::memcpy(stream_out, ps.bytes.data(), ps.bytes.size());
+    }
+    if (sources_out) {
+        if (sources_cap < (int64_t)src.size()) return fail(NRF_EINVAL, "sources_out too small");
+        std::memcpy(sources_out, src.data(), src.size() * sizeof(int32_t));
+    }
+    return NRF_OK;
+}
+
 int nrf_debug_pack_input_grad_v3(const nrf_arch* arch, const nrf_linear* linears, int n_linear, int mma_mode, uint8_t* stream_out, int64_t stream_cap,
                                  int64_t* stream_bytes) {
     if (!arch || !linears || n_linear <= 0) return fail(NRF_EINVAL, "nrf_debug_pack_input_grad_v3: null argument");
diff --git a/nerf_few_shot_limitations_amd/csrc/feature_map.hpp b/nerf_few_shot_limitations_amd/csrc/feature_map.hpp
--- a/nerf_few_shot_limitations_amd/csrc/feature_map.hpp
+++ b/nerf_few_shot_limitations_amd/csrc/feature_map.hpp
@@ -21,4 +21,22 @@
     return 32 * t + (r & 3) + 8 * (r >> 2) + 4 * h;
 }
 
+constexpr __host__ __device__ int pe16_half(int L) { return (L + 1) / 2; }
+constexpr __host__ __device__ int pe16_tiles(int L) { return (3 * pe16_half(L) + 1 + 7) / 8; }
+constexpr __host__ __device__ int pe16_ref_index(int L, int u, int g) {
+    const int FH = pe16_half(L);
+    if (u < 3 * FH) {
+        const int f = u / 3 + FH * (g >> 1);
+        return f < L ? 3 + 6 * f + 3 * (g & 1) + (u % 3) : -1;
+    }
+    if (u == 3 * FH) return g == 0 ? 0 : (g == 1 ? 2 : (g == 2 ? 1 : -1));
+    return -1;
 }
+constexpr __host__ __device__ int slot16_k(int u, int g) {
+    const int t = u >> 3, j = u & 7;
+    return 32 * t + 16 * (j >> 2) + 4 * g + (j & 3);
+}
+constexpr __host__ __device__ int k16_group(int k) { return (k >> 2) & 3; }
+constexpr __host__ __device__ int k16_slot(int k) { return 8 * (k >> 5) + 4 * ((k >> 4) & 1) + (k & 3); }
+
+}
diff --git a/nerf_few_shot_limitations_amd/csrc/fused_impl.hpp b/nerf_few_shot_limitations_amd/csrc/fused_impl.hpp
--- a/nerf_few_shot_limitations_amd/csrc/fused_impl.hpp
+++ b/nerf_few_shot_limitations_amd/csrc/fused_impl.hpp
@@ -5,6 +5,7 @@
 #include "kernels.hpp"
 #include "nets.hpp"
 #include "ray_deal.hpp"
+#include "walk16.hpp"
 
 namespace nrf {
 
@@ -58,6 +59,10 @@
     return take_hi ? hi : lo;
 }
 
+__device__ __forceinline__ float pick_reg4(float a, float b, float c, float d, int tile) {
+    return pick_reg(pick_reg(a, b, (tile & 1) != 0), pick_reg(c, d, (tile & 1) != 0), (tile & 2) != 0);
+}
+
 __device__ __forceinline__ void load_bias_table(NRF_LDS float* bias, const float* src, int n) {
     for (int i = threadIdx.x; i < n; i += blockDim.x) bias[i] = src[i];
     __syncthreads();
@@ -86,8 +91,10 @@
 
 template <class Net, class Mode, int NT, int WAVES, int LP, int LD, int PART>
 __device__ __forceinline__ void render_march(const RenderKArgs& P) {
-    static_assert(NT == 1 || NT == 2, "a wave marches 32 or 64 sample columns");
-    constexpr int COLS = 32 * NT;
+    constexpr int CW = ColMap<Mode>::kTileCols, CWL = ColMap<Mode>::kTileLog2;
+    constexpr bool W16 = ColMap<Mode>::kWalk16;
+    static_assert(W16 ? NT == 4 : (NT == 1 || NT == 2), "a wave marches 32 or 64 sample columns");
+    constexpr int COLS = CW * NT;
     extern __shared__ __attribute__((aligned(16))) char smem[];
     NRF_LDS char* lds = (NRF_LDS char*)smem;
     NRF_LDS float* bias = (NRF_LDS float*)(lds + kLdsRing);
@@ -99,7 +106,7 @@
     typedef typename Mode::Act Act;
     constexpr int KT0 = pe_tiles(LP);
 
-    int lane = threadIdx.x & 63, c = lane & 31, h = lane >> 5;
+    int lane = threadIdx.x & 63, c = lane & (CW - 1), h = lane >> CWL;
     const int wave = __builtin_amdgcn_readfirstlane(threadIdx.x >> 6);
     const RenderArgs& a = P.a;
     const int S = a.n_samples;
@@ -158,7 +165,7 @@
             base = next * (int64_t)(WAVES * (COLS >> spw_log2));
             next += gridDim.x;
         }
-        const int rpw_log2 = (NT == 2 ? 6 : 5) - spw_log2;
+        const int rpw_log2 = (COLS == 64 ? 6 : 5) - spw_log2;
         const int SPW = 1 << spw_log2, RPW = COLS >> spw_log2;
         const int n_pass = PART == kTail ? 1 : (SM + SPW - 1) >> spw_log2;
         auto column_ray = [&](int q) -> int64_t {
@@ -194,11 +201,12 @@
         for (int p = 0; p < n_pass; ++p) {
             tid_now = threadIdx.x;
             asm volatile("" : "+v"(tid_now));
-            lane = tid_now & 63; c = lane & 31; h = lane >> 5;
+            lane = tid_now & 63; c = lane & (CW - 1); h = lane >> CWL;
             st_me = st + tid_now;
 
-            auto SQ = [&](int n, int f) -> NRF_LDS float& { return (NT == 1 ? st_me : st_me - lane + c + 32 * n)[f * nthreads]; };
+            auto SQ = [&](int n, int f) -> NRF_LDS float& { return (NT == 1 ? st_me : st_me - lane + c + CW * n)[f * nthreads]; };
             auto dirT = [&](Act (&dt)[1][NT]) {
+                if constexpr (!W16) {
 #pragma unroll
                 for (int n = 0; n < NT; ++n) {
                     const float d[3] = {SQ(n, F_DX), SQ(n, F_DY), SQ(n, F_DZ)};
@@ -206,6 +214,7 @@
                     encode3<Mode, LD>(d, h, t1);
                     dt[0][n] = t1[0];
                 }
+                }
             };
             DinoHeld<Mode, Net::kDino ? Net::KT0 - KT0 : 1> held[NT];
             auto inputs = [&](const float (&w0)[NT], const float (&w1)[NT], Act (&x)[Net::KT0][NT], auto pass_) {
@@ -216,7 +225,7 @@
                     if (SPW == 1) {
                         zc = SQ(n, F_Z);
                     } else {
-                        const int q = c + 32 * n;
+                        const int q = c + CW * n;
                         const int sc = p * SPW + (q >> rpw_log2);
                         zc = z_ray(column_ray(q), sc < S ? sc : S - 1);
                     }
@@ -231,7 +240,8 @@
                         raw.issue(a.dino.features, tp, h);
                     }
                     Act e1[KT0];
-                    encode3<Mode, LP>(pt, h, e1, w0[n]);
+                    if constexpr (W16) encode3_w16<Mode, LP>(pt, h, e1, w0[n]);
+                    else encode3<Mode, LP>(pt, h, e1, w0[n]);
 #pragma unroll
                     for (int t = 0; t < KT0; ++t) x[t][n] = e1[t];
                     if constexpr (Net::kDino) {
@@ -250,7 +260,7 @@
 
             tid_now = threadIdx.x;
             asm volatile("" : "+v"(tid_now));
-            lane = tid_now & 63; c = lane & 31; h = lane >> 5;
+            lane = tid_now & 63; c = lane & (CW - 1); h = lane >> CWL;
             st_me = st + tid_now;
             const int64_t rid = column_ray(lane);
             const int64_t raw = base + wave * RPW + (lane & (RPW - 1));
@@ -264,7 +274,10 @@
                 const bool last = PART == kTail || (PART == kWhole && s + 1 == S);
                 float v[4];
 #pragma unroll
-                for (int k = 0; k < 4; ++k) v[k] = NT == 2 ? pick_reg(out4[0][k], out4[NT - 1][k], h != 0) : out4[0][k];
+                for (int k = 0; k < 4; ++k) {
+                    if constexpr (NT == 4) v[k] = pick_reg4(out4[0][k], out4[1][k], out4[NT / 2][k], out4[NT - 1][k], h);
+                    else v[k] = NT == 2 ? pick_reg(out4[0][k], out4[NT - 1][k], h != 0) : out4[0][k];
+                }
                 const float zn = last ? 0.0f : z_ray(rid, s + 1);
                 const float dist = last ? __fmul_rn(1e10f, norm) : __fmul_rn(__fsub_rn(zn, zo), norm);
                 const float w = comp.template add<Mode::FAST_EXP>(v[3], sigmoid_sel<Mode::FAST_EXP>(v[0]), sigmoid_sel<Mode::FAST_EXP>(v[1]),
@@ -275,14 +288,17 @@
                 }
                 zo = zn;
             } else {
-                const int q = NT == 2 ? lane : c;
+                const int q = NT >= 2 ? lane : c;
                 const int sq = p * SPW + (q >> rpw_log2);
                 float ca = 0.0f, cr = 0.0f, cg = 0.0f, cb = 0.0f, cz = 0.0f;
                 if (sq < SM) {
                     const bool last = PART == kWhole && (sq + 1 == S);
                     float v[4];
 #pragma unroll
-                    for (int k = 0; k < 4; ++k) v[k] = NT == 2 ? pick_reg(out4[0][k], out4[NT - 1][k], h != 0) : out4[0][k];
+                    for (int k = 0; k < 4; ++k) {
+                        if constexpr (NT == 4) v[k] = pick_reg4(out4[0][k], out4[1][k], out4[NT / 2][k], out4[NT - 1][k], h);
+                        else v[k] = NT == 2 ? pick_reg(out4[0][k], out4[NT - 1][k], h != 0) : out4[0][k];
+                    }
                     cz = z_ray(rid, sq);
                     const float zn = last ? 0.0f : z_ray(rid, sq + 1);
                     const float dist = last ? __fmul_rn(1e10f, norm) : __fmul_rn(__fsub_rn(zn, cz), norm);
@@ -293,7 +309,7 @@
                     const int s = p * SPW + j;
                     if (s >= SM) break;
                     const int qj = lane + (j << rpw_log2);
-                    const int src = (NT == 2 ? (qj & 63) : ((lane & 32) | (qj & 31))) << 2;
+                    const int src = (NT >= 2 ? (qj & 63) : ((lane & 32) | (qj & 31))) << 2;
                     auto from = [&](float x) { return __builtin_bit_cast(float, __builtin_amdgcn_ds_bpermute(src, __builtin_bit_cast(int, x))); };
                     const float aj = from(ca), rj = from(cr), gj = from(cg), bj = from(cb), zj = from(cz);
                     const float w = comp.add_alpha(aj, rj, gj, bj, zj);
@@ -492,9 +508,13 @@
     return NRF_OK;
 }
 
-NetArgs net_args(const DeviceNet& net, int mode) {
+NetArgs net_args(const DeviceNet& net, int mode, bool walk16 = false) {
     NetArgs n;
     n.stream = net.stream[mode]; n.bias = net.bias; n.n_chunks = net.n_chunks[mode]; n.n_bias = net.n_bias; n.n_layers = net.arch.n_layers;
+    if (walk16) {
+        n.stream = net.stream16w[mode];
+        n.n_chunks = net.n_chunks16w[mode];
+    }
     return n;
 }
 
@@ -516,10 +536,10 @@
 int run_render_v(const DeviceNet& net, int mode, const RenderArgs& a, hipStream_t s, std::string& err) {
     RenderKArgs k;
     k.a = a;
-    const Deal d = pick_deal(a.n_rays, a.n_samples, WAVES, 32 * NT, net.cu_count);
+    const Deal d = pick_deal(a.n_rays, a.n_samples, WAVES, ColMap<Mode>::kTileCols * NT, net.cu_count);
     k.a.spw_log2 = d.spw_log2;
     k.even = d.even;
-    return launch_persistent<render_kernel<Net, Mode, NT, WAVES, LP, LD>, WAVES, kLdsBytesQueue>(net, net_args(net, mode), k, d.items, s, "render", err);
+    return launch_persistent<render_kernel<Net, Mode, NT, WAVES, LP, LD>, WAVES, kLdsBytesQueue>(net, net_args(net, mode, ColMap<Mode>::kWalk16), k, d.items, s, "render", err);
 }
 
 template <class Net, class Mode, int NT, int WAVES, int LP, int LD>
@@ -527,10 +547,10 @@
     RenderKArgs k;
     k.a = a;
     k.carry = carry;
-    const Deal d = pick_deal(a.n_rays, a.n_samples - 1, WAVES, 32 * NT, net.cu_count);
+    const Deal d = pick_deal(a.n_rays, a.n_samples - 1, WAVES, ColMap<Mode>::kTileCols * NT, net.cu_count);
     k.a.spw_log2 = d.spw_log2;
     k.even = d.even;
-    return launch_persistent<render_hold_kernel<Net, Mode, NT, WAVES, LP, LD>, WAVES, kLdsBytesQueue>(net, net_args(net, mode), k, d.items,
+    return launch_persistent<render_hold_kernel<Net, Mode, NT, WAVES, LP, LD>, WAVES, kLdsBytesQueue>(net, net_args(net, mode, ColMap<Mode>::kWalk16), k, d.items,
                                                                                                       s, "render (tail mode, prefix)", err);
 }
 
@@ -548,7 +568,7 @@
 inline RenderKArgs& render_part(RenderKArgs& k) { return k; }
 inline RenderKArgs& render_part(OccKArgs& k) { return k.r; }
 
-template <auto kernel, int NT, int WAVES, class KArgs>
+template <auto kernel, int NT, int WAVES, bool WALK16 = false, class KArgs>
 int launch_queue(const DeviceNet& net, int mode, RenderArgs a, KArgs k, hipStream_t s, std::string& err) {
     static unsigned char done[64] = {};
     const int prepared = prepare(kernel, net.device, done, err, kLdsBytesQueue);
@@ -558,7 +578,7 @@
     hipError_t e = hipMemsetAsync(a.queue, 0, sizeof(unsigned long long), s);
     if (e != hipSuccess) { err = std::string("queue reset: ") + hipGetErrorString(e); return NRF_EHIP; }
     RenderKArgs& r = render_part(k);
-    r.net = net_args(net, mode);
+    r.net = net_args(net, mode, WALK16);
     r.a = a;
     r.n_tiles = 0;
     const int64_t strips = (a.n_rays + kStrip * NT - 1) / (kStrip * NT);
@@ -572,7 +592,7 @@
 
 template <class Net, class Mode, int NT, int WAVES, int LP, int LD>
 int run_render_queue(const DeviceNet& net, int mode, const RenderArgs& a, hipStream_t s, std::string& err) {
-    return launch_queue<render_queue_kernel<Net, Mode, NT, WAVES, LP, LD>, NT, WAVES>(net, mode, a, RenderKArgs{}, s, err);
+    return launch_queue<render_queue_kernel<Net, Mode, NT, WAVES, LP, LD>, ColMap<Mode>::kTileCols * NT / kStrip, WAVES, ColMap<Mode>::kWalk16>(net, mode, a, RenderKArgs{}, s, err);
 }
 
 template <class Net, class Mode, int NT, int WAVES, int LP, int LD>
@@ -580,7 +600,7 @@
     if (!net.queues || a.n_rays >= (int64_t)1 << 31) { err = "render with a grid: launch too large (>= 2^31 rays)"; return NRF_EINVAL; }
     OccKArgs k{};
     k.g = g;
-    return launch_queue<render_queue_occ_kernel<Net, Mode, NT, WAVES, LP, LD>, NT, WAVES>(net, mode, a, k, s, err);
+    return launch_queue<render_queue_occ_kernel<Net, Mode, NT, WAVES, LP, LD>, ColMap<Mode>::kTileCols * NT / kStrip, WAVES, ColMap<Mode>::kWalk16>(net, mode, a, k, s, err);
 }
 
 template <class Net, class Mode, int NT, int WAVES, int LP, int LD>
@@ -628,6 +648,11 @@
         default:            return FN<NETT(ModeF32, 1), ModeF32, 1, 4, LP, 4>(__VA_ARGS__);           \
     }
 #endif
+#define NRF_DISPATCH_W16(FN, LP, ...)                                                                        \
+    switch (mode) {                                                                                           \
+        case NRF_MMA_BF16: return FN<NetV1W<ModeBF16W, 4, LP>, ModeBF16W, 4, 4, LP, 4>(__VA_ARGS__);          \
+        default:           return FN<NetV1W<ModeF16W, 4, LP>, ModeF16W, 4, 4, LP, 4>(__VA_ARGS__);            \
+    }
 #define NRF_NET_V1_10(M, NT) NetV1<M, NT, 10>
 #define NRF_NET_V2_10(M, NT) NetV2<M, NT, 10>
 #define NRF_NET_V3_12_64(M, NT) NetV3<M, NT, 12, 2>
@@ -654,6 +679,9 @@
         return (mode == NRF_MMA_BF16 || mode == NRF_MMA_F16) ? forward_##fam##_16(net, mode, k, s, err) : forward_##fam##_32(net, mode, k, s, err); \
     }
 NRF_DECLARE_FAMILY(v1)
+int render_w16_v1(const DeviceNet& net, int mode, const RenderArgs& a, hipStream_t s, std::string& err);
+int render_hold_w16_v1(const DeviceNet& net, int mode, const RenderArgs& a, float* carry, hipStream_t s, std::string& err);
+int render_occ_w16_v1(const DeviceNet& net, int mode, const RenderArgs& a, const OccDev& g, hipStream_t s, std::string& err);
 NRF_DECLARE_FAMILY(v2)
 NRF_DECLARE_FAMILY(v3)
 NRF_DECLARE_FAMILY(v3w)
diff --git a/nerf_few_shot_limitations_amd/csrc/fused_kernels.hip b/nerf_few_shot_limitations_amd/csrc/fused_kernels.hip
--- a/nerf_few_shot_limitations_amd/csrc/fused_kernels.hip
+++ b/nerf_few_shot_limitations_amd/csrc/fused_kernels.hip
@@ -5,7 +5,7 @@
 int launch_render(const DeviceNet& net, int mode, const RenderArgs& a, hipStream_t s, std::string& err) {
     if (!check_net(net, mode, err)) return NRF_EINVAL;
     if (a.n_rays <= 0) return NRF_OK;
-    if (net.arch.net == NRF_NET_V1 && net.arch.pos_freq == 10) return render_v1(net, mode, a, s, err);
+    if (net.arch.net == NRF_NET_V1 && net.arch.pos_freq == 10) return walk16_selected(mode) ? render_w16_v1(net, mode, a, s, err) : render_v1(net, mode, a, s, err);
     if (net.arch.net == NRF_NET_V2 && net.arch.pos_freq == 10) return render_v2(net, mode, a, s, err);
     if (net.arch.net == NRF_NET_V3 && net.arch.pos_freq == 12 && net.arch.dino_dim == 64) return render_v3(net, mode, a, s, err);
     if (net.arch.net == NRF_NET_V3 && net.arch.pos_freq == 12 && net.arch.dino_dim == 128) return render_v3w(net, mode, a, s, err);
@@ -16,7 +16,7 @@
 int launch_render_occ(const DeviceNet& net, int mode, const RenderArgs& a, const OccDev& g, hipStream_t s, std::string& err) {
     if (!check_net(net, mode, err)) return NRF_EINVAL;
     if (a.n_rays <= 0) return NRF_OK;
-    if (net.arch.net == NRF_NET_V1 && net.arch.pos_freq == 10) return render_occ_v1(net, mode, a, g, s, err);
+    if (net.arch.net == NRF_NET_V1 && net.arch.pos_freq == 10) return walk16_selected(mode) ? render_occ_w16_v1(net, mode, a, g, s, err) : render_occ_v1(net, mode, a, g, s, err);
     if (net.arch.net == NRF_NET_V2 && net.arch.pos_freq == 10) return render_occ_v2(net, mode, a, g, s, err);
     if (net.arch.net == NRF_NET_V3 && net.arch.pos_freq == 12 && net.arch.dino_dim == 64) return render_occ_v3(net, mode, a, g, s, err);
     if (net.arch.net == NRF_NET_V3 && net.arch.pos_freq == 12 && net.arch.dino_dim == 128) return render_occ_v3w(net, mode, a, g, s, err);
@@ -30,7 +30,7 @@
     const bool prefix = a.n_samples > 1;
     int rc = NRF_OK;
     if (net.arch.net == NRF_NET_V1 && net.arch.pos_freq == 10) {
-        if (prefix) rc = render_hold_v1_16(net, base_mode, a, carry, s, err);
+        if (prefix) rc = walk16_selected(base_mode) ? render_hold_w16_v1(net, base_mode, a, carry, s, err) : render_hold_v1_16(net, base_mode, a, carry, s, err);
         return rc != NRF_OK ? rc : render_tail_v1(net, a, carry, s, err);
     }
     if (net.arch.net == NRF_NET_V2 && net.arch.pos_freq == 10) {
diff --git a/nerf_few_shot_limitations_amd/csrc/fused_occ_w16_v1.hip b/nerf_few_shot_limitations_amd/csrc/fused_occ_w16_v1.hip
--- /dev/null
+++ b/nerf_few_shot_limitations_amd/csrc/fused_occ_w16_v1.hip
@@ -0,0 +1,7 @@
+#include "fused_impl.hpp"
+
+namespace nrf {
+
+int render_occ_w16_v1(const DeviceNet& net, int mode, const RenderArgs& a, const OccDev& g, hipStream_t s, std::string& err) { NRF_DISPATCH_W16(run_render_occ, 10, net, mode, a, g, s, err) }
+
+}
diff --git a/nerf_few_shot_limitations_amd/csrc/fused_w16_v1.hip b/nerf_few_shot_limitations_amd/csrc/fused_w16_v1.hip
--- /dev/null
+++ b/nerf_few_shot_limitations_amd/csrc/fused_w16_v1.hip
@@ -0,0 +1,8 @@
+#include "fused_impl.hpp"
+
+namespace nrf {
+
+int render_w16_v1(const DeviceNet& net, int mode, const RenderArgs& a, hipStream_t s, std::string& err) { NRF_DISPATCH_W16(run_render, 10, net, mode, a, s, err) }
+int render_hold_w16_v1(const DeviceNet& net, int mode, const RenderArgs& a, float* carry, hipStream_t s, std::string& err) { NRF_DISPATCH_W16(run_render_hold, 10, net, mode, a, carry, s, err) }
+
+}
diff --git a/nerf_few_shot_limitations_amd/csrc/kernels.hpp b/nerf_few_shot_limitations_amd/csrc/kernels.hpp
--- a/nerf_few_shot_limitations_amd/csrc/kernels.hpp
+++ b/nerf_few_shot_limitations_amd/csrc/kernels.hpp
@@ -22,6 +22,8 @@
     int device;
     int cu_count;
     unsigned long long* queues;
+    const void* stream16w[2];
+    uint32_t n_chunks16w[2];
 };
 
 constexpr int kQueueSlots = 64;
diff --git a/nerf_few_shot_limitations_amd/csrc/packing.cpp b/nerf_few_shot_limitations_amd/csrc/packing.cpp
--- a/nerf_few_shot_limitations_amd/csrc/packing.cpp
+++ b/nerf_few_shot_limitations_amd/csrc/packing.cpp
@@ -255,7 +255,46 @@
 }
 }
 
+bool make_walk16_plan(const nrf_arch& a, const std::vector<HostLinear>& lin, NetPlan& plan, std::string& err) {
+    if (a.net != NRF_NET_V1) { plan = NetPlan(); err = "the 16x16x32 walk is built for the V1 network"; return false; }
+    if (!make_plan(a, lin, plan, err)) return false;
+    if (pe16_tiles(a.pos_freq) != pe_tiles(a.pos_freq)) { err = "the 16x16x32 walk's encoder needs the operand tiles of the 32x32x16 one"; return false; }
+    LayerPlan& L0 = plan.layers.front();
+    for (int k = 0; k < 32 * L0.KT; ++k) L0.col[k] = pe16_ref_index(a.pos_freq, k16_slot(k), k16_group(k));
+    for (auto& L : plan.layers) L.MT16 = 2 * L.MT;
+    LayerPlan& Hd = plan.layers.back();
+    const int n = a.n_layers;
+    Hd.MT16 = 1;
+    Hd.row.assign(32, {-1, 0});
+    for (int rep = 0; rep < 4; ++rep) {
+        for (int c = 0; c < 3; ++c) Hd.row[4 * rep + c] = {n + 1, c};
+        Hd.row[4 * rep + 3] = {n, 0};
+    }
+    return true;
+}
+
+namespace {
+std::vector<int32_t> walk16_sources(const NetPlan& plan, const ParamLayout& lay) {
+    size_t total_frags = 0;
+    for (const auto& L : plan.layers) total_frags += ((size_t)L.MT16 * L.KT + kChunkFrags - 1) / kChunkFrags * kChunkFrags;
+    std::vector<int32_t> src(total_frags * 512, -1);
+    size_t frag = 0;
+    for (const auto& L : plan.layers) {
+        for (int m = 0; m < L.MT16; ++m)
+            for (int t = 0; t < L.KT; ++t, ++frag)
+                for (int lane = 0; lane < 64; ++lane) {
+                    const int i = lane & 15, g = lane >> 4;
+                    for (int e = 0; e < 8; ++e)
+                        src[(frag * 64 + lane) * 8 + e] = (int32_t)element_source(L, lay, 16 * m + i, slot16_k(8 * t + e, g));
+                }
+        frag = (frag + kChunkFrags - 1) / kChunkFrags * kChunkFrags;
+    }
+    return src;
+}
+}
+
 std::vector<int32_t> stream_sources(const NetPlan& plan, const ParamLayout& lay, int kind) {
+    if (kind == kStream16W) return walk16_sources(plan, lay);
     const bool f32 = kind == kStreamF32, x3 = kind == kStreamX3;
     const int SUB = (f32 || x3) ? 4 : 2, n_el = f32 ? 4 : 8;
     size_t total_frags = 0;
@@ -293,7 +332,16 @@
     return b;
 }
 
-PackedStream pack_stream(const NetPlan& plan, const std::vector<HostLinear>& lin, int mode) {
+namespace {
+PackedStream pack_stream_kind(const NetPlan& plan, const std::vector<HostLinear>& lin, int mode, int kind);
+}
+
+PackedStream pack_stream(const NetPlan& plan, const std::vector<HostLinear>& lin, int mode) { return pack_stream_kind(plan, lin, mode, stream_kind(mode)); }
+
+PackedStream pack_stream_walk16(const NetPlan& plan, const std::vector<HostLinear>& lin, int mode) { return pack_stream_kind(plan, lin, mode, kStream16W); }
+
+namespace {
+PackedStream pack_stream_kind(const NetPlan& plan, const std::vector<HostLinear>& lin, int mode, int kind) {
     const bool f32 = (mode == NRF_MMA_F32), x3 = (mode == NRF_MMA_F16X3);
     const ParamLayout lay = param_layout(lin);
     std::vector<float> flat((size_t)lay.total);
@@ -301,7 +349,7 @@
         std::memcpy(flat.data() + lay.w_off[i], lin[i].w.data(), lin[i].w.size() * sizeof(float));
         std::memcpy(flat.data() + lay.b_off[i], lin[i].b.data(), lin[i].b.size() * sizeof(float));
     }
-    const std::vector<int32_t> src = stream_sources(plan, lay, stream_kind(mode));
+    const std::vector<int32_t> src = stream_sources(plan, lay, kind);
     PackedStream out;
     const size_t per_frag = f32 ? 256 : 512;
     out.n_chunks = (uint32_t)(src.size() / per_frag / kChunkFrags);
@@ -322,6 +370,7 @@
         }
     }
     return out;
+}
 }
 
 bool make_backward_plan(const nrf_arch& a, const std::vector<HostLinear>& lin, NetPlan& plan, std::string& err) {
diff --git a/nerf_few_shot_limitations_amd/csrc/packing.hpp b/nerf_few_shot_limitations_amd/csrc/packing.hpp
--- a/nerf_few_shot_limitations_amd/csrc/packing.hpp
+++ b/nerf_few_shot_limitations_amd/csrc/packing.hpp
@@ -18,6 +18,7 @@
     std::vector<int> col;
     std::vector<std::pair<int, int>> row;
     int bias_off = 0;
+    int MT16 = 0;
     bool transposed = false;
     std::vector<std::pair<int, int>> krow;
     std::vector<int> rcol;
@@ -38,6 +39,8 @@
 
 bool make_plan(const nrf_arch& arch, const std::vector<HostLinear>& lin, NetPlan& plan, std::string& err);
 
+bool make_walk16_plan(const nrf_arch& arch, const std::vector<HostLinear>& lin, NetPlan& plan, std::string& err);
+
 int expected_linears(const nrf_arch& arch);
 
 bool make_backward_plan(const nrf_arch& arch, const std::vector<HostLinear>& lin, NetPlan& plan, std::string& err);
@@ -46,7 +49,7 @@
 bool make_input_grad_plan(const nrf_arch& arch, const std::vector<HostLinear>& lin, NetPlan& plan, std::string& err);
 bool make_input_grad_v3_plan(const nrf_arch& arch, const std::vector<HostLinear>& lin, NetPlan& plan, std::string& err);
 
-enum { kStream16 = 0, kStreamF32 = 1, kStreamX3 = 2 };
+enum { kStream16 = 0, kStreamF32 = 1, kStreamX3 = 2, kStream16W = 3 };
 inline int stream_kind(int mma_mode) { return mma_mode == NRF_MMA_F32 ? kStreamF32 : (mma_mode == NRF_MMA_F16X3 ? kStreamX3 : kStream16); }
 std::vector<int32_t> stream_sources(const NetPlan& plan, const ParamLayout& lay, int kind);
 std::vector<int32_t> bias_sources(const NetPlan& plan, const ParamLayout& lay);
@@ -69,6 +72,7 @@
     uint32_t n_chunks = 0;
 };
 PackedStream pack_stream(const NetPlan& plan, const std::vector<HostLinear>& lin, int mma_mode);
+PackedStream pack_stream_walk16(const NetPlan& plan, const std::vector<HostLinear>& lin, int mma_mode);
 std::vector<float> pack_bias(const NetPlan& plan, const std::vector<HostLinear>& lin);
 
 uint16_t f32_to_bf16(float x);
diff --git a/nerf_few_shot_limitations_amd/csrc/ray_deal.hpp b/nerf_few_shot_limitations_amd/csrc/ray_deal.hpp
--- a/nerf_few_shot_limitations_amd/csrc/ray_deal.hpp
+++ b/nerf_few_shot_limitations_amd/csrc/ray_deal.hpp
@@ -12,6 +12,17 @@
 inline int pinned_spw_log2() {
     const char* env = getenv("NRF_SPW");
     return (env && *env) ? atoi(env) : -1;
+}
+
+constexpr bool kWalk16Default[2] = {true, false};
+inline int& walk16_pin() {
+    static int pin = -1;
+    return pin;
+}
+inline bool walk16_selected(int mode) {
+    if (mode < 0 || mode > 1) return false;
+    const int pin = walk16_pin();
+    return pin >= 0 ? pin != 0 : kWalk16Default[mode];
 }
 
 inline int pick_spw_log2(int64_t n_rays, int S, int waves, int cols_per_wave, int cu, int64_t* passes = nullptr, double* cost = nullptr) {
diff --git a/nerf_few_shot_limitations_amd/csrc/render_queue_body.inc b/nerf_few_shot_limitations_amd/csrc/render_queue_body.inc
--- a/nerf_few_shot_limitations_amd/csrc/render_queue_body.inc
+++ b/nerf_few_shot_limitations_amd/csrc/render_queue_body.inc
@@ -1,5 +1,7 @@
-    static_assert(NT == 1 || NT == 2, "a wave marches 32 or 64 sample columns");
-    constexpr int STRIP = kStrip * NT;
+    constexpr int CW = ColMap<Mode>::kTileCols, CWL = ColMap<Mode>::kTileLog2;
+    constexpr bool W16 = ColMap<Mode>::kWalk16;
+    static_assert(W16 ? NT == 4 : (NT == 1 || NT == 2), "a wave marches 32 or 64 sample columns");
+    constexpr int STRIP = kStrip * (CW * NT / 32);
     extern __shared__ __attribute__((aligned(16))) char smem[];
     NRF_LDS char* lds = (NRF_LDS char*)smem;
     NRF_LDS float* bias = (NRF_LDS float*)(lds + kLdsRing);
@@ -13,7 +15,7 @@
     typedef typename Mode::Act Act;
     constexpr int KT0 = pe_tiles(LP);
 
-    int lane = threadIdx.x & 63, c = lane & 31, h = lane >> 5;
+    int lane = threadIdx.x & 63, c = lane & (CW - 1), h = lane >> CWL;
     const int wave = __builtin_amdgcn_readfirstlane(threadIdx.x >> 6);
     const RenderArgs& a = P.a;
     const int S = a.n_samples;
@@ -71,12 +73,12 @@
     for (int pass = 0;; ++pass) {
         tid_now = threadIdx.x;
         asm volatile("" : "+v"(tid_now));
-        lane = tid_now & 63; c = lane & 31; h = lane >> 5;
+        lane = tid_now & 63; c = lane & (CW - 1); h = lane >> CWL;
         st_me = st + tid_now;
         if (!pipe.skip) {
             for (;;) {
                 const bool need = ray < 0;
-                const uint64_t m = NT == 2 ? (uint64_t)__ballot(need) : (uint64_t)(__ballot(need) & 0xFFFFFFFFull);
+                const uint64_t m = NT >= 2 ? (uint64_t)__ballot(need) : (uint64_t)(__ballot(need) & 0xFFFFFFFFull);
                 const int cnt = __builtin_popcountll(m);
                 if (cnt > 0 && !exhausted) {
                     if (pool_next == pool_end) {
@@ -92,7 +94,7 @@
                         }
                     }
                     if (pool_next < pool_end) {
-                        const int64_t idx = pool_next + __builtin_popcountll(m & ((1ull << (NT == 2 ? lane : c)) - 1ull));
+                        const int64_t idx = pool_next + __builtin_popcountll(m & ((1ull << (NT >= 2 ? lane : c)) - 1ull));
                         if (need && idx < pool_end) {
                             ray = (int)idx;
                             s = 0;
@@ -111,7 +113,7 @@
                             if constexpr (!OCC) {
                                 ST(F_Z) = z_of(idx, 0);
                             } else {
-                                const bool stores = NT == 2 || h == 0;
+                                const bool stores = NT >= 2 || h == 0;
                                 float z = 0.0f;
                                 s = skip_empty(idx, 0, stores, z);
                                 ST(F_Z) = z;
@@ -141,21 +143,23 @@
             pipe.skip = (uint32_t)__builtin_amdgcn_readfirstlane(run_dry);
             if constexpr (OCC) {
                 if (G.stats && !pipe.skip) {
-                    const uint64_t live = NT == 2 ? (uint64_t)__ballot(ray >= 0) : (uint64_t)(__ballot(ray >= 0) & 0xFFFFFFFFull);
+                    const uint64_t live = NT >= 2 ? (uint64_t)__ballot(ray >= 0) : (uint64_t)(__ballot(ray >= 0) & 0xFFFFFFFFull);
                     n_eval += (unsigned)__builtin_popcountll(live);
                     n_live += 1;
                 }
             }
         }
 
-        auto SQ = [&](int n, int f) -> NRF_LDS float& { return (NT == 1 ? st_me : st_me - lane + c + 32 * n)[f * nthreads]; };
+        auto SQ = [&](int n, int f) -> NRF_LDS float& { return (NT == 1 ? st_me : st_me - lane + c + CW * n)[f * nthreads]; };
         auto dirT = [&](Act (&dt)[1][NT]) {
+            if constexpr (!W16) {
 #pragma unroll
             for (int n = 0; n < NT; ++n) {
                 const float d[3] = {SQ(n, F_DX), SQ(n, F_DY), SQ(n, F_DZ)};
                 Act t1[pe_tiles(LD)];
                 encode3<Mode, LD>(d, h, t1);
                 dt[0][n] = t1[0];
+            }
             }
         };
         DinoHeld<Mode, Net::kDino ? Net::KT0 - KT0 : 1> held[NT];
@@ -175,7 +179,8 @@
                     raw.issue(a.dino.features, tp, h);
                 }
                 Act e1[KT0];
-                encode3<Mode, LP>(p, h, e1, w0[n]);
+                if constexpr (W16) encode3_w16<Mode, LP>(p, h, e1, w0[n]);
+                else encode3<Mode, LP>(p, h, e1, w0[n]);
 #pragma unroll
                 for (int t = 0; t < KT0; ++t) x[t][n] = e1[t];
                 if constexpr (Net::kDino) {
@@ -201,11 +206,14 @@
             comp.T = ST(F_T); comp.r = ST(F_R); comp.g = ST(F_G); comp.b = ST(F_B); comp.depth = ST(F_DEPTH); comp.acc = ST(F_ACC);
             float v[4];
 #pragma unroll
-            for (int k = 0; k < 4; ++k) v[k] = NT == 2 ? pick_reg(out4[0][k], out4[NT - 1][k], h != 0) : out4[0][k];
+            for (int k = 0; k < 4; ++k) {
+                if constexpr (NT == 4) v[k] = pick_reg4(out4[0][k], out4[1][k], out4[NT / 2][k], out4[NT - 1][k], h);
+                else v[k] = NT == 2 ? pick_reg(out4[0][k], out4[NT - 1][k], h != 0) : out4[0][k];
+            }
             const float w = comp.template add<Mode::FAST_EXP>(v[3], sigmoid_sel<Mode::FAST_EXP>(v[0]),
                                                               sigmoid_sel<Mode::FAST_EXP>(v[1]), sigmoid_sel<Mode::FAST_EXP>(v[2]), zc, dist);
             const int64_t rr = ray;
-            const bool stores = NT == 2 || h == 0;
+            const bool stores = NT >= 2 || h == 0;
             if (stores) {
                 if (a.weights) a.weights[rr * S + s] = w;
                 if (a.z_vals) a.z_vals[rr * S + s] = zc;
diff --git a/nerf_few_shot_limitations_amd/csrc/walk16.hpp b/nerf_few_shot_limitations_amd/csrc/walk16.hpp
--- /dev/null
+++ b/nerf_few_shot_limitations_amd/csrc/walk16.hpp
@@ -0,0 +1,228 @@
+#pragma once
+#include "nets.hpp"
+
+namespace nrf {
+
+struct ModeF16W {
+    static constexpr bool kWalk16 = true;
+    static constexpr bool kPinned = true;
+    static constexpr int TRIG = 1;
+    static constexpr bool FAST_EXP = ModeF16::FAST_EXP;
+    typedef f16x8 frag_t;
+    typedef f16x2 pair_t;
+    struct Act { f16x8 f; };
+    __device__ static __forceinline__ f32x4 mma(const frag_t& a, const Act& b, const f32x4& c) {
+        return __builtin_amdgcn_mfma_f32_16x16x32_f16(a, b.f, c, 0, 0, 0);
+    }
+};
+
+struct ModeBF16W {
+    static constexpr bool kWalk16 = true;
+    static constexpr bool kPinned = true;
+    static constexpr int TRIG = 1;
+    static constexpr bool FAST_EXP = ModeBF16::FAST_EXP;
+    typedef bf16x8 frag_t;
+    typedef bf16x2 pair_t;
+    struct Act { bf16x8 f; };
+    __device__ static __forceinline__ f32x4 mma(const frag_t& a, const Act& b, const f32x4& c) {
+        return __builtin_amdgcn_mfma_f32_16x16x32_bf16(a, b.f, c, 0, 0, 0);
+    }
+};
+
+template <class Mode, class = void>
+struct ColMap { static constexpr int kTileCols = 32, kTileLog2 = 5; static constexpr bool kWalk16 = false; };
+template <class Mode>
+struct ColMap<Mode, typename std::enable_if<Mode::kWalk16>::type> { static constexpr int kTileCols = 16, kTileLog2 = 4; static constexpr bool kWalk16 = true; };
+
+template <class Mode, bool RELU, int PAR, int P>
+__device__ __forceinline__ void to_act_pair16(const f32x4 (&acc)[4], typename Mode::Act (&o)[4]) {
+    constexpr int n = P >> 1, w = P & 1, word = 2 * PAR + w;
+    int nw = pack_pair<typename Mode::pair_t, RELU>(acc[n][2 * w], acc[n][2 * w + 1]);
+    NRF_PIN_ACT1(nw);
+    i32x4 v = __builtin_bit_cast(i32x4, o[n].f);
+    v[word] = nw;
+    if (word == 3) NRF_PARK_ACT(v);
+    o[n].f = __builtin_bit_cast(typename Mode::frag_t, v);
+}
+
+template <class Mode, int L>
+__device__ __forceinline__ void encode3_w16(const float p[3], int g, typename Mode::Act (&out)[pe16_tiles(L)], float scale = 1.0f) {
+    static_assert(L % 2 == 0 && Mode::TRIG == 1, "encode3_w16: an even number of frequencies, v_sin on reduced turns");
+    constexpr int FH = pe16_half(L), KT = pe16_tiles(L);
+    float hi[3], lo[3];
+    const float up = (g >> 1) ? (float)(1u << FH) : 1.0f;
+#pragma unroll
+    for (int c = 0; c < 3; ++c) {
+        const float h0 = p[c] * kInv2PiHi;
+        const float l0 = __builtin_fmaf(p[c], kInv2PiHi, -h0) + p[c] * kInv2PiLo;
+        hi[c] = h0 * up;
+        lo[c] = l0 * up;
+    }
+    const float quarter = (g & 1) ? 0.25f : 0.0f;
+    float e[8 * KT];
+    static_for<8 * KT>([&](auto u_) {
+        constexpr int u = decltype(u_)::value;
+        float v = 0.0f;
+        if constexpr (u < 3 * FH) {
+            constexpr int f = u / 3, c = u % 3;
+            constexpr float sc = (float)(1u << f);
+            const float rev = __builtin_fmaf(lo[c], sc, __builtin_amdgcn_fractf(hi[c] * sc)) + quarter;
+            v = __builtin_amdgcn_sinf(rev);
+        } else if constexpr (u == 3 * FH) {
+            v = g == 0 ? p[0] : (g == 1 ? p[2] : (g == 2 ? p[1] : 0.0f));
+        }
+        e[u] = v * scale;
+    });
+#pragma unroll
+    for (int t = 0; t < KT; ++t) {
+        i32x4 w;
+#pragma unroll
+        for (int j = 0; j < 4; ++j) w[j] = pack_pair<typename Mode::pair_t, false>(e[8 * t + 2 * j], e[8 * t + 2 * j + 1]);
+        out[t].f = __builtin_bit_cast(typename Mode::frag_t, w);
+    }
+}
+
+template <class Mode>
+struct Carry16 {
+    f32x4 tail[4];
+    f32x4 bias0;
+    typename Mode::frag_t fr[kPrefetch];
+};
+
+template <class Mode, int KT, int MT, int CIN, int COUT, bool OWN_BIAS, int TAIL_TILE, class P, class FinSlice, class TailSlice>
+__device__ __forceinline__ void dense_pinned16(P& pipe, const NRF_LDS float* bias, const NRF_LDS float* bias_next,
+                                               const typename Mode::Act (&in)[KT][4], FinSlice&& fin, TailSlice&& tail, Carry16<Mode>& carry) {
+    static_assert((CIN == kCarryNone || CIN == kCarryTail) && (COUT == kCarryNone || COUT == kCarryTail), "this walk chains whole tiles");
+    constexpr int NT = 4, NF = MT * KT, PF = kPrefetch;
+    static_assert(NF >= PF, "layer shorter than the fragment prefetch");
+    constexpr int SPS = KT >= 8 ? 2 : (8 + KT - 1) / KT;
+    constexpr int NSTEP = (8 + SPS - 1) / SPS;
+    static_assert(NSTEP <= KT, "a tile's epilogue must fit into the next tile's steps");
+    static_assert(CIN != kCarryTail || NSTEP <= TAIL_TILE, "the carried tile is read before its slices are done");
+    constexpr int BIAS_AT = KT >= 2 ? KT - 2 : 0;
+    typedef typename Mode::frag_t frag_t;
+    frag_t fr[PF], nxt[PF];
+    static_assert((NF % kChunkFrags == 0 ? kChunkFrags : NF % kChunkFrags) >= P::kFragsPerWave, "last chunk of the layer too short for the spread LDS-DMA issue");
+    auto read = [&](auto g_) -> frag_t {
+        constexpr int g = decltype(g_)::value;
+        if constexpr (g % kChunkFrags == 0) pipe.acquire_begin((g / kChunkFrags) & 1);
+        else if constexpr (g % kChunkFrags < P::kFragsPerWave) pipe.template issue_part<g % kChunkFrags>();
+        return *(const NRF_LDS frag_t*)(pipe.base[(g / kChunkFrags) & 1] + (g % kChunkFrags) * kFragBytes);
+    };
+    auto bias_of = [&](const NRF_LDS float* rows) -> f32x4 { return *(const NRF_LDS f32x4*)rows; };
+    f32x4 acc[2][NT];
+    f32x4 bnext;
+    if constexpr (CIN != kCarryNone) {
+        static_for<PF>([&](auto i_) { fr[decltype(i_)::value] = carry.fr[decltype(i_)::value]; });
+        if constexpr (OWN_BIAS) bnext = bias_of(bias);
+        else bnext = carry.bias0;
+    } else {
+        static_for<PF>([&](auto i_) { fr[decltype(i_)::value] = read(i_); });
+        bnext = bias_of(bias);
+    }
+    f32x4 bias0_next;
+    __builtin_amdgcn_sched_barrier(0);
+    static_for<NF>([&](auto f_) {
+        constexpr int f = decltype(f_)::value;
+        constexpr int m = f / KT, t = f % KT;
+        const frag_t a = fr[f % PF];
+#pragma unroll
+        for (int n = 0; n < NT; ++n) {
+            if constexpr (t == 0) acc[m & 1][n] = Mode::mma(a, in[t][n], bnext);
+            else acc[m & 1][n] = Mode::mma(a, in[t][n], acc[m & 1][n]);
+        }
+        if constexpr (f + PF < NF) fr[f % PF] = read(std::integral_constant<int, f + PF>{});
+        else if constexpr (COUT != kCarryNone) nxt[f + PF - NF] = read(std::integral_constant<int, f + PF - NF>{});
+        if constexpr ((m > 0 || CIN == kCarryTail) && t < NSTEP) {
+            static_for<SPS>([&](auto k_) {
+                constexpr int j = t * SPS + decltype(k_)::value;
+                if constexpr (j < 8) {
+                    if constexpr (m > 0) fin(std::integral_constant<int, m - 1>{}, acc[(m - 1) & 1], std::integral_constant<int, j>{});
+                    else tail(carry.tail, std::integral_constant<int, j>{});
+                }
+            });
+        }
+        if constexpr (t == BIAS_AT) {
+            if constexpr (m + 1 < MT) bnext = bias_of(bias + 16 * (m + 1));
+            else if constexpr (COUT != kCarryNone) bias0_next = bias_of(bias_next);
+        }
+        __builtin_amdgcn_sched_barrier(0);
+    });
+    if constexpr (COUT != kCarryNone) {
+        static_for<PF>([&](auto i_) { carry.fr[decltype(i_)::value] = nxt[decltype(i_)::value]; });
+        carry.bias0 = bias0_next;
+    }
+    if constexpr (COUT == kCarryTail) {
+#pragma unroll
+        for (int n = 0; n < NT; ++n) carry.tail[n] = acc[(MT - 1) & 1][n];
+    } else {
+        static_for<8>([&](auto j_) { fin(std::integral_constant<int, MT - 1>{}, acc[(MT - 1) & 1], j_); });
+    }
+}
+
+template <class Mode, int KT, int CIN, class P>
+__device__ __forceinline__ void dense_act16(P& pipe, const NRF_LDS float* bias, const NRF_LDS float* bias_next,
+                                            typename Mode::Act (&in)[KT][4], typename Mode::Act (&out)[8][4], Carry16<Mode>& carry) {
+    dense_pinned16<Mode, KT, 16, CIN, kCarryTail, false, KT - 1>(pipe, bias, bias_next, in,
+        [&](auto m_, f32x4(&acc)[4], auto j_) {
+            constexpr int m = decltype(m_)::value;
+            to_act_pair16<Mode, true, m & 1, decltype(j_)::value>(acc, out[m >> 1]);
+        },
+        [&](f32x4(&tl)[4], auto j_) { to_act_pair16<Mode, true, 1, decltype(j_)::value>(tl, in[KT - 1]); }, carry);
+}
+
+template <class Mode, class P>
+__device__ __forceinline__ void dense_head16(P& pipe, const NRF_LDS float* bias, typename Mode::Act (&in)[8][4], f32x4 (&out)[4], Carry16<Mode>& carry) {
+    dense_pinned16<Mode, 8, 1, kCarryTail, kCarryNone, true, 7>(pipe, bias, bias, in,
+        [&](auto, f32x4(&acc)[4], auto j_) {
+            constexpr int j = decltype(j_)::value, n = j >> 1, w = j & 1;
+            out[n][2 * w] = acc[n][2 * w];
+            out[n][2 * w + 1] = acc[n][2 * w + 1];
+        },
+        [&](f32x4(&tl)[4], auto j_) { to_act_pair16<Mode, true, 1, decltype(j_)::value>(tl, in[7]); }, carry);
+}
+
+template <class Mode, int NT, int LP>
+struct NetV1W {
+    static_assert(NT == 4 && Mode::kWalk16, "64 columns as four 16-column tiles");
+    static constexpr int KT0 = pe16_tiles(LP);
+    static constexpr int HT = 8;
+    static constexpr bool kNeedsDir = false;
+    static constexpr bool kDino = false;
+    typedef typename Mode::Act Act;
+
+    template <class P, class Inputs, class Dirs>
+    __device__ static __forceinline__ void eval(P& pipe, const NRF_LDS float* bias, int g, int n_layers,
+                                                Inputs&& inputs, Dirs&&, float (&out4)[NT][4]) {
+        Act A[HT][NT], B[HT][NT];
+        Carry16<Mode> cy;
+        const NRF_LDS float* bl = bias + 4 * g;
+        {
+            Act enc[KT0][NT];
+            float one[NT];
+#pragma unroll
+            for (int n = 0; n < NT; ++n) one[n] = 1.0f;
+            inputs(one, one, enc, std::integral_constant<int, 0>{});
+            dense_act16<Mode, KT0, kCarryNone>(pipe, bl, bl + 32 * HT, enc, A, cy);
+        }
+        int boff = 32 * HT;
+        const int hidden = n_layers - 1;
+        for (int p = 0; p < hidden / 2; ++p) {
+            dense_act16<Mode, HT, kCarryTail>(pipe, bl + boff, bl + boff + 32 * HT, A, B, cy); boff += 32 * HT;
+            dense_act16<Mode, HT, kCarryTail>(pipe, bl + boff, bl + boff + 32 * HT, B, A, cy); boff += 32 * HT;
+        }
+        f32x4 head[NT];
+        if (hidden & 1) {
+            dense_act16<Mode, HT, kCarryTail>(pipe, bl + boff, bl + boff + 32 * HT, A, B, cy); boff += 32 * HT;
+            dense_head16<Mode>(pipe, bias + boff + 4 * (g & 1), B, head, cy);
+        } else {
+            dense_head16<Mode>(pipe, bias + boff + 4 * (g & 1), A, head, cy);
+        }
+#pragma unroll
+        for (int n = 0; n < NT; ++n)
+#pragma unroll
+            for (int k = 0; k < 4; ++k) out4[n][k] = head[n][k];
+    }
+};
+
+}
```

Result: no change. 1541 M ray-samples/s (-0.3%).
